# medvedevgroup/TwoPaCo

Hardware: AMD Instinct MI355X
Metric: kmers_hashed_per_sec (higher is better)
Workload: dtype u64

## Files before the change

twopaco_amd/csrc/tpc_capi.hip:

```cpp
#include "tpc_ctx.h"

namespace tpch {

int fail(tpc_ctx *c, int code, const char *fmt, ...)
{
    char buf[512];
    va_list ap;
    va_start(ap, fmt);
    vsnprintf(buf, sizeof buf, fmt, ap);
    va_end(ap);
    if (c) c->err = buf;
    return code;
}





TpcLaunch make_launch(const tpc_ctx *c)
{
    TpcLaunch a;
    a.P = c->P; a.tab = c->tab; a.bases = c->bases; a.nmask = c->nmask; a.n_text = c->n_text;
    a.n_tiles = c->n_tiles; a.filter = c->filter; a.stream = c->stream;
    a.stat_kernel = c->stat_kernel;
    return a;
}

TpcLaunch make_launch_periodic(const tpc_ctx *c)
{
    TpcLaunch a = make_launch(c);
    if (c->periodic && c->periodic_valid) {
        if (c->periodic_any_q) a.per_qs = c->periodic;
        if (c->periodic_any_i) a.per_i = c->periodic + (size_t)(1 + TPC_PER_PLANES) * c->n_words_alloc;
    }
    return a;
}

void ensure_periodic(tpc_ctx *c)
{
    if (c->periodic_valid || !c->opt_periodic || !c->bases || !c->have_params || c->n_words_alloc == 0) return;
    if ((c->sh_world > 1 || c->text_windowed) && !c->opt_shard_periodic && !replicated(c)) return;
    TpcLaunch a = make_launch(c);
    const uint64_t w0 = c->text_windowed ? c->text_w0 : 0, w1 = c->text_windowed ? std::min(c->text_w1, c->n_words) : c->n_words;
    const uint64_t pos_hi = c->text_windowed ? c->text_w1 << 5 : ~0ull;
    uint32_t any[2] = {0, 0};
    uint32_t *flags = reinterpret_cast<uint32_t *>(c->counters + 6);
    if (hipMemsetAsync(flags, 0, sizeof any, c->stream) != hipSuccess) return;
    tpc_launch_periodic_build(a, nullptr, nullptr, 0, nullptr, w0, w1, w0 << 5, pos_hi, flags);
    if (hipMemcpyAsync(any, flags, sizeof any, hipMemcpyDeviceToHost, c->stream) != hipSuccess || hipStreamSynchronize(c->stream) != hipSuccess) return;
    c->periodic_any_q = any[0] != 0; c->periodic_any_i = any[1] != 0;
    if (any[0] || any[1]) {
        const size_t words = (size_t)(2 + TPC_PER_PLANES) * c->n_words_alloc;
        if (!c->periodic && hipMalloc((void **)&c->periodic, words * sizeof(uint32_t)) != hipSuccess) { (void)hipGetLastError(); c->periodic = nullptr; return; }
        if (hipMemsetAsync(c->periodic, 0, words * sizeof(uint32_t), c->stream) != hipSuccess) return;
        tpc_launch_periodic_build(a, c->periodic, c->periodic + c->n_words_alloc, c->n_words_alloc, c->periodic + (size_t)(1 + TPC_PER_PLANES) * c->n_words_alloc, w0, w1, w0 << 5, pos_hi, flags);
        if (hipStreamSynchronize(c->stream) != hipSuccess) return;
    }
    c->periodic_valid = true;
}

uint64_t rotln_host(uint64_t x, int L, int r)
{
    if (r == 0) return x;
    const uint64_t maskn = (1ull << (L - r)) - 1ull;
    return ((x & maskn) << r) | (x >> (L - r));
}

std::atomic<int> tpc_test_fail_mallocs{0};
hipError_t dev_malloc(tpc_ctx *c, void **p, size_t bytes)
{
    hipError_t e = hipErrorOutOfMemory;
    if (tpc_test_fail_mallocs.load(std::memory_order_relaxed) > 0 && tpc_test_fail_mallocs.fetch_sub(1) > 0) *p = nullptr; else e = hipMalloc(p, bytes);
    if (e == hipSuccess) return e;
    (void)hipGetLastError();
    if (!release_partition_buffers(c)) return e;
    e = hipMalloc(p, bytes);
    if (e != hipSuccess) *p = nullptr;
    return e;
}


int read_counter(tpc_ctx *c, int i, uint64_t *out)
{
    unsigned long long v = 0;
    HIPCHK(c, hipMemcpyAsync(&v, c->counters + i, sizeof v, hipMemcpyDeviceToHost, c->stream));
    HIPCHK(c, hipStreamSynchronize(c->stream));
    *out = v;
    return 0;
}


int materialize_reset(tpc_ctx *c)
{
    { int rc0 = flush_pending_apply(c); if (rc0) return rc0; }
    if (!c->filter_zero_pending) return 0;
    Timed t(c, TPC_K_FILTER_RESET);
    HIPCHK(c, hipMemsetAsync(c->filter, 0, c->filter_words * sizeof(uint32_t), c->stream));
    c->filter_zero_pending = false;
    return 0;
}

int flush_pending_apply(tpc_ctx *c)
{
    if (!c->pending_apply) return 0;
    c->pending_apply = false;
    if (c->pending_lists) {
        c->pending_lists = false;
        Timed t(c, TPC_K_FUSED);
        const TpcPartPlan &g = c->pending_pl;
        if (tpc_launch_slice_combine(make_launch(c), g.slice_bits, g.b1, g.b2, g.perm_mult, g.perm_inv, nullptr, nullptr, nullptr, c->cmb_ls, true, c->pending_fresh, nullptr, 0, 1))
            return fail(c, -1, "apply launch failed");
        HIPCHK(c, hipGetLastError());
        return 0;
    }
    c->qb_valid = false;
    if (c->pending_shard) {
        c->pending_shard = false;
        Timed t(c, TPC_K_SHARD_APPLY);
        if (tpc_launch_insert_part_apply_only(make_launch(c), c->pending_pl, c->pending_fresh)) return fail(c, -1, "apply launch failed");
        HIPCHK(c, hipGetLastError());
        return 0;
    }
    Timed t(c, TPC_K_FUSED);
    const size_t ovf_need = std::max<size_t>((size_t)c->pending_novf * sizeof(uint64_t), sizeof(uint64_t));
    if (!ensure_pbuf(c, 4, ovf_need) || !ensure_pbuf(c, 5, 32 * sizeof(unsigned long long))) return fail(c, -10, "out of device memory for the deferred apply's overflow list");
    c->pending_pl.ovf = (uint64_t *)c->pbuf[4];
    c->pending_pl.ovf_cur = (unsigned long long *)c->pbuf[5];
    c->pending_pl.ovf_cap = std::min<uint64_t>(c->pending_pl.ovf_cap, c->pbytes[4] / sizeof(uint64_t));
    const unsigned long long cur[2] = {c->pending_novf, 0};
    if (c->pending_novf) HIPCHK(c, hipMemcpyAsync(c->pending_pl.ovf, c->ikeep_ovf, c->pending_novf * sizeof(uint64_t), hipMemcpyDeviceToDevice, c->stream));
    HIPCHK(c, hipMemcpyAsync(c->pending_pl.ovf_cur, cur, sizeof cur, hipMemcpyHostToDevice, c->stream));
    HIPCHK(c, hipStreamSynchronize(c->stream));
    if (tpc_launch_insert_part_apply_only(make_launch(c), c->pending_pl, c->pending_fresh)) return fail(c, -1, "apply launch failed");
    HIPCHK(c, hipGetLastError());
    return 0;
}

double range_mass(const tpc_ctx *c, uint64_t lo, uint64_t hi)
{
    const double size = (double)(c->P.lmask) + 1.0;
    auto below = [size](double x) { x = std::min(1.0, std::max(0.0, x / size)); return 1.0 - (1.0 - x) * (1.0 - x); };
    return std::min(1.0, std::max(0.0, below((double)hi + 1.0) - below((double)lo)));
}

bool ensure_pbuf(tpc_ctx *c, int i, size_t need)
{
    if (need <= c->pbytes[i]) return true;
    c->qb_valid = false;
    if (c->pbuf[i]) (void)hipFree(c->pbuf[i]);
    c->pbuf[i] = nullptr; c->pbytes[i] = 0;
    if (i == 8) c->off2_uploaded.clear();
    if (i == 11) c->off3_uploaded.clear();
    if (hipMalloc(&c->pbuf[i], need) != hipSuccess) { (void)hipGetLastError(); return false; }
    c->pbytes[i] = need;
    return true;
}

bool release_partition_buffers(tpc_ctx *c)
{
    if (c->pending_apply) return false;
    size_t held = 0;
    for (size_t b : c->pbytes) held += b;
    for (void *p : c->ikeep) if (p) held += 1;
    if (!held) return false;
    (void)hipStreamSynchronize(c->stream);
    c->qb_valid = false;
    for (int i = 0; i < tpc_ctx::NPBUF; i++) {
        if (c->pbuf[i]) (void)hipFree(c->pbuf[i]);
        c->pbuf[i] = nullptr; c->pbytes[i] = 0;
    }
    for (void *&p : c->ikeep) { if (p) (void)hipFree(p); p = nullptr; }
    for (size_t &b : c->ikeep_bytes) b = 0;
    c->off2_uploaded.clear();
    c->off3_uploaded.clear();
    c->sh_have[0] = c->sh_have[1] = false;
    c->stat_pbuf_releases++;
    return true;
}

uint64_t filter_words_for(int L, uint32_t world)
{
    return std::max<uint64_t>(1, ((1ull << L) >> 5) / world) + 1;
}

int64_t part_budget(const tpc_ctx *c)
{
    if (c->opt_part_budget > 0) return c->opt_part_budget;
    size_t free_b = 0, total_b = 0;
    if (hipMemGetInfo(&free_b, &total_b) != hipSuccess) { (void)hipGetLastError(); return (int64_t)40 << 30; }
    size_t held = 0;
    for (size_t b : c->pbytes) held += b;
    const double avail = std::max(0.0, (double)(free_b + held) - (double)(c->bases ? 0 : c->reserve_text_bytes));
    return std::max<int64_t>(std::min<int64_t>((int64_t)40 << 30, (int64_t)(avail * 0.90)), (int64_t)(avail * 0.60));
}

uint64_t next_batches(uint64_t b) { return b + std::max<uint64_t>(1, b / 8); }

uint64_t text_tiles512(const tpc_ctx *c) { return (c->n_text / TPC_RUN + 512) / 512; }

bool replicated(const tpc_ctx *c) { return c->opt_replicate && c->sh_world > 1; }
void pass_tiles(const tpc_ctx *c, uint64_t &t_begin, uint64_t &t_end)
{
    const uint64_t tiles = text_tiles512(c);
    t_begin = 0; t_end = tiles;
    if (replicated(c)) {
        const uint64_t chunk = (tiles + c->sh_world - 1) / c->sh_world;
        t_begin = std::min<uint64_t>(tiles, (uint64_t)c->sh_rank * chunk);
        t_end = std::min<uint64_t>(tiles, t_begin + chunk);
    }
}
uint64_t pass_tile_count(const tpc_ctx *c) { uint64_t a, b; pass_tiles(c, a, b); return std::max<uint64_t>(1, b - a); }

size_t qpart_need(const TpcQPlan &pl, int i)
{
    if (i == 0) return std::max(tpc_qpart_bytes(pl, 0), tpc_qpart_bytes(pl, 9));
    if (i == 9) return 0;
    return tpc_qpart_bytes(pl, i);
}

bool part_hash_supported(const tpc_ctx *c)
{
    if (c->P.q > TPC_KERNEL_MAXQ || tpc_test_force_anyq) return false;
    if (c->P.q > 8 && (c->P.L - c->opt_slice_bits > 24 || c->no_lean)) return false;
    return true;
}

bool plan_query(const tpc_ctx *c, uint64_t lo, uint64_t hi, bool gated, TpcQPlan &pl)
{
    const uint64_t tiles = pass_tile_count(c);
    if (c->P.q > TPC_KERNEL_MAXQ || tpc_test_force_anyq) return false;
    if (!replicated(c) && (c->opt_query_mode == 1 || (c->opt_query_mode == 0 && c->P.L < 28))) return false;
    const int64_t budget = part_budget(c);
    for (uint64_t batches = 1;; batches = next_batches(batches)) {
        const uint64_t per = (tiles + batches - 1) / batches;
        const bool ok = tpc_qpart_plan(c->P.L, c->opt_slice_bits, per, gated ? std::min(1.0, range_mass(c, lo, hi) * 1.15) : 1.0, pl, c->opt_part_levels);
        if (!ok && per * 512 * TPC_RUN <= (1ull << 30)) return false;
        if (ok && ((int64_t)(qpart_need(pl, 0) + tpc_qpart_bytes(pl, 2)) <= budget || (int64_t)per <= c->opt_part_min_tiles)) {
            const double per_slice = 6.0 * (gated ? range_mass(c, lo, hi) : 1.0) * (double)per * 512 * TPC_RUN / (double)(1ull << (c->P.L - pl.slice_bits));
            if (c->opt_query_mode == 0 && batches > 1 && per_slice < 2500.0 && !replicated(c)) return false;
            return true;
        }
        if (per <= 1) return false;
    }
}

int compact_mask(tpc_ctx *c, const uint32_t *m)
{
    Timed t(c, TPC_K_COMPACT);
    uint64_t n = 0;
    int rc = 0;
    if (m == c->rmask && c->rmask_sums_valid) {
        n = c->rmask_sums_n;
    } else {
        c->rmask_sums_valid = false;
        tpc_launch_mask_count(c->stream, m, c->n_words, c->block_sums, c->counters + 2);
        if ((rc = read_counter(c, 2, &n))) return rc;
    }
    rc = ensure(c, c->marks, c->marks_cap, n);
    if (rc) return rc;
    if (n) tpc_launch_mask_scatter(c->stream, m, c->n_words, c->block_sums, c->marks);
    c->n_marks = n;
    return 0;
}

}

extern "C" {

int tpc_ctx_create(int device, tpc_ctx **out)
{
    if (!out) return -1;
    *out = nullptr;
    int n = 0;
    if (hipGetDeviceCount(&n) != hipSuccess || n <= 0) return -2;
    if (device < 0 || device >= n) return -3;
    if (hipSetDevice(device) != hipSuccess) return -4;
    tpc_ctx *c = new tpc_ctx();
    c->device = device;
    c->dbg_ovf = getenv("TPC_DEBUG_OVF") != nullptr; c->dbg_phases = getenv("TPC_PROFILE_PHASES") != nullptr; c->dbg_timing = getenv("TWOPACO_TIMING") != nullptr; c->no_lean = TpcEnv::get().no_lean;
    if (const char *e = getenv("TPC_SHARD_TIGHT")) c->opt_shard_tight = atoi(e) ? 1 : 0;
    if (hipStreamCreate(&c->stream) != hipSuccess) { delete c; return -5; }
    for (int i = 0; i < TPC_K_COUNT; i++) {
        if (hipEventCreate(&c->ev0[i]) != hipSuccess || hipEventCreate(&c->ev1[i]) != hipSuccess) { delete c; return -5; }
    }
    if (hipMalloc((void **)&c->tab, TPC_TAB_WORDS * sizeof(uint64_t)) != hipSuccess ||
        hipMalloc((void **)&c->counters, 8 * sizeof(unsigned long long)) != hipSuccess ||
        hipMalloc((void **)&c->route_scratch, 128 * sizeof(unsigned long long)) != hipSuccess) { delete c; return -6; }
    *out = c;
    return 0;
}

void tpc_ctx_destroy(tpc_ctx *c)
{
    if (!c) return;
    (void)hipSetDevice(c->device);
    (void)hipStreamSynchronize(c->stream);
    void *ptrs[] = { c->tab, c->bases_alloc, c->nmask_alloc, c->filter, c->rmask, c->mask, c->marks, c->block_sums, c->table,
                     c->keys, c->idtab, c->emit_id, c->stream_buf, c->counters, c->route_scratch, c->sh_off, c->scan_blocks, c->sort_scratch, c->seg_name, c->seg_first, c->seg_ev[0], c->seg_ev[1], c->seg_ev[2] };
    for (void *p : ptrs) if (p) (void)hipFree(p);
    stream_part_release(c);
    for (void *p : c->pbuf) if (p) (void)hipFree(p);
    for (void *p : c->ikeep) if (p) (void)hipFree(p);
    if (c->periodic) (void)hipFree(c->periodic);
    if (c->cmb_base) (void)hipFree(c->cmb_base);
    if (c->cmb_cur) (void)hipFree(c->cmb_cur);
    if (c->ikeep_ovf) (void)hipFree(c->ikeep_ovf);
    if (c->iovf_cnt) (void)hipFree(c->iovf_cnt);
    if (c->iovf_off) (void)hipFree(c->iovf_off);
    for (int i = 0; i < TPC_K_COUNT; i++) { if (c->ev0[i]) (void)hipEventDestroy(c->ev0[i]); if (c->ev1[i]) (void)hipEventDestroy(c->ev1[i]); }
    if (c->stream2) (void)hipStreamDestroy(c->stream2);
    if (c->stream) (void)hipStreamDestroy(c->stream);
    delete c;
}

const char *tpc_last_error(const tpc_ctx *c) { return c ? c->err.c_str() : "null context"; }

int tpc_set_option(tpc_ctx *c, const char *name, int64_t value)
{
    if (!c || !name) return -1;
    if (!strcmp(name, "insert_test_first")) { c->opt_test_first = value != 0; return 0; }
    if (!strcmp(name, "insert_mode")) { c->opt_insert_mode = (int)value; return 0; }
    if (!strcmp(name, "slice_bits")) { c->opt_slice_bits = (int)value; return 0; }
    if (!strcmp(name, "query_mode")) { c->opt_query_mode = (int)value; return 0; }
    if (!strcmp(name, "part_budget_bytes")) { c->opt_part_budget = value; return 0; }
    if (!strcmp(name, "part_levels")) { c->opt_part_levels = (int)value; return 0; }
    if (!strcmp(name, "shard_tight_regions")) { c->opt_shard_tight = value ? 1 : 0; c->sh_have[0] = c->sh_have[1] = false; return 0; }
    if (!strcmp(name, "part_min_tiles")) { c->opt_part_min_tiles = value < 1 ? 1 : value; return 0; }
    if (!strcmp(name, "fuse_apply_lookup")) { c->opt_fuse = value != 0; return 0; }
    if (!strcmp(name, "test_q6_pb2")) { tpc_test_q6_pb2 = (int)value; return 0; }
    if (!strcmp(name, "insert_entry_fmt")) { tpc_test_insert_p3 = value == 3; return 0; }
    if (!strcmp(name, "shard_periodic_skip")) { c->opt_shard_periodic = value != 0; return 0; }
    if (!strcmp(name, "periodic_skip")) { c->opt_periodic = value != 0; if (!value) c->periodic_valid = false; return 0; }
    if (!strcmp(name, "test_tight_pinch")) { tpc_test_tight_pinch = (int)value; c->sh_have[0] = c->sh_have[1] = false; return 0; }
    if (!strcmp(name, "test_sched_cap")) { tpc_test_sched_cap = value > 0 ? (uint32_t)value : 0; return 0; }
    if (!strcmp(name, "text_window")) { c->opt_text_window = value != 0; return 0; }
    if (!strcmp(name, "replicate_filter")) { c->opt_replicate = value != 0; return 0; }
    if (!strcmp(name, "test_force_anyq")) { tpc_test_force_anyq = value != 0; return 0; }
    if (!strcmp(name, "test_fail_mallocs")) { tpc_test_fail_mallocs.store(value > 0 ? (int)value : 0); return 0; }
    return fail(c, -1, "unknown option %s", name);
}

int tpc_preload(int device)
{
    if (hipSetDevice(device) != hipSuccess) { (void)hipGetLastError(); return -10; }
    const bool timing = getenv("TWOPACO_TIMING") != nullptr;
    int (*const warm[4])() = { tpc_warm_partition, tpc_warm_qpartition, tpc_warm_pass2, tpc_warm_stream };
    const char *const name[4] = { "partition", "qpartition", "pass2", "stream" };
    for (int i = 0; i < 4; i++) {
        const auto t0 = std::chrono::steady_clock::now();
        if (warm[i]() != 0) return -10;
        if (timing) fprintf(stderr, "[timing]     code object %s: %.1f ms\n", name[i], std::chrono::duration<double, std::milli>(std::chrono::steady_clock::now() - t0).count());
    }
    return 0;
}

int tpc_warmup(tpc_ctx *c)
{
    if (!c) return -1;
    return tpc_preload(c->device);
}

int64_t tpc_get_stat(const tpc_ctx *c, const char *name)
{
    if (!c || !name) return -1;
    if (!strcmp(name, "insert_path")) return c->stat_path[0];
    if (!strcmp(name, "query_path")) return c->stat_path[1];
    if (!strcmp(name, "insert_entry_fmt")) return c->stat_fmt[0];
    if (!strcmp(name, "query_entry_fmt")) return c->stat_fmt[1];
    if (!strcmp(name, "insert_hash_kernel")) return c->stat_kernel[0];
    if (!strcmp(name, "query_hash_kernel")) return c->stat_kernel[1];
    if (!strcmp(name, "query_verify_kernel")) return c->stat_kernel[2];
    if (!strcmp(name, "insert_batches")) return c->stat_batches[0];
    if (!strcmp(name, "query_batches")) return c->stat_batches[1];
    if (!strcmp(name, "query_tiles_per_batch")) return c->stat_q_plan[0];
    if (!strcmp(name, "query_b1")) return c->stat_q_plan[1];
    if (!strcmp(name, "query_b2")) return c->stat_q_plan[2];
    if (!strcmp(name, "query_begun")) return c->stat_q_begun;
    if (!strcmp(name, "filter2_retries")) return c->stat_filter2_retries;
    if (!strcmp(name, "aggregate_retries")) return c->stat_aggregate_retries;
    if (!strcmp(name, "filter2_counted")) return c->stat_filter2_counted;
    if (!strcmp(name, "fused_lookups")) return c->stat_fused;
    if (!strcmp(name, "query_overflow_entries")) return c->stat_query_overflow;
    if (!strcmp(name, "insert_overflow_entries")) return c->stat_insert_overflow;
    if (!strcmp(name, "periodic_skip")) return c->periodic_valid ? 1 : 0;
    if (!strcmp(name, "pbuf_releases")) return c->stat_pbuf_releases;
    if (!strcmp(name, "text_words")) return (int64_t)(c->text_w1 - c->text_w0);
    if (!strcmp(name, "text_word_begin")) return (int64_t)c->text_w0;
    if (!strcmp(name, "text_word_end")) return (int64_t)c->text_w1;
    if (!strcmp(name, "periodic_any_query")) return c->periodic_valid && c->periodic_any_q ? 1 : 0;
    if (!strcmp(name, "periodic_any_insert")) return c->periodic_valid && c->periodic_any_i ? 1 : 0;
    if (!strcmp(name, "device_free_bytes") || !strcmp(name, "device_total_bytes")) {
        size_t free_b = 0, total_b = 0;
        if (hipSetDevice(c->device) != hipSuccess || hipMemGetInfo(&free_b, &total_b) != hipSuccess) { (void)hipGetLastError(); return -1; }
        return (int64_t)(name[7] == 'f' ? free_b : total_b);
    }
    if (!strcmp(name, "round_marks")) return c->marks_valid ? (int64_t)c->n_marks : -1;
    return -1;
}

int tpc_set_params(tpc_ctx *c, int k, int L, int q, const uint64_t *seed_table)
{
    if (!c || !seed_table) return -1;
    if (q < 1 || q > TPC_MAX_Q) return fail(c, -1, "q=%d unsupported (1..%d)", q, TPC_MAX_Q);
    if (L < 2 || L > 62) return fail(c, -1, "filter bits L=%d unsupported (2..62)", L);
    if (k < 1) return fail(c, -1, "k must be positive");
    const int C = (k + 4 + 31) / 32;
    if (C >= 20)
        return fail(c, -1, "The value of K is too big. Please refer to documentaion how to increase the max supported value of K.");
    HIPCHK(c, hipSetDevice(c->device));
    c->P.k = k; c->P.L = L; c->P.q = q; c->P.rk = k % L; c->P.lmask = (1ull << L) - 1ull;
    c->C = C;
    memset(c->tab_host, 0, sizeof c->tab_host);
    for (int i = 0; i < q; i++)
        for (int ch = 0; ch < 5; ch++) {
            const uint64_t h = seed_table[i * 5 + ch];
            if (h > c->P.lmask) return fail(c, -1, "seed table entry exceeds L bits");
            c->tab_host[i * 5 + ch] = h;
            c->tab_host[TPC_TAB_HK + i * 5 + ch] = rotln_host(h, L, c->P.rk);
        }
    HIPCHK(c, hipMemcpy(c->tab, c->tab_host, sizeof c->tab_host, hipMemcpyHostToDevice));
    const uint64_t fw = filter_words_for(L, c->opt_replicate ? 1 : c->sh_world);
    c->sh_have[0] = c->sh_have[1] = false;
    c->pending_lists = false; c->cmb_have_geo = false;
    if (fw != c->filter_words) {
        if (c->filter) (void)hipFree(c->filter);
        c->filter = nullptr;
        HIPCHK(c, hipMalloc((void **)&c->filter, fw * sizeof(uint32_t)));
        c->filter_words = fw;
    }
    c->have_params = true;
    c->periodic_valid = false;
    c->pending_apply = false;
    c->qb_valid = false;
    c->n_keys = 0; c->finalized = false; c->rounds_done = 0; c->mask_dirty = false; c->marks_valid = false; c->rmask_sums_valid = false;
    return 0;
}

int tpc_seq_upload(tpc_ctx *c, const uint64_t *bases, const uint32_t *nmask, uint64_t n_text)
{
    if (!c || !bases || !nmask || n_text < 2) return fail(c, -1, "bad text");
    HIPCHK(c, hipSetDevice(c->device));
    const auto t_begin = std::chrono::steady_clock::now();
    c->qb_valid = false;
    const uint64_t nw = (n_text + 31) / 32;
    if (!((nmask[0] & 1u) && ((nmask[(n_text - 1) >> 5] >> ((n_text - 1) & 31)) & 1u)))
        return fail(c, -1, "text must start and end with the N separator");
    const uint64_t tiles = (nw + TPC_TILE_THREADS - 1) / TPC_TILE_THREADS;
    const uint64_t alloc = ((n_text / TPC_RUN + 512) / 512) * 512 + TPC_XW_MAX + 2;
    uint64_t w0 = 0, w1 = alloc;
    const bool windowed = c->opt_text_window && c->sh_world > 1;
    if (windowed) {
        const uint64_t t512 = (n_text / TPC_RUN + 512) / 512, chunk = (t512 + c->sh_world - 1) / c->sh_world;
        const uint64_t ta = std::min<uint64_t>(t512, (uint64_t)c->sh_rank * chunk), tb = std::min<uint64_t>(t512, ta + chunk);
        w0 = ta * 512 > 0 ? ta * 512 - 1 : 0;
        w1 = std::min<uint64_t>(alloc, tb * 512 + TPC_XW_MAX + 2);
        if (w1 <= w0) w1 = w0 + 1;
    }
    for (void *p : { (void *)c->bases_alloc, (void *)c->nmask_alloc, (void *)c->rmask, (void *)c->mask, (void *)c->block_sums, (void *)c->periodic })
        if (p) (void)hipFree(p);
    c->periodic = nullptr; c->periodic_valid = false;
    c->bases = nullptr; c->nmask = nullptr; c->bases_alloc = nullptr; c->nmask_alloc = nullptr; c->rmask = nullptr; c->mask = nullptr; c->block_sums = nullptr;
    const uint64_t wn = w1 - w0;
    HIPCHK(c, dev_malloc(c, (void **)&c->bases_alloc, wn * sizeof(uint64_t)));
    HIPCHK(c, dev_malloc(c, (void **)&c->nmask_alloc, wn * sizeof(uint32_t)));
    HIPCHK(c, dev_malloc(c, (void **)&c->rmask, alloc * sizeof(uint32_t)));
    HIPCHK(c, dev_malloc(c, (void **)&c->mask, alloc * sizeof(uint32_t)));
    HIPCHK(c, dev_malloc(c, (void **)&c->block_sums, (alloc / 256 + 2 + 64) * sizeof(uint64_t)));
    HIPCHK(c, hipMemsetAsync(c->bases_alloc, 0, wn * sizeof(uint64_t), c->stream));
    HIPCHK(c, hipMemsetAsync(c->nmask_alloc, 0xFF, wn * sizeof(uint32_t), c->stream));
    HIPCHK(c, hipMemsetAsync(c->rmask, 0, alloc * sizeof(uint32_t), c->stream));
    HIPCHK(c, hipMemsetAsync(c->mask, 0, alloc * sizeof(uint32_t), c->stream));
    const uint64_t ce = std::min(nw, w1);
    uint32_t last_word = 0;
    if (ce > w0) {
        HIPCHK(c, hipMemcpyAsync(c->bases_alloc, bases + w0, (ce - w0) * sizeof(uint64_t), hipMemcpyHostToDevice, c->stream));
        HIPCHK(c, hipMemcpyAsync(c->nmask_alloc, nmask + w0, (ce - w0) * sizeof(uint32_t), hipMemcpyHostToDevice, c->stream));
        if ((n_text & 31) && ce == nw) {
            last_word = nmask[nw - 1] | (~0u << (n_text & 31));
            HIPCHK(c, hipMemcpyAsync(c->nmask_alloc + (nw - 1 - w0), &last_word, sizeof last_word, hipMemcpyHostToDevice, c->stream));
        }
    }
    HIPCHK(c, hipStreamSynchronize(c->stream));
    if (c->dbg_timing)
        fprintf(stderr, "[timing]   tpc_seq_upload (allocations, %.0f MB host to device): %.1f ms\n", (double)(ce > w0 ? (ce - w0) * 12 : 0) / 1e6,
                std::chrono::duration<double, std::milli>(std::chrono::steady_clock::now() - t_begin).count());
    c->bases = c->bases_alloc - w0;
    c->nmask = c->nmask_alloc - w0;
    c->text_windowed = windowed; c->text_w0 = w0; c->text_w1 = w1;
    c->pending_apply = false;
    c->n_text = n_text; c->n_words = (n_text >> 5) + 1; c->n_words_alloc = alloc; c->n_tiles = tiles;
    c->n_keys = 0; c->finalized = false; c->rounds_done = 0; c->mask_dirty = false; c->marks_valid = false; c->rmask_sums_valid = false;
    return 0;
}

int tpc_run_begin(tpc_ctx *c)
{
    if (!c) return -1;
    c->n_keys = 0; c->finalized = false; c->rounds_done = 0; c->mask_dirty = false; c->marks_valid = false; c->rmask_sums_valid = false;
    c->n_marks = 0; c->n_emit = 0; c->keys_host.clear();
    return 0;
}

int tpc_filter_reset(tpc_ctx *c)
{
    if (!c || !c->have_params) return fail(c, -1, "set_params first");
    c->filter_zero_pending = true;
    c->pending_apply = false;
    c->pending_shard = false;
    c->pending_lists = false;
    c->ev_used[TPC_K_FILTER_RESET] = false;
    return 0;
}

int tpc_pass1_insert(tpc_ctx *c, uint64_t lo, uint64_t hi, uint64_t *n_kmers)
{
    if (!c || !c->have_params || !c->bases) return fail(c, -1, "set_params and seq_upload first");
    if (c->sh_world > 1 && !c->opt_replicate) return fail(c, -1, "the filter is sharded: use tpc_shard_hash / tpc_shard_apply");
    HIPCHK(c, hipSetDevice(c->device));
    const bool gated = !(lo == 0 && hi >= c->P.lmask);
    { int rc0 = flush_pending_apply(c); if (rc0) return rc0; }
    c->qb_valid = false;
    ensure_periodic(c);
    if (n_kmers) HIPCHK(c, hipMemsetAsync(c->counters, 0, sizeof(unsigned long long), c->stream));
    uint64_t t_begin, t_end;
    pass_tiles(c, t_begin, t_end);
    TpcPartPlan pl;
    const double m_ins = gated ? range_mass(c, lo, hi) : 1.0;
    const double ins_frac = gated ? std::min(1.0, (1.0 - (1.0 - m_ins) * (1.0 - m_ins)) * 1.15) : 1.0;
    const uint64_t tiles = pass_tile_count(c);
    uint64_t batches = 1;
    bool defer = false;
    bool part = ((c->opt_insert_mode != 1 && !(c->opt_insert_mode == 0 && c->P.L < 28)) || replicated(c)) && part_hash_supported(c);
    if (replicated(c) && !part && c->P.q <= TPC_KERNEL_MAXQ)
        return fail(c, -1, "a replicated multi-GPU pass needs the partitioned hash kernels (q=%d, L=%d, slice_bits=%d are outside what they cover)", c->P.q, c->P.L, c->opt_slice_bits);
    if (part) {
        const int64_t budget = part_budget(c);
        for (;; batches = next_batches(batches)) {
            const uint64_t per = (tiles + batches - 1) / batches;
            if (!tpc_part_plan(c->P.L, c->P.q, c->opt_slice_bits, per, ins_frac, pl, c->opt_part_levels)) { part = false; break; }
            if ((int64_t)(std::max(tpc_part_buf1_bytes(pl), tpc_part_buf3_bytes(pl)) + tpc_part_buf2_bytes(pl)) <= budget || (int64_t)per <= c->opt_part_min_tiles) break;
        }
        if (part && c->opt_insert_mode == 0 && batches > 1 && !replicated(c)) {
            const double per_slice = (double)c->P.q * ins_frac * (double)pl.n_tiles * 512 * TPC_RUN / (double)(1ull << (c->P.L - pl.slice_bits));
            if (per_slice < (double)(1ull << pl.slice_bits) / 800.0) part = false;
        }
    }
    if (part) {
        size_t need[tpc_ctx::NPBUF] = { std::max(tpc_part_buf1_bytes(pl), tpc_part_buf3_bytes(pl)), tpc_part_cnt1_bytes(pl), tpc_part_buf2_bytes(pl), tpc_part_cnt2_bytes(pl),
                                        pl.ovf_cap * sizeof(uint64_t), 32 * sizeof(unsigned long long), 0, 0, 0, 0, tpc_part_cnt3_bytes(pl), 0 };
        TpcQPlan qpl;
        const bool qpart = plan_query(c, lo, hi, gated, qpl);
        for (int i = 0; i < tpc_ctx::NPBUF && qpart; i++) need[i] = std::max(need[i], qpart_need(qpl, i));
        for (int i = 0; i < tpc_ctx::NPBUF && part; i++) if (need[i]) part = ensure_pbuf(c, i, need[i]);
        defer = part && c->opt_fuse && batches == 1 && qpart && pl.b3 == 0 && qpl.b3 == 0 && qpl.slice_bits == pl.slice_bits &&
                qpl.b1 == pl.b1 && qpl.b2 == pl.b2 && (qpl.fmt == 6 || pl.fmt2 == 0);
        if (defer) {
            const size_t want[2] = { tpc_part_buf2_bytes(pl), tpc_part_cnt2_bytes(pl) };
            for (int i = 0; i < 2 && defer; i++) {
                if (want[i] <= c->ikeep_bytes[i]) continue;
                if (c->ikeep[i]) (void)hipFree(c->ikeep[i]);
                c->ikeep[i] = nullptr; c->ikeep_bytes[i] = 0;
                if (hipMalloc(&c->ikeep[i], want[i]) != hipSuccess) { (void)hipGetLastError(); defer = false; break; }
                c->ikeep_bytes[i] = want[i];
            }
        }
    }
    if (part) {
        pl.buf1 = (uint32_t *)c->pbuf[0]; pl.cnt1 = (uint32_t *)c->pbuf[1]; pl.buf2 = (uint32_t *)c->pbuf[2]; pl.cnt2 = (uint32_t *)c->pbuf[3];
        pl.ovf = (uint64_t *)c->pbuf[4]; pl.ovf_cur = (unsigned long long *)c->pbuf[5];
        pl.buf3 = (uint32_t *)c->pbuf[0]; pl.cnt3 = (uint32_t *)c->pbuf[10];
        if (defer) { pl.buf2 = (uint32_t *)c->ikeep[0]; pl.cnt2 = (uint32_t *)c->ikeep[1]; }
        bool fresh = c->filter_zero_pending;
        unsigned long long ov[2] = {0, 0};
        bool overflowed = false;
        uint64_t per_batch = 1;
        {
            Timed t(c, TPC_K_INSERT);
            if (fresh) HIPCHK(c, hipMemsetAsync(c->filter + (c->filter_words - 1), 0, sizeof(uint32_t), c->stream));
            const uint64_t per = pl.n_tiles;
            per_batch = per;
            for (uint64_t t0 = t_begin; t0 < t_end || t0 == t_begin; t0 += per) {
                pl.tile0 = t0;
                pl.n_tiles = t0 < t_end ? std::min<uint64_t>(per, t_end - t0) : 0;
                HIPCHK(c, hipMemsetAsync(pl.ovf_cur, 0, 2 * sizeof(unsigned long long), c->stream));
                if (defer) {
                    TpcPartPlan p1 = pl;
                    p1.rbuf1 = p1.buf1; p1.rcnt1 = p1.cnt1;
                    if (tpc_launch_insert_part_hash(make_launch_periodic(c), p1, lo, hi, gated, n_kmers ? c->counters : nullptr) ||
                        tpc_launch_insert_part_split(make_launch(c), p1)) return fail(c, -1, "partitioned insert launch failed");
                    HIPCHK(c, hipMemcpyAsync(ov, pl.ovf_cur, sizeof ov, hipMemcpyDeviceToHost, c->stream));
                    HIPCHK(c, hipStreamSynchronize(c->stream));
                    bool keep = ov[0] <= TPC_FUSE_MAX_OVF && ov[1] == 0;
                    const uint32_t n_slices = 1u << (p1.b1 + p1.b2);
                    if (keep && ov[0]) {
                        if (c->ikeep_ovf_cap < ov[0]) {
                            if (c->ikeep_ovf) (void)hipFree(c->ikeep_ovf);
                            c->ikeep_ovf = nullptr; c->ikeep_ovf_cap = 0;
                            const uint64_t cap = std::max<uint64_t>(4096, ov[0] + ov[0] / 4);
                            if (hipMalloc((void **)&c->ikeep_ovf, 2 * cap * sizeof(uint64_t)) == hipSuccess) c->ikeep_ovf_cap = cap; else { (void)hipGetLastError(); keep = false; }
                        }
                        if (keep && c->iovf_slices < n_slices) {
                            if (c->iovf_cnt) (void)hipFree(c->iovf_cnt);
                            if (c->iovf_off) (void)hipFree(c->iovf_off);
                            c->iovf_cnt = nullptr; c->iovf_off = nullptr; c->iovf_slices = 0;
                            if (hipMalloc((void **)&c->iovf_cnt, 2 * (size_t)n_slices * sizeof(uint32_t)) == hipSuccess &&
                                hipMalloc((void **)&c->iovf_off, ((size_t)n_slices + 1) * sizeof(uint64_t)) == hipSuccess) c->iovf_slices = n_slices;
                            else { (void)hipGetLastError(); keep = false; }
                        }
                        if (keep) {
                            HIPCHK(c, hipMemcpyAsync(c->ikeep_ovf, pl.ovf, ov[0] * sizeof(uint64_t), hipMemcpyDeviceToDevice, c->stream));
                            if (tpc_launch_ovf_by_slice(make_launch(c), c->ikeep_ovf, ov[0], p1.slice_bits, n_slices, c->iovf_cnt, c->iovf_cnt + n_slices, c->iovf_off,
                                                        c->ikeep_ovf + c->ikeep_ovf_cap)) return fail(c, -1, "overflow grouping launch failed");
                        }
                    }
                    if (keep) { c->pending_apply = true; c->pending_shard = false; c->pending_lists = false; c->pending_fresh = fresh; c->pending_pl = p1; c->pending_novf = ov[0]; }
                    else if (tpc_launch_insert_part_apply_only(make_launch(c), p1, fresh)) return fail(c, -1, "apply launch failed");
                    break;
                }
                if (tpc_launch_insert_partitioned(make_launch_periodic(c), pl, lo, hi, gated, fresh, n_kmers ? c->counters : nullptr))
                    return fail(c, -1, "partitioned insert launch failed");
                fresh = false;
                HIPCHK(c, hipMemcpyAsync(ov, pl.ovf_cur, sizeof ov, hipMemcpyDeviceToHost, c->stream));
                if (t0 + per < t_end) { HIPCHK(c, hipStreamSynchronize(c->stream)); overflowed = overflowed || ov[1] != 0; }
            }
        }
        c->filter_zero_pending = false;
        HIPCHK(c, hipGetLastError());
        HIPCHK(c, hipStreamSynchronize(c->stream));
        if (c->dbg_ovf)
            fprintf(stderr, "[ovf] insert: %llu overflow entries (cap %llu, flag %llu) b1=%d b2=%d ppr=%d cap1=%llu cap2=%llu nwg1=%u\n", ov[0], (unsigned long long)pl.ovf_cap, ov[1], pl.b1,
                    pl.b2, pl.pos_per_round, (unsigned long long)pl.cap1, (unsigned long long)pl.cap2, pl.nwg1);
        overflowed = overflowed || ov[1] != 0;
        c->stat_path[0] = (pl.b3 ? 3 : 2) + (overflowed ? 10 : 0);
        c->stat_fmt[0] = pl.fmt2;
        c->stat_insert_overflow = (int64_t)ov[0];
        c->stat_batches[0] = (int64_t)((tiles + per_batch - 1) / per_batch);
        if (!overflowed) {
            if (n_kmers) return read_counter(c, 0, n_kmers);
            return 0;
        }
        if (replicated(c)) return fail(c, -20, "overflow list overflowed (address skew beyond what the sharded path handles)");
        if (n_kmers) HIPCHK(c, hipMemsetAsync(c->counters, 0, sizeof(unsigned long long), c->stream));
    }
    int rc = materialize_reset(c);
    if (rc) return rc;
    if (!part) { c->stat_path[0] = 1; c->stat_batches[0] = 1; }
    {
        Timed t(c, TPC_K_INSERT);
        TpcLaunch ad = make_launch(c);
        if (replicated(c)) { ad.g_begin = t_begin * 512ull * TPC_RUN; ad.g_end = t_end * 512ull * TPC_RUN; }
        if (part) ad.stat_kernel = nullptr;
        if (tpc_launch_insert(ad, lo, hi, gated, c->opt_test_first != 0, n_kmers ? c->counters : nullptr))
            return fail(c, -1, "insert launch failed");
    }
    HIPCHK(c, hipGetLastError());
    if (n_kmers) return read_counter(c, 0, n_kmers);
    return 0;
}

int tpc_reserve(tpc_ctx *c, uint64_t n_text_max)
{
    if (!c || !c->have_params) return fail(c, -1, "set_params first");
    if (c->sh_world > 1 || n_text_max < 2) return 0;
    HIPCHK(c, hipSetDevice(c->device));
    const uint64_t keep = c->n_text;
    c->n_text = n_text_max;
    c->reserve_text_bytes = c->bases ? 0 : (n_text_max / 32 + 1024) * 20;
    const uint64_t tiles = text_tiles512(c);
    size_t need[tpc_ctx::NPBUF] = {};
    TpcPartPlan pl;
    bool part = c->opt_insert_mode != 1 && !(c->opt_insert_mode == 0 && c->P.L < 28) && part_hash_supported(c);
    if (part) {
        const int64_t budget = part_budget(c);
        for (uint64_t batches = 1;; batches = next_batches(batches)) {
            const uint64_t per = (tiles + batches - 1) / batches;
            if (!tpc_part_plan(c->P.L, c->P.q, c->opt_slice_bits, per, 1.0, pl, c->opt_part_levels)) { part = false; break; }
            if ((int64_t)(std::max(tpc_part_buf1_bytes(pl), tpc_part_buf3_bytes(pl)) + tpc_part_buf2_bytes(pl)) <= budget || (int64_t)per <= c->opt_part_min_tiles) break;
        }
    }
    if (part) {
        const size_t ins[tpc_ctx::NPBUF] = { std::max(tpc_part_buf1_bytes(pl), tpc_part_buf3_bytes(pl)), tpc_part_cnt1_bytes(pl), tpc_part_buf2_bytes(pl), tpc_part_cnt2_bytes(pl),
                                             pl.ovf_cap * sizeof(uint64_t), 32 * sizeof(unsigned long long), 0, 0, 0, 0, tpc_part_cnt3_bytes(pl), 0 };
        for (int i = 0; i < tpc_ctx::NPBUF; i++) need[i] = ins[i];
    }
    TpcQPlan qpl;
    const bool qpart = plan_query(c, 0, c->P.lmask + 1, false, qpl);
    for (int i = 0; i < tpc_ctx::NPBUF && qpart; i++) need[i] = std::max(need[i], qpart_need(qpl, i));
    c->n_text = keep;
    for (int i = 0; i < tpc_ctx::NPBUF; i++)
        if (need[i] && !ensure_pbuf(c, i, need[i])) {
            release_partition_buffers(c);
            return 0;
        }
    if (part && qpart && c->opt_fuse && pl.b3 == 0 && qpl.b3 == 0) {
        const size_t want[2] = { tpc_part_buf2_bytes(pl), tpc_part_cnt2_bytes(pl) };
        for (int i = 0; i < 2; i++) {
            if (want[i] <= c->ikeep_bytes[i]) continue;
            if (c->ikeep[i]) (void)hipFree(c->ikeep[i]);
            c->ikeep[i] = nullptr; c->ikeep_bytes[i] = 0;
            if (hipMalloc(&c->ikeep[i], want[i]) != hipSuccess) { (void)hipGetLastError(); break; }
            c->ikeep_bytes[i] = want[i];
        }
    }
    return 0;
}

int tpc_pass1_split_hist(tpc_ctx *c, const uint64_t *rec_start, const uint64_t *rec_len, uint32_t n_rec, uint32_t *bins_host)
{
    if (!c || !c->have_params || !c->bases || !bins_host) return fail(c, -1, "bad arguments");
    if (c->sh_world > 1) return fail(c, -1, "the split pass needs the whole filter as scratch: not available on a sharded context");
    HIPCHK(c, hipSetDevice(c->device));
    const uint64_t BINS = 1ull << 24;
    c->filter_zero_pending = false;
    c->pending_apply = false;
    const auto t_begin = std::chrono::steady_clock::now();
    std::vector<uint64_t> rs, rl;
    for (uint32_t r = 0; r < n_rec; r++) if (rec_len[r] >= (uint64_t)c->P.k) { rs.push_back(rec_start[r]); rl.push_back(rec_len[r]); }
    uint32_t *d_em = nullptr, *d_bins = nullptr;
    uint64_t *d_rec = nullptr;
    HIPCHK(c, hipMalloc((void **)&d_em, c->n_words_alloc * sizeof(uint32_t)));
    HIPCHK(c, hipMalloc((void **)&d_bins, BINS * sizeof(uint32_t)));
    HIPCHK(c, hipMalloc((void **)&d_rec, std::max<size_t>(1, 2 * rs.size()) * sizeof(uint64_t)));
    if (!rs.empty()) {
        HIPCHK(c, hipMemcpyAsync(d_rec, rs.data(), rs.size() * sizeof(uint64_t), hipMemcpyHostToDevice, c->stream));
        HIPCHK(c, hipMemcpyAsync(d_rec + rs.size(), rl.data(), rl.size() * sizeof(uint64_t), hipMemcpyHostToDevice, c->stream));
    }
    tpc_launch_split_emask(c->stream, d_rec, d_rec + rs.size(), (uint32_t)rs.size(), c->P.k, c->n_words_alloc, d_em);
    HIPCHK(c, hipMemsetAsync(d_bins, 0, BINS * sizeof(uint32_t), c->stream));
    HIPCHK(c, hipMemsetAsync(c->filter, 0, c->filter_words * sizeof(uint32_t), c->stream));
    const uint64_t real = 1ull << c->P.L;
    const uint64_t bin_size = std::max<uint64_t>(1, real / BINS);
    {
        Timed t(c, TPC_K_SPLIT);
        tpc_launch_split(make_launch(c), d_em, d_bins, bin_size);
    }
    HIPCHK(c, hipMemcpyAsync(bins_host, d_bins, BINS * sizeof(uint32_t), hipMemcpyDeviceToHost, c->stream));
    HIPCHK(c, hipStreamSynchronize(c->stream));
    (void)hipFree(d_em);
    (void)hipFree(d_bins);
    (void)hipFree(d_rec);
    if (c->dbg_timing)
        fprintf(stderr, "[timing]   tpc_pass1_split_hist: %.1f ms in all, the split kernel %.1f ms\n", std::chrono::duration<double, std::milli>(std::chrono::steady_clock::now() - t_begin).count(),
                tpc_kernel_ms(c, TPC_K_SPLIT));
    return 0;
}

namespace {
int pass1_query_impl(tpc_ctx *c, uint64_t lo, uint64_t hi, uint64_t *n_marks, bool begin_only);
}

int tpc_pass1_query(tpc_ctx *c, uint64_t lo, uint64_t hi, uint64_t *n_marks) { return pass1_query_impl(c, lo, hi, n_marks, false); }

int tpc_pass1_query_begin(tpc_ctx *c, uint64_t lo, uint64_t hi) { return pass1_query_impl(c, lo, hi, nullptr, true); }

namespace {

int pass1_query_impl(tpc_ctx *c, uint64_t lo, uint64_t hi, uint64_t *n_marks, bool begin_only)
{
    if (!c || !c->have_params || !c->bases) return fail(c, -1, "set_params and seq_upload first");
    if (c->sh_world > 1 && !c->opt_replicate) return fail(c, -1, "the filter is sharded: use tpc_shard_hash / tpc_shard_apply");
    HIPCHK(c, hipSetDevice(c->device));
    const bool gated = !(lo == 0 && hi >= c->P.lmask);
    bool begun = !begin_only && c->qb_valid && c->qb_lo == lo && c->qb_hi == hi;
    c->qb_valid = false;
    auto fuses = [c](const TpcQPlan &p) {
        return c->pending_apply && !c->pending_shard && p.b3 == 0 && p.slice_bits == c->pending_pl.slice_bits && p.b1 == c->pending_pl.b1 && p.b2 == c->pending_pl.b2 &&
               (p.fmt == 6 || c->pending_pl.fmt2 == 0);
    };
    if (begun && c->pending_apply && !fuses(c->qb_pl)) {
        int rc0 = materialize_reset(c);
        if (rc0) return rc0;
        begun = false;
    }
    c->stat_q_begun = begun ? 1 : 0;
    c->marks_valid = false; c->rmask_sums_valid = false;
    ensure_periodic(c);
    TpcQPlan pl;
    uint64_t t_begin, t_end;
    pass_tiles(c, t_begin, t_end);
    bool part = begun ? (pl = c->qb_pl, true) : plan_query(c, lo, hi, gated, pl);
    if (replicated(c)) {
        if (!part && c->P.q <= TPC_KERNEL_MAXQ) return fail(c, -1, "a replicated multi-GPU pass needs the partitioned query (q=%d, L=%d, slice_bits=%d)", c->P.q, c->P.L, c->opt_slice_bits);
        if (!begun) HIPCHK(c, hipMemsetAsync(c->rmask, 0, c->n_words_alloc * sizeof(uint32_t), c->stream));
    }
    if (begin_only && !part) return 0;
    if (part)
        for (int i = 0; i < tpc_ctx::NPBUF && part; i++) if (qpart_need(pl, i)) part = ensure_pbuf(c, i, qpart_need(pl, i));
    const bool fused = !begin_only && part && fuses(pl);
    if (!fused && !begin_only) { int rc0 = materialize_reset(c); if (rc0) return rc0; }
    if (part) {
        pl.buf1 = (uint64_t *)c->pbuf[0]; pl.cnt1 = (uint32_t *)c->pbuf[1]; pl.buf2 = (uint64_t *)c->pbuf[2]; pl.cnt2 = (uint32_t *)c->pbuf[3];
        pl.ovf = (uint64_t *)c->pbuf[4]; pl.ovf_cur = (unsigned long long *)c->pbuf[5];
        pl.surv = (uint64_t *)c->pbuf[6]; pl.surv_cur = (unsigned long long *)c->pbuf[7];
        pl.off2 = (const uint64_t *)c->pbuf[8];
        if (c->off2_uploaded != pl.off2_host) {
            HIPCHK(c, hipMemcpy(c->pbuf[8], pl.off2_host.data(), pl.off2_host.size() * 8, hipMemcpyHostToDevice));
            c->off2_uploaded = pl.off2_host;
        }
        pl.buf3 = (uint64_t *)c->pbuf[0]; pl.cnt3 = (uint32_t *)c->pbuf[10]; pl.off3 = (const uint64_t *)c->pbuf[11];
        pl.bnd = (uint32_t *)c->pbuf[18];
        if (pl.b3 && c->off3_uploaded != pl.off3_host) {
            HIPCHK(c, hipMemcpy(c->pbuf[11], pl.off3_host.data(), pl.off3_host.size() * 8, hipMemcpyHostToDevice));
            c->off3_uploaded = pl.off3_host;
        }
        unsigned long long f1[2] = {0, 0}, f2 = 0;
        bool overflowed = false;
        uint64_t per_batch = 1;
        {
            Timed t(c, TPC_K_QUERY);
            const uint64_t per = pl.n_tiles;
            per_batch = per;
            for (uint64_t t0 = t_begin; (t0 < t_end || t0 == t_begin) && !overflowed; t0 += per) {
                pl.tile0 = t0;
                pl.tile0_global = t0;
                pl.n_tiles = t0 < t_end ? std::min<uint64_t>(per, t_end - t0) : 0;
                const bool presplit = begun && t0 == t_begin;
                if (!presplit) {
                    HIPCHK(c, hipMemsetAsync(pl.ovf_cur, 0, 32 * sizeof(unsigned long long), c->stream));
                    HIPCHK(c, hipMemsetAsync(pl.surv_cur, 0, TPC_SURV_CUR_WORDS * sizeof(unsigned long long), c->stream));
                }
                if (begin_only) {
                    TpcQPlan p1 = pl;
                    p1.rbuf1 = p1.buf1; p1.rcnt1 = p1.cnt1;
                    if (tpc_launch_query_part_hash(make_launch_periodic(c), p1, c->rmask, lo, hi, gated) || tpc_launch_query_part_split(make_launch(c), p1))
                        return fail(c, -1, "partitioned query launch failed");
                    HIPCHK(c, hipGetLastError());
                    c->qb_valid = true; c->qb_lo = lo; c->qb_hi = hi;
                    c->qb_pl = pl; c->qb_pl.n_tiles = per;
                    return 0;
                }
                if (fused && t0 == t_begin) {
                    TpcQPlan p1 = pl;
                    p1.rbuf1 = p1.buf1; p1.rcnt1 = p1.cnt1;
                    p1.presplit = presplit;
                    c->pending_apply = false;
                    c->stat_fused++;
                    if (!presplit && tpc_launch_query_part_hash(make_launch_periodic(c), p1, c->rmask, lo, hi, gated)) return fail(c, -1, "partitioned query launch failed");
                    {
                        Timed tf(c, TPC_K_FUSED);
                        TpcLaunch af = make_launch(c);
                        af.ev_lookup0 = c->ev0[TPC_K_LOOKUP]; af.ev_lookup1 = c->ev1[TPC_K_LOOKUP]; c->ev_used[TPC_K_LOOKUP] = true;
                        const bool lists = c->pending_lists;
                        c->pending_lists = false;
                        if (tpc_launch_query_part_fused_lookup(af, p1, c->pending_pl, c->pending_fresh, c->pending_novf && !lists ? c->ikeep_ovf + c->ikeep_ovf_cap : nullptr,
                                                               c->pending_novf && !lists ? c->iovf_off : nullptr, lists ? &c->cmb_ls : nullptr)) return fail(c, -1, "fused lookup launch failed");
                    }
                    if (tpc_launch_query_verify(make_launch(c), p1, c->rmask)) return fail(c, -1, "verify launch failed");
                } else if (presplit) {
                    TpcQPlan p1 = pl;
                    p1.rbuf1 = p1.buf1; p1.rcnt1 = p1.cnt1;
                    p1.presplit = true;
                    if (tpc_launch_query_part_lookup(make_launch(c), p1) || tpc_launch_query_verify(make_launch(c), p1, c->rmask)) return fail(c, -1, "partitioned query launch failed");
                } else
                if (tpc_launch_query_partitioned(make_launch_periodic(c), pl, c->rmask, lo, hi, gated)) return fail(c, -1, "partitioned query launch failed");
                HIPCHK(c, hipMemcpyAsync(f1, pl.ovf_cur, sizeof f1, hipMemcpyDeviceToHost, c->stream));
                HIPCHK(c, hipMemcpyAsync(&f2, pl.surv_cur + 64, sizeof f2, hipMemcpyDeviceToHost, c->stream));
                if (t0 + per < t_end) {
                    unsigned long long sc[TPC_SURV_CUR_WORDS], batch_marks = 0;
                    const uint64_t w0 = t0 * 512, wn = std::min<uint64_t>(pl.n_tiles * 512, c->n_words > w0 ? c->n_words - w0 : 0);
                    if (wn) tpc_launch_mask_count(c->stream, c->rmask + w0, wn, c->block_sums, c->counters + 3);
                    HIPCHK(c, hipMemcpyAsync(sc, pl.surv_cur, sizeof sc, hipMemcpyDeviceToHost, c->stream));
                    if (wn) HIPCHK(c, hipMemcpyAsync(&batch_marks, c->counters + 3, sizeof batch_marks, hipMemcpyDeviceToHost, c->stream));
                    HIPCHK(c, hipStreamSynchronize(c->stream));
                    overflowed = f1[1] != 0 || f2 != 0;
                    unsigned long long surv = 0;
                    for (int i = 0; i < 64; i++) surv += std::min<unsigned long long>(sc[i], pl.surv_cap);
                    if (surv > 0) pl.group_survivors = batch_marks * 4 >= surv;
                }
            }
            if (c->periodic_valid && c->periodic_any_q && c->periodic) tpc_launch_periodic_copy(c->stream, c->rmask, c->periodic, c->periodic + c->n_words_alloc, c->n_words_alloc, c->n_words);
            tpc_launch_mask_count(c->stream, c->rmask, c->n_words, c->block_sums, c->counters + 1);
        }
        HIPCHK(c, hipGetLastError());
        uint64_t n = 0;
        int rc = read_counter(c, 1, &n);
        if (rc) return rc;
        overflowed = overflowed || f1[1] != 0 || f2 != 0;
        c->stat_query_overflow = (int64_t)f1[0];
        c->stat_path[1] = (pl.b3 ? 3 : 2) + (overflowed ? 10 : 0);
        c->stat_fmt[1] = pl.fmt;
        c->stat_batches[1] = (int64_t)((pass_tile_count(c) + per_batch - 1) / per_batch);
        c->stat_q_plan[0] = (int64_t)per_batch; c->stat_q_plan[1] = pl.b1; c->stat_q_plan[2] = pl.b2;
        if (c->dbg_ovf) {
            unsigned long long sc[65];
            (void)hipMemcpy(sc, pl.surv_cur, sizeof sc, hipMemcpyDeviceToHost);
            unsigned long long tot = 0, most = 0;
            for (int i = 0; i < 64; i++) { tot += sc[i]; most = std::max(most, sc[i]); }
            fprintf(stderr, "[ovf] query: %llu overflow entries (cap %llu, flag %llu), survivors %llu (fullest list %llu of %llu, flag %llu) b1=%d b2=%d ppr=%d loads=%d\n", f1[0],
                    (unsigned long long)pl.ovf_cap, f1[1], tot, most, (unsigned long long)pl.surv_cap, f2, pl.b1, pl.b2, pl.pos_per_round, pl.loads);
            static const char *const dump_path = getenv("TPC_DUMP_SURV");
            if (const char *path = dump_path) {
                if (FILE *fp = fopen(path, "w")) {
                    for (int i = 0; i < 64; i++) {
                        const size_t n = (size_t)std::min<unsigned long long>(sc[i], pl.surv_cap);
                        std::vector<uint64_t> ids(n);
                        if (n) (void)hipMemcpy(ids.data(), pl.surv + (size_t)i * pl.surv_cap, n * 8, hipMemcpyDeviceToHost);
                        for (uint64_t v : ids) fprintf(fp, "%llu\n", (unsigned long long)v);
                    }
                    fclose(fp);
                }
            }
            static const bool dbg_regions = getenv("TPC_DEBUG_OVF_REGIONS") != nullptr;
            if (dbg_regions && f1[0]) {
                const size_t n = (size_t)std::min<unsigned long long>(f1[0], 1u << 22);
                std::vector<uint64_t> ent(2 * n);
                (void)hipMemcpy(ent.data(), pl.ovf, 2 * n * 8, hipMemcpyDeviceToHost);
                std::map<uint32_t, uint32_t> h;
                std::map<uint64_t, uint32_t> ha;
                for (size_t i = 0; i < n; i++) { h[(uint32_t)(ent[2 * i] >> pl.slice_bits)]++; ha[ent[2 * i]]++; }
                std::vector<std::pair<uint32_t, uint32_t>> top;
                for (auto &kv : h) top.push_back({kv.second, kv.first});
                std::sort(top.rbegin(), top.rend());
                fprintf(stderr, "[ovf]   %zu entries in %zu permuted slices, %zu distinct addresses; top:", n, h.size(), ha.size());
                for (size_t i = 0; i < std::min<size_t>(top.size(), 10); i++) fprintf(stderr, " slice %u x %u;", top[i].second, top[i].first);
                std::vector<std::pair<uint32_t, uint64_t>> topa;
                for (auto &kv : ha) topa.push_back({kv.second, kv.first});
                std::sort(topa.rbegin(), topa.rend());
                for (size_t i = 0; i < std::min<size_t>(topa.size(), 6); i++) fprintf(stderr, " addr %llx x %u (edge %llu pos %llu);", (unsigned long long)topa[i].second, topa[i].first, 0ull, 0ull);
                fprintf(stderr, "\n");
            }
            if (dbg_regions && !pl.b3 && pl.fmt == 0) {
                const size_t nreg = pl.off2_host.size() - 1;
                std::vector<uint32_t> cnt(nreg);
                (void)hipMemcpy(cnt.data(), pl.cnt2, nreg * 4, hipMemcpyDeviceToHost);
                const uint32_t smask = (1u << (pl.b1 + pl.b2)) - 1u;
                size_t full = 0;
                std::vector<uint32_t> hist(64, 0);
                for (size_t r = 0; r < nreg; r++) {
                    const uint64_t cap = pl.off2_host[r + 1] - pl.off2_host[r];
                    const uint32_t s = (uint32_t)(((uint64_t)r * pl.perm_inv) & smask);
                    if (cnt[r] + 16 >= cap) { full++; hist[s >> (pl.b1 + pl.b2 - 6)]++; if (full <= 12) fprintf(stderr, "[ovf]   region %zu (slice %u of %zu): %u of %llu\n", r, s, nreg, cnt[r], (unsigned long long)cap); }
                }
                fprintf(stderr, "[ovf]   %zu full regions; by 64ths of the address space:", full);
                for (int i = 0; i < 64; i++) fprintf(stderr, " %u", hist[i]);
                fprintf(stderr, "\n");
            }
        }
        if (c->dbg_phases) {
            unsigned long long pr[32];
            (void)hipMemcpy(pr, pl.ovf_cur, sizeof pr, hipMemcpyDeviceToHost);
            fprintf(stderr, "[phases] ovf=%llu  split: push %llu book %llu copy %llu rounds %llu | hash: push %llu book %llu copy %llu rounds %llu (10 ns ticks summed over WGs) | lost at level 1: %llu, at level 2/3: %llu\n",
                    pr[0], pr[8], pr[9], pr[10], pr[12], pr[16], pr[17], pr[18], pr[20], pr[25], pr[27]);
        }
        if (!overflowed) {
            c->rmask_sums_valid = true;
            c->rmask_sums_n = n;
            if (n_marks) *n_marks = n;
            return 0;
        }
        if (replicated(c)) return fail(c, -20, "overflow or survivor list overflowed (address skew beyond what the sharded path handles)");
    }
    if (!part) { c->stat_path[1] = 1; c->stat_batches[1] = 1; }
    HIPCHK(c, hipMemsetAsync(c->counters + 1, 0, sizeof(unsigned long long), c->stream));
    {
        Timed t(c, TPC_K_QUERY);
        TpcLaunch ad = make_launch(c);
        if (replicated(c)) { ad.g_begin = t_begin * 512ull * TPC_RUN; ad.g_end = t_end * 512ull * TPC_RUN; }
        if (part) ad.stat_kernel = nullptr;
        if (tpc_launch_query(ad, c->rmask, lo, hi, gated, c->counters + 1)) return fail(c, -1, "query launch failed");
    }
    HIPCHK(c, hipGetLastError());
    uint64_t n = 0;
    int rc = read_counter(c, 1, &n);
    if (rc) return rc;
    if (n_marks) *n_marks = n;
    return 0;
}

}

uint64_t tpc_filter_words(const tpc_ctx *c) { return c ? c->filter_words : 0; }

int tpc_filter_download(tpc_ctx *c, uint32_t *words_host)
{
    if (!c || !c->filter) return -1;
    HIPCHK(c, hipSetDevice(c->device));
    { int rc0 = materialize_reset(c); if (rc0) return rc0; }
    HIPCHK(c, hipStreamSynchronize(c->stream));
    HIPCHK(c, hipMemcpy(words_host, c->filter, c->filter_words * sizeof(uint32_t), hipMemcpyDeviceToHost));
    return 0;
}

int tpc_filter_upload(tpc_ctx *c, const uint32_t *words_host)
{
    if (!c || !c->filter || !words_host) return -1;
    HIPCHK(c, hipSetDevice(c->device));
    HIPCHK(c, hipStreamSynchronize(c->stream));
    HIPCHK(c, hipMemcpy(c->filter, words_host, c->filter_words * sizeof(uint32_t), hipMemcpyHostToDevice));
    c->filter_zero_pending = false;
    c->pending_apply = false;
    return 0;
}

uint64_t tpc_mask_words(const tpc_ctx *c) { return c ? c->n_words : 0; }

int tpc_mask_download(tpc_ctx *c, int run_wide, uint32_t *words_host)
{
    if (!c || !c->rmask) return -1;
    HIPCHK(c, hipSetDevice(c->device));
    HIPCHK(c, hipStreamSynchronize(c->stream));
    HIPCHK(c, hipMemcpy(words_host, run_wide ? c->mask : c->rmask, c->n_words * sizeof(uint32_t), hipMemcpyDeviceToHost));
    return 0;
}

int tpc_periodic_download(tpc_ctx *c, uint32_t *qs_host, uint32_t *planes_host, uint32_t *ins_host)
{
    if (!c || !c->have_params || !c->bases || !qs_host || !planes_host || !ins_host) return fail(c, -1, "set_params and seq_upload first");
    HIPCHK(c, hipSetDevice(c->device));
    ensure_periodic(c);
    const size_t nw = c->n_words, stride = c->n_words_alloc;
    memset(qs_host, 0, nw * sizeof(uint32_t));
    memset(planes_host, 0, nw * TPC_PER_PLANES * sizeof(uint32_t));
    memset(ins_host, 0, nw * sizeof(uint32_t));
    if (!(c->periodic_valid && c->periodic && (c->periodic_any_q || c->periodic_any_i))) return 0;
    HIPCHK(c, hipStreamSynchronize(c->stream));
    HIPCHK(c, hipMemcpy(qs_host, c->periodic, nw * sizeof(uint32_t), hipMemcpyDeviceToHost));
    for (int b = 0; b < TPC_PER_PLANES; b++)
        HIPCHK(c, hipMemcpy(planes_host + (size_t)b * nw, c->periodic + (size_t)(1 + b) * stride, nw * sizeof(uint32_t), hipMemcpyDeviceToHost));
    HIPCHK(c, hipMemcpy(ins_host, c->periodic + (size_t)(1 + TPC_PER_PLANES) * stride, nw * sizeof(uint32_t), hipMemcpyDeviceToHost));
    return 0;
}

int tpc_hash_dump(tpc_ctx *c, uint64_t g0, uint64_t n, uint64_t *out_host)
{
    if (!c || !c->have_params || !c->bases) return -1;
    if (g0 + n + c->P.k > c->n_text) return fail(c, -1, "range past the text");
    if (c->text_windowed) return fail(c, -1, "this context holds only its window of the text");
    HIPCHK(c, hipSetDevice(c->device));
    uint64_t *d = nullptr;
    const size_t bytes = n * 2 * c->P.q * sizeof(uint64_t);
    HIPCHK(c, hipMalloc((void **)&d, bytes));
    tpc_launch_hash_dump(make_launch(c), g0, n, d);
    HIPCHK(c, hipMemcpy(out_host, d, bytes, hipMemcpyDeviceToHost));
    (void)hipFree(d);
    return 0;
}

double tpc_kernel_ms(const tpc_ctx *c, int which)
{
    if (!c || which < 0 || which >= TPC_K_COUNT || !c->ev_used[which]) return -1.0;
    if (hipEventSynchronize(c->ev1[which]) != hipSuccess) return -1.0;
    float ms = 0;
    if (hipEventElapsedTime(&ms, c->ev0[which], c->ev1[which]) != hipSuccess) return -1.0;
    return ms;
}

}
```

twopaco_amd/csrc/tpc_capi_pass2.hip:

```cpp
#include "tpc_ctx.h"

namespace {
int pass2_filter_impl(tpc_ctx *c, const uint64_t *fmarks, uint64_t n_fmarks, bool external, uint64_t abundance, uint64_t *n_true, uint64_t *n_false, uint64_t *table_size,
                      bool records = false, bool aggregated = false);
inline bool aggregated_counted(uint64_t abundance) { return abundance < (1ull << 40); }
}

int tpc_pass2_filter(tpc_ctx *c, uint64_t abundance, uint64_t *n_true, uint64_t *n_false, uint64_t *table_size)
{
    return pass2_filter_impl(c, nullptr, 0, false, abundance, n_true, n_false, table_size);
}

int tpc_pass2_marks(tpc_ctx *c, uint64_t *n_marks)
{
    if (!c || !c->have_params || !c->bases || !n_marks) return fail(c, -1, "set_params and seq_upload first");
    HIPCHK(c, hipSetDevice(c->device));
    int rc = compact_mask(c, c->rmask);
    if (rc) return rc;
    c->marks_valid = true;
    *n_marks = c->n_marks;
    return 0;
}

int tpc_pass2_mark_owners(tpc_ctx *c, uint32_t world, uint64_t *pos_dev, int32_t *owner_dev)
{
    if (!c || !c->marks_valid || world == 0 || (c->n_marks && (!pos_dev || !owner_dev))) return fail(c, -1, "tpc_pass2_marks first");
    if (c->text_windowed) return fail(c, -1, "this context holds only its window of the text (option text_window)");
    HIPCHK(c, hipSetDevice(c->device));
    if (c->n_marks) {
        HIPCHK(c, hipMemcpyAsync(pos_dev, c->marks, c->n_marks * sizeof(uint64_t), hipMemcpyDeviceToDevice, c->stream));
        if (tpc_launch_mark_owner(make_launch(c), c->C, c->marks, c->n_marks, world, owner_dev)) return fail(c, -1, "owner launch failed");
    }
    HIPCHK(c, hipGetLastError());
    HIPCHK(c, hipStreamSynchronize(c->stream));
    return 0;
}

int tpc_pass2_filter_positions(tpc_ctx *c, const uint64_t *pos_dev, uint64_t n, uint64_t abundance, uint64_t *n_true, uint64_t *n_false, uint64_t *table_size)
{
    if (n && !pos_dev) return fail(c, -1, "bad arguments");
    return pass2_filter_impl(c, pos_dev, n, true, abundance, n_true, n_false, table_size);
}

int tpc_pass2_mark_records(tpc_ctx *c, uint32_t world, uint64_t *records_dev, int32_t *owner_dev)
{
    if (!c || !c->marks_valid || world == 0 || (c->n_marks && (!records_dev || !owner_dev))) return fail(c, -1, "tpc_pass2_marks first");
    HIPCHK(c, hipSetDevice(c->device));
    if (c->n_marks && tpc_launch_mark_records(make_launch(c), c->C, c->marks, c->n_marks, world, records_dev, owner_dev)) return fail(c, -1, "record launch failed");
    HIPCHK(c, hipGetLastError());
    HIPCHK(c, hipStreamSynchronize(c->stream));
    return 0;
}

int tpc_pass2_filter_records(tpc_ctx *c, const uint64_t *records_dev, uint64_t n, uint64_t abundance, uint64_t *n_true, uint64_t *n_false, uint64_t *table_size)
{
    if (n && !records_dev) return fail(c, -1, "bad arguments");
    return pass2_filter_impl(c, records_dev, n, true, abundance, n_true, n_false, table_size, true);
}

int tpc_pass2_aggregate_records(tpc_ctx *c, uint32_t world, uint64_t abundance, uint64_t *records_dev, int32_t *owner_dev, uint64_t *n_records)
{
    if (!c || !c->marks_valid || world == 0 || !n_records || (c->n_marks && (!records_dev || !owner_dev))) return fail(c, -1, "tpc_pass2_marks first");
    HIPCHK(c, hipSetDevice(c->device));
    *n_records = 0;
    if (c->n_marks == 0) return 0;
    const size_t sb = tpc_table_slot_bytes(c->C);
    TpcLaunch a = make_launch(c);
    const bool counted = aggregated_counted(abundance);
    if (!c->scan_blocks) HIPCHK(c, hipMalloc((void **)&c->scan_blocks, 2 * TPC_SCAN2_BLOCKS * sizeof(uint64_t)));
    uint64_t full = 1024;
    while (full < 2 * c->n_marks + 2) full <<= 1;
    uint64_t cap = 1024;
    while (cap < c->n_marks / 4 + 2) cap <<= 1;
    c->stat_filter2_counted = counted ? 1 : 0;
    c->stat_aggregate_retries = 0;
    for (;;) {
        if (cap > c->table_alloc) {
            if (c->table) (void)hipFree(c->table);
            c->table = nullptr;
            c->table_alloc = 0;
            HIPCHK(c, dev_malloc(c, &c->table, cap * sb));
            c->table_alloc = cap;
        }
        HIPCHK(c, hipMemsetAsync(c->counters + 6, 0, sizeof(unsigned long long), c->stream));
        Timed t(c, TPC_K_FILTER2);
        tpc_launch_table_init(c->stream, c->table, cap);
        if (tpc_launch_filter2(a, c->C, c->marks, c->n_marks, c->table, cap, counted, c->counters + 6)) return fail(c, -1, "filter2 launch failed");
        if (tpc_launch_scan2_count(a, c->table, cap, abundance, counted, c->scan_blocks, c->scan_blocks + TPC_SCAN2_BLOCKS, c->counters + 4))
            return fail(c, -1, "scan2 launch failed");
        unsigned long long three[3] = {0, 0, 0};
        HIPCHK(c, hipMemcpyAsync(three, c->counters + 4, sizeof three, hipMemcpyDeviceToHost, c->stream));
        HIPCHK(c, hipStreamSynchronize(c->stream));
        if (!three[2]) {
            *n_records = three[1];
            if (tpc_launch_table_records(a, c->C, c->marks, c->table, cap, c->scan_blocks + TPC_SCAN2_BLOCKS, world, records_dev, owner_dev))
                return fail(c, -1, "record launch failed");
            break;
        }
        if (cap >= full) return fail(c, -1, "exact-filter table overflow at full size");
        cap = full;
        c->stat_aggregate_retries++;
    }
    HIPCHK(c, hipGetLastError());
    HIPCHK(c, hipStreamSynchronize(c->stream));
    return 0;
}

int tpc_pass2_filter_aggregated(tpc_ctx *c, const uint64_t *records_dev, uint64_t n, uint64_t abundance, uint64_t *n_true, uint64_t *n_false, uint64_t *table_size)
{
    if (n && !records_dev) return fail(c, -1, "bad arguments");
    return pass2_filter_impl(c, records_dev, n, true, abundance, n_true, n_false, table_size, true, true);
}

int tpc_shard_permute_rows(tpc_ctx *c, const uint64_t *src_dev, const uint32_t *perm_dev, uint64_t n, int row_words, uint64_t *dst_dev)
{
    if (!c || row_words < 1 || (n && (!src_dev || !perm_dev || !dst_dev))) return fail(c, -1, "bad arguments");
    HIPCHK(c, hipSetDevice(c->device));
    tpc_launch_permute_rows(c->stream, src_dev, perm_dev, n, row_words, dst_dev);
    HIPCHK(c, hipGetLastError());
    HIPCHK(c, hipStreamSynchronize(c->stream));
    return 0;
}

namespace {

int pass2_filter_impl(tpc_ctx *c, const uint64_t *fmarks, uint64_t n_fmarks, bool external, uint64_t abundance, uint64_t *n_true, uint64_t *n_false, uint64_t *table_size,
                      bool records, bool aggregated)
{
    if (!c || !c->have_params || !c->bases) return fail(c, -1, "set_params and seq_upload first");
    if (c->text_windowed && !records) return fail(c, -1, "this context holds only its window of the text (option text_window): the second pass needs all of it");
    HIPCHK(c, hipSetDevice(c->device));
    if (!external) {
        int rc = compact_mask(c, c->rmask);
        if (rc) return rc;
        c->marks_valid = true;
    } else if (!c->marks_valid) return fail(c, -1, "tpc_pass2_marks first");
    const uint64_t *marks = external ? fmarks : c->marks;
    const uint64_t n_marks = external ? n_fmarks : c->n_marks;
    const size_t sb = tpc_table_slot_bytes(c->C);
    TpcLaunch a = make_launch(c);
    const bool counted = (records && aggregated_counted(abundance)) || (!aggregated && abundance < n_marks);
    if (!c->scan_blocks) HIPCHK(c, hipMalloc((void **)&c->scan_blocks, 2 * TPC_SCAN2_BLOCKS * sizeof(uint64_t)));
    uint64_t full = 1024;
    while (full < 2 * n_marks + 2) full <<= 1;
    uint64_t cap = 1024;
    while (cap < n_marks / 4 + 2) cap <<= 1;
    if (aggregated) cap = full;
    uint64_t tp = 0, used = 0;
    c->stat_filter2_retries = 0;
    c->stat_filter2_counted = counted ? 1 : 0;
    for (;;) {
        if (cap > c->table_alloc) {
            if (c->table) (void)hipFree(c->table);
            c->table = nullptr;
            c->table_alloc = 0;
            HIPCHK(c, dev_malloc(c, &c->table, cap * sb));
            c->table_alloc = cap;
        }
        c->table_cap = cap;
        HIPCHK(c, hipMemsetAsync(c->counters + 6, 0, sizeof(unsigned long long), c->stream));
        {
            Timed t(c, TPC_K_FILTER2);
            tpc_launch_table_init(c->stream, c->table, cap);
            if (records ? tpc_launch_filter2_rec(a, c->C, marks, n_marks, c->table, cap, counted, c->counters + 6)
                        : tpc_launch_filter2(a, c->C, marks, n_marks, c->table, cap, counted, c->counters + 6)) return fail(c, -1, "filter2 launch failed");
        }
        uint64_t too_full = 0;
        {
            Timed t(c, TPC_K_SCAN2);
            if (tpc_launch_scan2_count(a, c->table, cap, abundance, counted, c->scan_blocks, c->scan_blocks + TPC_SCAN2_BLOCKS, c->counters + 4))
                return fail(c, -1, "scan2 launch failed");
            unsigned long long three[3] = {0, 0, 0};
            HIPCHK(c, hipMemcpyAsync(three, c->counters + 4, sizeof three, hipMemcpyDeviceToHost, c->stream));
            HIPCHK(c, hipStreamSynchronize(c->stream));
            tp = three[0]; used = three[1]; too_full = three[2];
            if (!too_full && tp) {
                const uint64_t need = c->n_keys + tp;
                if (need > c->keys_cap) {
                    uint64_t *nk = nullptr;
                    const uint64_t ncap = need + need / 4 + 1024;
                    HIPCHK(c, dev_malloc(c, (void **)&nk, ncap * c->C * sizeof(uint64_t)));
                    if (c->n_keys) HIPCHK(c, hipMemcpyAsync(nk, c->keys, c->n_keys * c->C * sizeof(uint64_t), hipMemcpyDeviceToDevice, c->stream));
                    HIPCHK(c, hipStreamSynchronize(c->stream));
                    if (c->keys) (void)hipFree(c->keys);
                    c->keys = nk;
                    c->keys_cap = ncap;
                }
                if (records ? tpc_launch_scan2_write_rec(a, c->C, marks, c->table, cap, abundance, counted, c->scan_blocks, c->keys + c->n_keys * c->C)
                            : tpc_launch_scan2_write(a, c->C, marks, c->table, cap, abundance, counted, c->scan_blocks, c->keys + c->n_keys * c->C))
                    return fail(c, -1, "scan2 launch failed");
                c->n_keys += tp;
            }
        }
        if (!too_full) break;
        if (cap >= full) return fail(c, -1, "exact-filter table overflow at full size");
        cap = full;
        c->stat_filter2_retries++;
    }
    if (c->rounds_done == 0) {
        HIPCHK(c, hipMemcpyAsync(c->mask, c->rmask, c->n_words_alloc * sizeof(uint32_t), hipMemcpyDeviceToDevice, c->stream));
    } else {
        tpc_launch_mask_or(c->stream, c->mask, c->rmask, c->n_words_alloc);
        c->mask_dirty = true;
    }
    c->rounds_done++;
    c->finalized = false;
    HIPCHK(c, hipGetLastError());
    HIPCHK(c, hipStreamSynchronize(c->stream));
    if (n_true) *n_true = tp;
    if (n_false) *n_false = used - tp;
    if (table_size) *table_size = used;
    return 0;
}

}

int tpc_junctions_finalize(tpc_ctx *c, uint64_t *n_junctions)
{
    if (!c || !c->have_params) return fail(c, -1, "set_params first");
    HIPCHK(c, hipSetDevice(c->device));
    {
        Timed t(c, TPC_K_SORT);
        int rc = tpc_launch_sort_keys(c->stream, c->C, c->P.k, c->keys, c->n_keys, &c->sort_scratch, &c->sort_scratch_bytes);
        if (rc) return fail(c, rc, "key sort failed (%d)", rc);
        uint64_t cap = 1024;
        while (cap < 2 * c->n_keys + 2) cap <<= 1;
        const size_t slot_bytes = c->C == 1 ? 16 : 4;
        if (cap * slot_bytes > c->idtab_bytes) {
            if (c->idtab) (void)hipFree(c->idtab);
            c->idtab = nullptr;
            c->idtab_bytes = 0;
            HIPCHK(c, dev_malloc(c, (void **)&c->idtab, cap * slot_bytes));
            c->idtab_bytes = cap * slot_bytes;
        }
        c->idtab_cap = cap;
        HIPCHK(c, hipMemsetAsync(c->idtab, 0, cap * slot_bytes, c->stream));
        if (c->n_keys >= 0xFFFFFFFFull) return fail(c, -1, "too many junctions for the 32-bit id index");
        tpc_launch_idtab_build(c->stream, c->C, c->keys, c->n_keys, c->idtab, cap);
    }
    HIPCHK(c, hipGetLastError());
    HIPCHK(c, hipStreamSynchronize(c->stream));
    c->finalized = true;
    c->keys_host.clear();
    if (n_junctions) *n_junctions = c->n_keys;
    return 0;
}

int tpc_key_words(const tpc_ctx *c) { return c ? c->C : 0; }

int tpc_junction_keys(tpc_ctx *c, uint64_t *keys_host)
{
    if (!c || !c->finalized) return fail(c, -1, "junctions_finalize first");
    HIPCHK(c, hipSetDevice(c->device));
    if (c->n_keys) HIPCHK(c, hipMemcpy(keys_host, c->keys, c->n_keys * c->C * sizeof(uint64_t), hipMemcpyDeviceToHost));
    return 0;
}

int tpc_junction_keys_raw(tpc_ctx *c, uint64_t *keys_host, uint64_t *n)
{
    if (!c || !n) return -1;
    HIPCHK(c, hipSetDevice(c->device));
    *n = c->n_keys;
    if (keys_host && c->n_keys) {
        HIPCHK(c, hipStreamSynchronize(c->stream));
        HIPCHK(c, hipMemcpy(keys_host, c->keys, c->n_keys * c->C * sizeof(uint64_t), hipMemcpyDeviceToHost));
    }
    return 0;
}

int tpc_junction_keys_set(tpc_ctx *c, const uint64_t *keys_host, uint64_t n)
{
    if (!c || (!keys_host && n)) return -1;
    HIPCHK(c, hipSetDevice(c->device));
    if (n > c->keys_cap) {
        if (c->keys) (void)hipFree(c->keys);
        c->keys = nullptr; c->keys_cap = 0;
        HIPCHK(c, dev_malloc(c, (void **)&c->keys, (n + 1024) * c->C * sizeof(uint64_t)));
        c->keys_cap = n + 1024;
    }
    if (n) HIPCHK(c, hipMemcpy(c->keys, keys_host, n * c->C * sizeof(uint64_t), hipMemcpyHostToDevice));
    c->n_keys = n;
    c->finalized = false;
    c->keys_host.clear();
    return 0;
}

int tpc_junction_keys_export(tpc_ctx *c, uint64_t *dst_dev, uint64_t cap_keys, uint64_t *n)
{
    if (!c || !n || (!dst_dev && cap_keys)) return -1;
    HIPCHK(c, hipSetDevice(c->device));
    *n = c->n_keys;
    const uint64_t m = std::min(c->n_keys, cap_keys);
    if (m) HIPCHK(c, hipMemcpyAsync(dst_dev, c->keys, m * c->C * sizeof(uint64_t), hipMemcpyDeviceToDevice, c->stream));
    HIPCHK(c, hipStreamSynchronize(c->stream));
    return 0;
}

int tpc_junction_keys_import(tpc_ctx *c, const uint64_t *src_dev, uint64_t n, int append)
{
    if (!c || (!src_dev && n)) return -1;
    HIPCHK(c, hipSetDevice(c->device));
    const uint64_t base = append ? c->n_keys : 0;
    const uint64_t need = base + n;
    if (need > c->keys_cap) {
        uint64_t *nk = nullptr;
        const uint64_t ncap = need + need / 2 + 1024;
        HIPCHK(c, dev_malloc(c, (void **)&nk, ncap * c->C * sizeof(uint64_t)));
        if (base) HIPCHK(c, hipMemcpy(nk, c->keys, base * c->C * sizeof(uint64_t), hipMemcpyDeviceToDevice));
        if (c->keys) (void)hipFree(c->keys);
        c->keys = nk;
        c->keys_cap = ncap;
    }
    if (n) HIPCHK(c, hipMemcpyAsync(c->keys + base * c->C, src_dev, n * c->C * sizeof(uint64_t), hipMemcpyDeviceToDevice, c->stream));
    HIPCHK(c, hipStreamSynchronize(c->stream));
    c->n_keys = need;
    c->finalized = false;
    c->keys_host.clear();
    return 0;
}

int64_t tpc_get_id(tpc_ctx *c, const char *kmer)
{
    if (!c || !c->finalized || !kmer) return TPC_INVALID_VERTEX;
    const int k = c->P.k, C = c->C;
    if (c->keys_host.size() != c->n_keys * C) {
        c->keys_host.resize(c->n_keys * C);
        if (tpc_junction_keys(c, c->keys_host.data())) return TPC_INVALID_VERTEX;
    }
    std::vector<uint64_t> fw(C, 0), rc(C, 0);
    for (int i = 0; i < k; i++) {
        int code;
        switch (kmer[i]) { case 'A': code = 0; break; case 'C': code = 1; break; case 'G': code = 2; break; case 'T': code = 3; break; default: return TPC_INVALID_VERTEX; }
        fw[i >> 5] |= (uint64_t)code << (2 * (i & 31));
        const int j = k - 1 - i;
        rc[j >> 5] |= (uint64_t)(3 - code) << (2 * (j & 31));
    }
    auto find = [&](const std::vector<uint64_t> &key) -> int64_t {
        uint64_t lo = 0, hi = c->n_keys;
        auto less = [&](const uint64_t *a, const uint64_t *b) {
            for (int w = 0; w < C; w++) if (a[w] != b[w]) return a[w] < b[w];
            return false;
        };
        while (lo < hi) {
            const uint64_t mid = (lo + hi) / 2;
            if (less(&c->keys_host[mid * C], key.data())) lo = mid + 1; else hi = mid;
        }
        if (lo < c->n_keys && !less(key.data(), &c->keys_host[lo * C]) && !less(&c->keys_host[lo * C], key.data())) return (int64_t)lo;
        return -1;
    };
    int64_t r = find(fw);
    if (r >= 0) return r + 1;
    r = find(rc);
    if (r >= 0) return -(r + 1);
    return TPC_INVALID_VERTEX;
}

int tpc_emit(tpc_ctx *c, uint64_t *n_marked, uint64_t *n_valid)
{
    if (!c || !c->finalized) return fail(c, -1, "junctions_finalize first");
    HIPCHK(c, hipSetDevice(c->device));
    int rc;
    if (c->mask_dirty || !c->marks_valid) {
        if ((rc = compact_mask(c, c->mask))) return rc;
        c->marks_valid = false; c->rmask_sums_valid = false;
    }
    if (c->n_marks > c->emit_cap || !c->emit_id) {
        if (c->emit_id) (void)hipFree(c->emit_id);
        c->emit_id = nullptr;
        const uint64_t cap = c->n_marks + c->n_marks / 8 + 16;
        HIPCHK(c, dev_malloc(c, (void **)&c->emit_id, cap * sizeof(int64_t)));
        c->emit_cap = cap;
    }
    HIPCHK(c, hipMemsetAsync(c->counters + 3, 0, sizeof(unsigned long long), c->stream));
    {
        Timed t(c, TPC_K_EMIT);
        if (tpc_launch_emit(make_launch(c), c->C, c->marks, c->n_marks, c->keys, c->n_keys, c->idtab, c->idtab_cap, c->emit_id, c->counters + 3))
            return fail(c, -1, "emit launch failed");
    }
    HIPCHK(c, hipGetLastError());
    uint64_t nv = 0;
    if ((rc = read_counter(c, 3, &nv))) return rc;
    c->n_emit = c->n_marks;
    if (n_marked) *n_marked = c->n_marks;
    if (n_valid) *n_valid = nv;
    return 0;
}

int tpc_emit_stream(tpc_ctx *c, const uint64_t *rec_start, const uint64_t *rec_len, uint32_t n_rec, uint64_t *n_bytes, uint64_t *n_records)
{
    if (!c || !c->finalized || !rec_start || !rec_len || !n_rec) return fail(c, -1, "tpc_emit first; records required");
    if (c->n_emit != c->n_marks || (c->n_marks && !c->emit_id)) return fail(c, -1, "tpc_emit first");
    HIPCHK(c, hipSetDevice(c->device));
    uint32_t r_last = 0;
    for (uint32_t r = 0; r < n_rec; r++) if (rec_len[r] >= (uint64_t)c->P.k) r_last = r;
    uint64_t *d_rec = nullptr, *vscan = nullptr;
    void *plan = nullptr;
    int rc = 0;
    uint64_t totals[2] = {0, 0};
    if (hipMalloc((void **)&d_rec, 2 * (size_t)n_rec * sizeof(uint64_t)) != hipSuccess || dev_malloc(c, (void **)&vscan, (c->n_marks + 1) * sizeof(uint64_t)) != hipSuccess ||
        hipMalloc(&plan, tpc_stream_plan_bytes(n_rec)) != hipSuccess) rc = -10;
    if (rc == 0 && (hipMemcpyAsync(d_rec, rec_start, (size_t)n_rec * 8, hipMemcpyHostToDevice, c->stream) != hipSuccess ||
                    hipMemcpyAsync(d_rec + n_rec, rec_len, (size_t)n_rec * 8, hipMemcpyHostToDevice, c->stream) != hipSuccess)) rc = -10;
    if (rc == 0) {
        Timed t(c, TPC_K_STREAM);
        rc = tpc_launch_stream_plan(c->stream, d_rec, d_rec + n_rec, n_rec, c->P.k, c->marks, c->emit_id, c->n_marks, vscan, plan, r_last, totals);
        if (rc == 0) {
            const uint64_t bytes = totals[1] * 12;
            if (bytes > c->stream_cap) {
                if (c->stream_buf) (void)hipFree(c->stream_buf);
                c->stream_buf = nullptr; c->stream_cap = 0;
                if (dev_malloc(c, (void **)&c->stream_buf, bytes + 64) != hipSuccess) rc = -10; else c->stream_cap = bytes;
            }
            if (rc == 0 && bytes)
                rc = tpc_launch_stream_write(c->stream, d_rec, d_rec + n_rec, n_rec, c->P.k, c->marks, c->emit_id, c->n_marks, vscan, plan, r_last,
                                             c->n_keys + 42, c->stream_buf);
            c->stream_bytes = bytes;
        }
    }
    const hipError_t e = hipStreamSynchronize(c->stream);
    for (void *p : { (void *)d_rec, (void *)vscan, plan }) if (p) (void)hipFree(p);
    if (rc) return fail(c, rc, "junction stream failed (%d)", rc);
    HIPCHK(c, e);
    HIPCHK(c, hipGetLastError());
    if (n_bytes) *n_bytes = c->stream_bytes;
    if (n_records) *n_records = totals[0];
    return 0;
}

namespace tpch {
void stream_part_release(tpc_ctx *c)
{
    for (void *p : { (void *)c->sp_rec, (void *)c->sp_vscan, (void *)c->sp_cnt, (void *)c->sp_lo, (void *)c->sp_flags }) if (p) (void)hipFree(p);
    c->sp_rec = c->sp_vscan = c->sp_cnt = c->sp_lo = nullptr;
    c->sp_flags = nullptr;
    c->sp_n_rec = 0;
}
}

int tpc_shard_chunk(const tpc_ctx *c, uint64_t *chunk_lo, uint64_t *chunk_hi)
{
    if (!c || !chunk_lo || !chunk_hi || !c->n_text) return -1;
    const uint64_t W = c->sh_world, tiles = text_tiles512(c), chunk = (tiles + W - 1) / W;
    const uint64_t t0 = std::min<uint64_t>(tiles, (uint64_t)c->sh_rank * chunk), t1 = std::min<uint64_t>(tiles, t0 + chunk);
    *chunk_lo = t0 * 512 * TPC_RUN;
    *chunk_hi = c->sh_rank + 1 == W ? ~0ull : t1 * 512 * TPC_RUN;
    return 0;
}

int tpc_emit_stream_partial(tpc_ctx *c, const uint64_t *rec_start, const uint64_t *rec_len, uint32_t n_rec, uint64_t *cnt_host, uint32_t *flags_host)
{
    if (!c || !c->finalized || !rec_start || !rec_len || !n_rec || !cnt_host || !flags_host) return fail(c, -1, "tpc_emit first; records required");
    if (c->n_emit != c->n_marks || (c->n_marks && !c->emit_id)) return fail(c, -1, "tpc_emit first");
    HIPCHK(c, hipSetDevice(c->device));
    stream_part_release(c);
    if (hipMalloc((void **)&c->sp_rec, 2 * (size_t)n_rec * sizeof(uint64_t)) != hipSuccess || dev_malloc(c, (void **)&c->sp_vscan, (c->n_marks + 1) * sizeof(uint64_t)) != hipSuccess ||
        hipMalloc((void **)&c->sp_cnt, (size_t)n_rec * sizeof(uint64_t)) != hipSuccess || hipMalloc((void **)&c->sp_lo, (size_t)n_rec * sizeof(uint64_t)) != hipSuccess ||
        hipMalloc((void **)&c->sp_flags, (size_t)n_rec * sizeof(uint32_t)) != hipSuccess) { stream_part_release(c); return fail(c, -10, "out of device memory for the junction stream"); }
    c->sp_n_rec = n_rec;
    HIPCHK(c, hipMemcpyAsync(c->sp_rec, rec_start, (size_t)n_rec * 8, hipMemcpyHostToDevice, c->stream));
    HIPCHK(c, hipMemcpyAsync(c->sp_rec + n_rec, rec_len, (size_t)n_rec * 8, hipMemcpyHostToDevice, c->stream));
    int rc;
    {
        Timed t(c, TPC_K_STREAM);
        rc = tpc_launch_stream_partial(c->stream, c->sp_rec, c->sp_rec + n_rec, n_rec, c->P.k, c->marks, c->emit_id, c->n_marks, c->sp_vscan, c->sp_cnt, c->sp_flags, c->sp_lo);
    }
    if (rc) return fail(c, rc, "junction stream failed (%d)", rc);
    HIPCHK(c, hipMemcpy(cnt_host, c->sp_cnt, (size_t)n_rec * sizeof(uint64_t), hipMemcpyDeviceToHost));
    HIPCHK(c, hipMemcpy(flags_host, c->sp_flags, (size_t)n_rec * sizeof(uint32_t), hipMemcpyDeviceToHost));
    HIPCHK(c, hipGetLastError());
    return 0;
}

int tpc_emit_stream_part(tpc_ctx *c, const uint64_t *rec_start, const uint64_t *rec_len, uint32_t n_rec, const uint32_t *gflags_host,
                         const uint64_t *e_scan_host, const uint64_t *s_scan_host, const uint64_t *before_host, uint32_t r_last,
                         uint64_t chunk_lo, uint64_t chunk_hi, uint64_t slot0, uint64_t n_slots, uint64_t *n_bytes)
{
    (void)rec_start; (void)rec_len;
    if (!c || !c->sp_rec || c->sp_n_rec != n_rec || !gflags_host || !e_scan_host || !s_scan_host || !before_host) return fail(c, -1, "tpc_emit_stream_partial first");
    HIPCHK(c, hipSetDevice(c->device));
    uint64_t *d_e = nullptr, *d_s = nullptr, *d_b = nullptr;
    uint32_t *d_f = nullptr;
    int rc = 0;
    if (hipMalloc((void **)&d_e, ((size_t)n_rec + 1) * 8) != hipSuccess || hipMalloc((void **)&d_s, ((size_t)n_rec + 1) * 8) != hipSuccess ||
        hipMalloc((void **)&d_b, (size_t)n_rec * 8) != hipSuccess || hipMalloc((void **)&d_f, (size_t)n_rec * 4) != hipSuccess) rc = -10;
    const uint64_t bytes = n_slots * 12;
    if (rc == 0 && bytes > c->stream_cap) {
        if (c->stream_buf) (void)hipFree(c->stream_buf);
        c->stream_buf = nullptr; c->stream_cap = 0;
        if (dev_malloc(c, (void **)&c->stream_buf, bytes + 64) != hipSuccess) rc = -10; else c->stream_cap = bytes;
    }
    if (rc == 0 && (hipMemcpyAsync(d_e, e_scan_host, ((size_t)n_rec + 1) * 8, hipMemcpyHostToDevice, c->stream) != hipSuccess ||
                    hipMemcpyAsync(d_s, s_scan_host, ((size_t)n_rec + 1) * 8, hipMemcpyHostToDevice, c->stream) != hipSuccess ||
                    hipMemcpyAsync(d_b, before_host, (size_t)n_rec * 8, hipMemcpyHostToDevice, c->stream) != hipSuccess ||
                    hipMemcpyAsync(d_f, gflags_host, (size_t)n_rec * 4, hipMemcpyHostToDevice, c->stream) != hipSuccess)) rc = -10;
    if (rc == 0 && bytes) {
        Timed t(c, TPC_K_STREAM);
        rc = tpc_launch_stream_write_part(c->stream, c->sp_rec, c->sp_rec + n_rec, n_rec, c->P.k, c->marks, c->emit_id, c->n_marks, c->sp_vscan, c->sp_lo, d_f, d_e, d_s, d_b,
                                          r_last, c->n_keys + 42, chunk_lo, chunk_hi, slot0, c->stream_buf);
    }
    const hipError_t e = hipStreamSynchronize(c->stream);
    for (void *p : { (void *)d_e, (void *)d_s, (void *)d_b, (void *)d_f }) if (p) (void)hipFree(p);
    stream_part_release(c);
    if (rc) return fail(c, rc, "junction stream failed (%d)", rc);
    HIPCHK(c, e);
    HIPCHK(c, hipGetLastError());
    c->stream_bytes = bytes;
    if (n_bytes) *n_bytes = bytes;
    return 0;
}

int tpc_emit_stream_fetch(tpc_ctx *c, uint64_t offset, uint64_t nbytes, void *dst_host)
{
    if (!c || (nbytes && !dst_host) || offset + nbytes > c->stream_bytes) return -1;
    if (hipSetDevice(c->device) != hipSuccess) return -10;
    if (nbytes && hipMemcpy(dst_host, (const char *)c->stream_buf + offset, nbytes, hipMemcpyDeviceToHost) != hipSuccess) return -10;
    return 0;
}

int tpc_host_alloc(void **ptr, uint64_t bytes)
{
    if (!ptr) return -1;
    return hipHostMalloc(ptr, bytes, hipHostMallocDefault) == hipSuccess ? 0 : -10;
}

void tpc_host_free(void *ptr)
{
    if (ptr) (void)hipHostFree(ptr);
}

int tpc_emit_fetch(tpc_ctx *c, uint64_t *g_host, int64_t *id_host)
{
    if (!c) return -1;
    HIPCHK(c, hipSetDevice(c->device));
    if (c->n_emit) {
        HIPCHK(c, hipMemcpy(g_host, c->marks, c->n_emit * sizeof(uint64_t), hipMemcpyDeviceToHost));
        HIPCHK(c, hipMemcpy(id_host, c->emit_id, c->n_emit * sizeof(int64_t), hipMemcpyDeviceToHost));
    }
    return 0;
}

int tpc_emit_export(tpc_ctx *c, uint64_t *g_dev, int64_t *id_dev)
{
    if (!c || (c->n_emit && (!g_dev || !id_dev))) return fail(c, -1, "bad arguments");
    HIPCHK(c, hipSetDevice(c->device));
    if (c->n_emit) {
        HIPCHK(c, hipMemcpyAsync(g_dev, c->marks, c->n_emit * sizeof(uint64_t), hipMemcpyDeviceToDevice, c->stream));
        HIPCHK(c, hipMemcpyAsync(id_dev, c->emit_id, c->n_emit * sizeof(int64_t), hipMemcpyDeviceToDevice, c->stream));
    }
    HIPCHK(c, hipStreamSynchronize(c->stream));
    return 0;
}

int tpc_emit_import(tpc_ctx *c, const uint64_t *g_dev, const int64_t *id_dev, uint64_t n)
{
    if (!c || !c->finalized || (n && (!g_dev || !id_dev))) return fail(c, -1, "junctions_finalize first");
    HIPCHK(c, hipSetDevice(c->device));
    int rc = ensure(c, c->marks, c->marks_cap, n);
    if (rc) return rc;
    if (n > c->emit_cap || !c->emit_id) {
        if (c->emit_id) (void)hipFree(c->emit_id);
        c->emit_id = nullptr; c->emit_cap = 0;
        const uint64_t cap = n + n / 8 + 16;
        HIPCHK(c, dev_malloc(c, (void **)&c->emit_id, cap * sizeof(int64_t)));
        c->emit_cap = cap;
    }
    if (n) {
        HIPCHK(c, hipMemcpyAsync(c->marks, g_dev, n * sizeof(uint64_t), hipMemcpyDeviceToDevice, c->stream));
        HIPCHK(c, hipMemcpyAsync(c->emit_id, id_dev, n * sizeof(int64_t), hipMemcpyDeviceToDevice, c->stream));
    }
    HIPCHK(c, hipStreamSynchronize(c->stream));
    c->n_marks = n; c->n_emit = n;
    c->marks_valid = false; c->rmask_sums_valid = false;
    return 0;
}
```

twopaco_amd/csrc/tpc_ctx.h:

```cpp
#pragma once
#include "../../include/twopaco_hip.h"
#include "tpc_internal.h"

#include <algorithm>
#include <atomic>
#include <cmath>
#include <chrono>
#include <cstdarg>
#include <cstdio>
#include <cstdlib>
#include <cstring>
#include <string>
#include <vector>
#include <map>

struct tpc_ctx {
    int device = 0;
    hipStream_t stream = nullptr;
    std::string err;
    bool have_params = false;
    TpcHashParams P{};
    uint64_t tab_host[TPC_TAB_WORDS]{};
    uint64_t *tab = nullptr;
    int C = 1;
    uint64_t *bases = nullptr;
    uint32_t *nmask = nullptr;
    uint64_t n_text = 0, n_words = 0, n_words_alloc = 0, n_tiles = 0;
    uint32_t *periodic = nullptr;
    bool periodic_valid = false;
    bool periodic_any_q = false, periodic_any_i = false;
    int opt_periodic = 1;
    bool opt_shard_periodic = false;
    uint64_t *bases_alloc = nullptr;
    uint32_t *nmask_alloc = nullptr;
    int opt_text_window = 0;
    bool text_windowed = false;
    uint64_t text_w0 = 0, text_w1 = 0;
    uint32_t *filter = nullptr;
    uint64_t filter_words = 0;
    uint32_t *rmask = nullptr, *mask = nullptr;
    bool mask_dirty = false;
    int rounds_done = 0;
    uint64_t *marks = nullptr;
    uint64_t marks_cap = 0, n_marks = 0;
    bool marks_valid = false;
    bool rmask_sums_valid = false;
    uint64_t rmask_sums_n = 0;
    uint64_t *block_sums = nullptr;
    uint64_t *scan_blocks = nullptr;
    void *table = nullptr;
    uint64_t table_cap = 0, table_alloc = 0;
    uint64_t *keys = nullptr;
    uint64_t n_keys = 0, keys_cap = 0;
    bool finalized = false;
    std::vector<uint64_t> keys_host;
    uint32_t *idtab = nullptr;
    uint64_t idtab_cap = 0;
    size_t idtab_bytes = 0;
    void *sort_scratch = nullptr;
    size_t sort_scratch_bytes = 0;
    int64_t *emit_id = nullptr;
    uint64_t emit_cap = 0, n_emit = 0;
    uint32_t *stream_buf = nullptr;
    uint64_t stream_cap = 0, stream_bytes = 0;
    uint64_t *sp_rec = nullptr, *sp_vscan = nullptr, *sp_cnt = nullptr, *sp_lo = nullptr;
    uint32_t *sp_flags = nullptr;
    uint32_t sp_n_rec = 0;
    int64_t *seg_name = nullptr;
    uint32_t *seg_first = nullptr;
    uint32_t *seg_ev[3] = {nullptr, nullptr, nullptr};
    uint32_t seg_n_rec = 0;
    uint64_t seg_events = 0, seg_segments = 0, seg_named = 0, seg_table_bytes = 0, seg_slots = 0, seg_peak_bytes = 0;
    uint64_t seg_err_slot = 0;
    int seg_err_kind = 0;
    bool seg_valid = false;
    unsigned long long *counters = nullptr;
    unsigned long long *route_scratch = nullptr;
    uint64_t *sh_off = nullptr;
    size_t sh_off_bytes = 0;
    int opt_test_first = 0;
    int opt_insert_mode = 0;
    int opt_slice_bits = 20;
    bool filter_zero_pending = false;
    static constexpr int NPBUF = 19;
    void *pbuf[NPBUF] = {};
    size_t pbytes[NPBUF] = {};
    std::vector<uint64_t> off2_uploaded, off3_uploaded;
    int opt_part_levels = 0;
    int opt_shard_tight = 1;
    int stat_path[2] = {0, 0};
    int64_t stat_batches[2] = {0, 0};
    mutable int stat_kernel[3] = {0, 0, 0};
    int stat_fmt[2] = {0, 0};
    int64_t stat_filter2_retries = 0;
    int64_t stat_aggregate_retries = 0;
    int stat_filter2_counted = 0;
    int64_t opt_part_min_tiles = 256;
    int64_t opt_part_budget = 0;
    int opt_query_mode = 0;
    int opt_fuse = 1;
    bool pending_apply = false;
    bool pending_fresh = false;
    bool pending_shard = false;
    TpcPartPlan pending_pl;
    void *ikeep[2] = {nullptr, nullptr};
    size_t ikeep_bytes[2] = {0, 0};
    uint64_t *ikeep_ovf = nullptr;
    uint64_t ikeep_ovf_cap = 0;
    uint64_t pending_novf = 0;
    uint32_t *iovf_cnt = nullptr;
    uint64_t *iovf_off = nullptr;
    uint32_t iovf_slices = 0;
    int64_t stat_fused = 0;
    int64_t stat_query_overflow = 0;
    int64_t stat_insert_overflow = 0;
    int64_t stat_pbuf_releases = 0;
    uint32_t sh_rank = 0, sh_world = 1;
    TpcPartPlan sh_ipl;
    TpcQPlan sh_qpl;
    bool sh_have[2] = {false, false};
    uint64_t sh_per[2] = {0, 0}, sh_batches[2] = {0, 0};
    uint64_t sh_nsurv = 0;
    bool sh_defer = false;
    bool sh_ovf_set[2] = {false, false};
    hipStream_t stream2 = nullptr;
    bool sh_async[2] = {false, false};
    unsigned long long sh_ov_host[2][2] = {{0, 0}, {0, 0}};
    int opt_replicate = 0;
    bool qb_valid = false;
    uint64_t qb_lo = 0, qb_hi = 0;
    TpcQPlan qb_pl;
    int64_t stat_q_plan[3] = {0, 0, 0};
    int stat_q_begun = 0;
    bool pending_lists = false;
    TpcListSrc cmb_ls;
    TpcPartPlan cmb_geo;
    bool cmb_have_geo = false;
    uint64_t *cmb_base = nullptr;
    unsigned long long *cmb_cur = nullptr;
    hipEvent_t ev0[TPC_K_COUNT]{}, ev1[TPC_K_COUNT]{};
    bool ev_used[TPC_K_COUNT]{};
    bool dbg_ovf = false, dbg_phases = false, dbg_timing = false, no_lean = false;
    uint64_t reserve_text_bytes = 0;
};

namespace tpch {

int fail(tpc_ctx *c, int code, const char *fmt, ...);
TpcLaunch make_launch(const tpc_ctx *c);
TpcLaunch make_launch_periodic(const tpc_ctx *c);
void ensure_periodic(tpc_ctx *c);
uint64_t rotln_host(uint64_t x, int L, int r);
hipError_t dev_malloc(tpc_ctx *c, void **p, size_t bytes);
int read_counter(tpc_ctx *c, int i, uint64_t *out);
int materialize_reset(tpc_ctx *c);
int flush_pending_apply(tpc_ctx *c);
double range_mass(const tpc_ctx *c, uint64_t lo, uint64_t hi);
bool ensure_pbuf(tpc_ctx *c, int i, size_t need);
bool release_partition_buffers(tpc_ctx *c);
uint64_t filter_words_for(int L, uint32_t world);
int64_t part_budget(const tpc_ctx *c);
uint64_t next_batches(uint64_t b);
uint64_t text_tiles512(const tpc_ctx *c);
bool replicated(const tpc_ctx *c);
void pass_tiles(const tpc_ctx *c, uint64_t &t_begin, uint64_t &t_end);
uint64_t pass_tile_count(const tpc_ctx *c);
size_t qpart_need(const TpcQPlan &pl, int i);
bool part_hash_supported(const tpc_ctx *c);
bool plan_query(const tpc_ctx *c, uint64_t lo, uint64_t hi, bool gated, TpcQPlan &pl);
int compact_mask(tpc_ctx *c, const uint32_t *m);
void stream_part_release(tpc_ctx *c);

#define HIPCHK(c, expr)                                                                         \
    do {                                                                                        \
        hipError_t e_ = (expr);                                                                 \
        if (e_ != hipSuccess) return tpch::fail(c, -10, "%s failed: %s", #expr, hipGetErrorString(e_)); \
    } while (0)

struct Timed {
    tpc_ctx *c;
    int which;
    Timed(tpc_ctx *c_, int w) : c(c_), which(w) { (void)hipEventRecord(c->ev0[w], c->stream); }
    ~Timed() { (void)hipEventRecord(c->ev1[which], c->stream); c->ev_used[which] = true; }
};

template <typename T>
int ensure(tpc_ctx *c, T *&p, uint64_t &cap, uint64_t need)
{
    if (need <= cap && p) return 0;
    if (p) (void)hipFree(p);
    p = nullptr;
    cap = 0;
    uint64_t n = need + need / 8 + 16;
    HIPCHK(c, dev_malloc(c, (void **)&p, n * sizeof(T)));
    cap = n;
    return 0;
}

}

using namespace tpch;
```

twopaco_amd/csrc/tpc_internal.h:

```cpp
#pragma once
#include "tpc_device.h"
#include <algorithm>
#include <cstdlib>
#include <vector>

struct TpcEnv {
    bool no_lean, rb_hash, verify_eager, gated_full;
    int ppr_insert, gated_loads, split_loads9;
    int slice_grid;
    static const TpcEnv &get()
    {
        static const TpcEnv e = [] {
            TpcEnv v;
            v.no_lean = getenv("TPC_NO_LEAN") != nullptr;
            v.rb_hash = getenv("TPC_RB_HASH") != nullptr;
            const char *lz = getenv("TPC_VERIFY_LAZY");
            v.verify_eager = lz && lz[0] == '0';
            v.gated_full = getenv("TPC_GATED_FULL_REGIONS") != nullptr;
            const char *p = getenv("TPC_PPR_INSERT"), *g = getenv("TPC_GATED_LOADS");
            v.ppr_insert = p ? atoi(p) : 0;
            v.gated_loads = g ? atoi(g) : 0;
            const char *s9 = getenv("TPC_SPLIT_LOADS9");
            v.split_loads9 = s9 ? atoi(s9) : 0;
            const char *lg = getenv("TPC_LOOKUP_GRID");
            int n_cu = 0, dev = 0;
            if (hipGetDevice(&dev) != hipSuccess || hipDeviceGetAttribute(&n_cu, hipDeviceAttributeMultiprocessorCount, dev) != hipSuccess || n_cu <= 0) { (void)hipGetLastError(); n_cu = 256; }
            v.slice_grid = lg ? atoi(lg) : 2 * n_cu;
            return v;
        }();
        return e;
    }
};

inline uint32_t tpc_slice_grid(uint32_t n_slices)
{
    const int g = TpcEnv::get().slice_grid;
    return g > 0 ? std::min<uint32_t>(n_slices, (uint32_t)g) : n_slices;
}

#define TPC_TAB_MAXQ 64
#define TPC_KERNEL_MAXQ 16
#define TPC_TAB_HK (TPC_TAB_MAXQ * 5)
#define TPC_TAB_WORDS (2 * TPC_TAB_MAXQ * 5)

struct TpcLaunch {
    TpcHashParams P;
    const uint64_t *tab;
    const uint64_t *bases;
    const uint32_t *nmask;
    uint64_t n_text;
    uint64_t n_tiles;
    uint32_t *filter;
    hipStream_t stream;
    const uint32_t *per_i = nullptr, *per_qs = nullptr;
    uint64_t g_begin = 0, g_end = ~0ull;
    hipEvent_t ev_lookup0 = nullptr, ev_lookup1 = nullptr;
    int *stat_kernel = nullptr;
};
constexpr int TPC_PER_MAXP = 63;
constexpr int TPC_PER_PLANES = 6;
int tpc_launch_periodic_build(const TpcLaunch &a, uint32_t *qs, uint32_t *qd, uint64_t stride, uint32_t *ins, uint64_t w_begin, uint64_t w_end, uint64_t pos_lo, uint64_t pos_hi,
                              uint32_t *any);
int tpc_launch_periodic_copy(hipStream_t stream, uint32_t *rmask, const uint32_t *qs, const uint32_t *qd, uint64_t stride, uint64_t n_words);

int tpc_launch_insert(const TpcLaunch &a, uint64_t lo, uint64_t hi, bool gated, bool test, unsigned long long *n_kmers);
int tpc_launch_query(const TpcLaunch &a, uint32_t *rmask, uint64_t lo, uint64_t hi, bool gated, unsigned long long *n_marks);
int tpc_launch_split(const TpcLaunch &a, uint32_t *emask, uint32_t *bins, uint64_t bin_size);
int tpc_launch_split_emask(hipStream_t s, const uint64_t *d_rec_start, const uint64_t *d_rec_len, uint32_t n_rec, int k, uint64_t n_words, uint32_t *emask);
int tpc_launch_hash_dump(const TpcLaunch &a, uint64_t g0, uint64_t n, uint64_t *out);
int tpc_launch_insert_anyq(const TpcLaunch &a, uint64_t lo, uint64_t hi, bool gated, bool test, unsigned long long *n_kmers);
int tpc_launch_query_anyq(const TpcLaunch &a, uint32_t *rmask, uint64_t lo, uint64_t hi, bool gated, unsigned long long *n_marks);
int tpc_launch_split_anyq(const TpcLaunch &a, uint32_t *emask, uint32_t *bins, uint64_t bin_size);
extern int tpc_test_force_anyq;

struct TpcPartPlan {
    int slice_bits, b1, b2, pos_per_round;
    int b3 = 0;
    uint32_t perm_mult, perm_inv;
    uint64_t tile0, n_tiles;
    uint32_t nwg1, wpb;
    uint32_t wpb3 = 1;
    uint64_t cap1, cap2;
    uint64_t cap3 = 0;
    int fmt2 = 0;
    uint64_t ovf_cap;
    uint32_t *buf1, *cnt1, *buf2, *cnt2;
    uint32_t *buf3 = nullptr, *cnt3 = nullptr;
    uint64_t *ovf;
    unsigned long long *ovf_cur;
    uint32_t rank = 0, world = 1;
    const uint32_t *rbuf1 = nullptr, *rcnt1 = nullptr;
    const uint64_t *roff1 = nullptr;
    const uint32_t *rown1 = nullptr, *rowncnt1 = nullptr;
};
bool tpc_part_plan(int L, int q, int slice_bits, uint64_t n_tiles, double frac, TpcPartPlan &pl, int levels = 0);
size_t tpc_part_buf1_bytes(const TpcPartPlan &pl);
size_t tpc_part_cnt1_bytes(const TpcPartPlan &pl);
size_t tpc_part_buf2_bytes(const TpcPartPlan &pl);
size_t tpc_part_cnt2_bytes(const TpcPartPlan &pl);
size_t tpc_part_buf3_bytes(const TpcPartPlan &pl);
size_t tpc_part_cnt3_bytes(const TpcPartPlan &pl);
bool tpc_part_plan_sharded(int L, int q, int slice_bits, uint64_t n_tiles, double frac, uint32_t rank, uint32_t world, TpcPartPlan &pl, int levels = 0, bool tight = false,
                           bool packed = false);
int tpc_launch_insert_partitioned(const TpcLaunch &a, const TpcPartPlan &pl, uint64_t lo, uint64_t hi, bool gated, bool fresh,
                                  unsigned long long *n_kmers);
int tpc_launch_insert_part_hash(const TpcLaunch &a, const TpcPartPlan &pl, uint64_t lo, uint64_t hi, bool gated, unsigned long long *n_kmers);
int tpc_launch_insert_part_apply(const TpcLaunch &a, const TpcPartPlan &pl, bool fresh);

struct TpcQPlan {
    int slice_bits, b1, b2, pos_per_round, sub_rounds, loads;
    int b3 = 0, loads3 = 1;
    uint32_t wpb3 = 1;
    uint64_t cap2 = 0;
    std::vector<uint64_t> off3_host;
    uint64_t buf3_entries = 0;
    uint64_t *buf3 = nullptr;
    uint32_t *cnt3 = nullptr;
    const uint64_t *off3 = nullptr;
    uint32_t perm_mult, perm_inv;
    uint64_t tile0, n_tiles;
    uint64_t tile0_global = 0;
    uint32_t nwg1, wpb;
    uint64_t cap1;
    std::vector<uint64_t> off2_host;
    uint64_t buf2_entries;
    const uint64_t *off2;
    uint64_t ovf_cap;
    uint64_t surv_cap;
    uint64_t *buf1, *buf2;
    uint32_t *cnt1, *cnt2;
    uint64_t *ovf;
    unsigned long long *ovf_cur;
    uint64_t *surv;
    unsigned long long *surv_cur;
    uint32_t rank = 0, world = 1;
    const uint64_t *rbuf1 = nullptr;
    const uint32_t *rcnt1 = nullptr;
    const uint64_t *roff1 = nullptr;
    const uint64_t *rown1 = nullptr;
    const uint32_t *rowncnt1 = nullptr;
    bool group_survivors = true;
    int fmt = 0;
    bool presplit = false;
    uint32_t tiles_per_wg = 0, n_groups = 0, pb2 = 0;
    uint32_t *bnd = nullptr;
};
#define TPC_SURV_CUR_WORDS 72
bool tpc_qpart_plan(int L, int slice_bits, uint64_t n_tiles, double frac, TpcQPlan &pl, int levels = 0);
size_t tpc_qpart_bytes(const TpcQPlan &pl, int which);
bool tpc_qpart_plan_sharded(int L, int slice_bits, uint64_t n_tiles, double frac, uint32_t rank, uint32_t world, TpcQPlan &pl, int levels = 0, bool tight = false,
                            bool packed = false);
int tpc_launch_query_partitioned(const TpcLaunch &a, const TpcQPlan &pl, uint32_t *rmask, uint64_t lo, uint64_t hi, bool gated);
int tpc_launch_insert_part_split(const TpcLaunch &a, const TpcPartPlan &pl);
int tpc_launch_insert_part_apply_only(const TpcLaunch &a, const TpcPartPlan &pl, bool fresh);
struct TpcListSrc;
int tpc_launch_query_part_fused_lookup(const TpcLaunch &a, const TpcQPlan &pl, const TpcPartPlan &ipl, bool fresh, const uint64_t *iovf_sorted, const uint64_t *iovf_off,
                                       const TpcListSrc *lists = nullptr);
int tpc_launch_ovf_by_slice(const TpcLaunch &a, const uint64_t *list, uint64_t n, int slice_bits, uint32_t n_slices, uint32_t *cnt, uint32_t *cursor,
                            uint64_t *off, uint64_t *sorted, uint32_t rank = 0, uint32_t world = 1, int log_nb2 = 0);
#define TPC_FUSE_MAX_OVF (16ull << 20)
int tpc_launch_query_verify(const TpcLaunch &a, const TpcQPlan &pl, uint32_t *rmask);
extern int tpc_test_tight_pinch;
extern int tpc_test_q6_pb2;
extern int tpc_test_insert_p3;
extern uint32_t tpc_test_sched_cap;
int tpc_launch_region_offsets(const TpcLaunch &a, const uint32_t *cnt, uint32_t n_regions, uint64_t *off);
int tpc_launch_region_pack(const TpcLaunch &a, const void *regions, uint64_t cap_entries, uint32_t entry_bytes, const uint32_t *cnt, const uint64_t *off,
                           uint32_t n_regions, void *packed);
int tpc_launch_query_part_hash(const TpcLaunch &a, const TpcQPlan &pl, uint32_t *rmask, uint64_t lo, uint64_t hi, bool gated);
int tpc_launch_query_part_lookup(const TpcLaunch &a, const TpcQPlan &pl);
int tpc_launch_query_part_split(const TpcLaunch &a, const TpcQPlan &pl);
int tpc_launch_surv_gather(const TpcLaunch &a, const TpcQPlan &pl, uint64_t *out);
int tpc_launch_verify_addrs(const TpcLaunch &a, const TpcQPlan &pl, int fn, int fn_count, const uint64_t *sid, uint64_t n, uint64_t *addr_out, int32_t *owner_out,
                            unsigned long long *owner_counts = nullptr);
#define TPC_V_OWNER_SHIFT 56
int tpc_launch_finish(hipStream_t s, const TpcQPlan &pl, const uint64_t *sid, uint64_t n, int fn_count, const uint8_t *hit, const uint32_t *perm, uint32_t *rmask,
                      unsigned long long *n_marked);
int tpc_launch_route64(hipStream_t s, const uint64_t *v, uint64_t n, int shift, uint32_t omask, uint64_t keep, unsigned long long *counts, unsigned long long *cursor,
                       uint32_t *perm, uint64_t *dst, int phase);
int tpc_launch_shard_probe(const TpcLaunch &a, const uint64_t *addr, uint64_t n, uint8_t *hit);
int tpc_launch_shard_mark(const TpcLaunch &a, const TpcQPlan &pl, const uint64_t *sid, uint64_t n, uint32_t *rmask);

int tpc_launch_survivor_sources(hipStream_t s, const uint64_t *sid, uint64_t n, uint32_t world, int32_t *src);
int tpc_launch_route(hipStream_t s, const int32_t *owner, uint64_t n, unsigned long long *counts, unsigned long long *cursor, uint32_t *perm, int phase);
int tpc_launch_permute64(hipStream_t s, const uint64_t *src, const uint32_t *perm, uint64_t n, uint64_t *dst);
int tpc_launch_select(hipStream_t s, const uint64_t *sid, uint64_t n, int fn_count, const uint8_t *hit, const uint32_t *perm, uint64_t *out, unsigned long long *n_out);

constexpr int TPC_LIST_WINDOW_BITS = 16;
constexpr int TPC_LIST_WINDOW_WORDS = 1 << (TPC_LIST_WINDOW_BITS - 5);

struct TpcListSrc {
    const uint16_t *payload = nullptr;
    const uint64_t *base = nullptr;
    const uint64_t *dir = nullptr;
    uint64_t dir_stride = 0;
    uint32_t n_src = 0;
    uint32_t n_owner = 0;
};

__host__ __device__ __forceinline__ uint32_t tpc_list_windows(int slice_bits) { return slice_bits > TPC_LIST_WINDOW_BITS ? 1u << (slice_bits - TPC_LIST_WINDOW_BITS) : 1u; }

struct TpcCombineOut { uint16_t *payload; uint64_t cap; unsigned long long *cur; uint64_t *dir; uint32_t n_dest; };
constexpr uint32_t TPC_COMBINE_PERSIST_SLICES = 16384, TPC_COMBINE_CHUNK = 512, TPC_COMBINE_MAX_WG = 1024;
int tpc_launch_slice_combine(const TpcLaunch &a, int slice_bits, int b1, int b2, uint32_t perm_mult, uint32_t perm_inv, const TpcPartPlan *ipl, const uint64_t *iovf,
                             const uint64_t *iovf_off, const TpcListSrc &ls, bool dense, bool fresh, const TpcCombineOut *out, uint32_t rank, uint32_t world);

int tpc_launch_mask_count(hipStream_t s, const uint32_t *mask, uint64_t n_words, uint64_t *block_sums, unsigned long long *n_out);
int tpc_launch_mask_scatter(hipStream_t s, const uint32_t *mask, uint64_t n_words, const uint64_t *block_sums, uint64_t *list);
int tpc_launch_mask_or(hipStream_t s, uint32_t *dst, const uint32_t *src, uint64_t n_words);

size_t tpc_table_slot_bytes(int C);
int tpc_launch_table_init(hipStream_t s, void *table, uint64_t cap);
#define TPC_FILTER2_PROBE_LIMIT 512u
int tpc_launch_mark_owner(const TpcLaunch &a, int C, const uint64_t *marks, uint64_t n_marks, uint32_t world, int32_t *owner);
int tpc_launch_mark_records(const TpcLaunch &a, int C, const uint64_t *marks, uint64_t n_marks, uint32_t world, uint64_t *records, int32_t *owner);
int tpc_launch_table_records(const TpcLaunch &a, int C, const uint64_t *marks, const void *table, uint64_t cap, const uint64_t *block_off, uint32_t world,
                             uint64_t *records, int32_t *owner);
int tpc_launch_filter2_rec(const TpcLaunch &a, int C, const uint64_t *records, uint64_t n, void *table, uint64_t cap, bool counted, unsigned long long *overflow);
int tpc_launch_scan2_write_rec(const TpcLaunch &a, int C, const uint64_t *records, const void *table, uint64_t cap, uint64_t abundance, bool counted,
                               const uint64_t *block_off, uint64_t *keys_out);
int tpc_launch_permute_rows(hipStream_t s, const uint64_t *src, const uint32_t *perm, uint64_t n, int row_words, uint64_t *dst);
int tpc_launch_filter2(const TpcLaunch &a, int C, const uint64_t *marks, uint64_t n_marks, void *table, uint64_t cap, bool counted,
                       unsigned long long *overflow);
#define TPC_SCAN2_BLOCKS 4096
int tpc_launch_scan2_count(const TpcLaunch &a, const void *table, uint64_t cap, uint64_t abundance, bool counted, uint64_t *block_tp,
                           uint64_t *block_used, unsigned long long *totals);
int tpc_launch_scan2_write(const TpcLaunch &a, int C, const uint64_t *marks, const void *table, uint64_t cap, uint64_t abundance, bool counted,
                           const uint64_t *block_off, uint64_t *keys_out);

int tpc_launch_sort_keys(hipStream_t s, int C, int k, uint64_t *keys, uint64_t J, void **scratch, size_t *scratch_bytes);

int tpc_launch_idtab_build(hipStream_t s, int C, const uint64_t *keys, uint64_t J, uint32_t *idtab, uint64_t cap);
int tpc_launch_emit(const TpcLaunch &a, int C, const uint64_t *marks, uint64_t n_marks, const uint64_t *keys, uint64_t J,
                    const uint32_t *idtab, uint64_t cap, int64_t *ids, unsigned long long *n_valid);

size_t tpc_stream_plan_bytes(uint32_t n_rec);
int tpc_launch_stream_plan(hipStream_t s, const uint64_t *d_rec_start, const uint64_t *d_rec_len, uint32_t n_rec, int k, const uint64_t *marks,
                           const int64_t *ids, uint64_t n_marks, uint64_t *vscan, void *rec, uint32_t r_last, uint64_t *totals_host);
int tpc_launch_stream_write(hipStream_t s, const uint64_t *d_rec_start, const uint64_t *d_rec_len, uint32_t n_rec, int k, const uint64_t *marks,
                            const int64_t *ids, uint64_t n_marks, const uint64_t *vscan, const void *rec, uint32_t r_last, uint64_t first_stub, uint32_t *out);

int tpc_launch_stream_partial(hipStream_t s, const uint64_t *d_rec_start, const uint64_t *d_rec_len, uint32_t n_rec, int k, const uint64_t *marks,
                              const int64_t *ids, uint64_t n_marks, uint64_t *vscan, uint64_t *cnt, uint32_t *flags, uint64_t *mark_lo);
int tpc_launch_stream_write_part(hipStream_t s, const uint64_t *d_rec_start, const uint64_t *d_rec_len, uint32_t n_rec, int k, const uint64_t *marks,
                                 const int64_t *ids, uint64_t n_marks, const uint64_t *vscan, const uint64_t *mark_lo, const uint32_t *gflags,
                                 const uint64_t *e_scan, const uint64_t *s_scan, const uint64_t *before, uint32_t r_last, uint64_t first_stub,
                                 uint64_t chunk_lo, uint64_t chunk_hi, uint64_t slot0, uint32_t *out);

int tpc_warm_pass1();
int tpc_warm_partition();
int tpc_warm_qpartition();
int tpc_warm_pass2();
int tpc_warm_stream();
#define TPC_SEG_ERR_TEXT 256
struct TpcSegResult { uint64_t events, segments, named, table_bytes, peak_bytes, err_slot; int err_kind; };
int tpc_launch_segments(hipStream_t s, const uint32_t *slots, uint64_t n_slots, int k, const uint64_t *bases, const uint32_t *nmask,
                        const uint64_t *d_rec_start, const uint64_t *d_rec_len, uint32_t n_rec, const uint64_t *d_amb, uint64_t n_amb,
                        int64_t **name_out, uint32_t **first_out, uint32_t **ev_out , TpcSegResult *res, char *err);
```

twopaco_amd/csrc/tpc_pass2.hip:

```cpp
#include "tpc_device.h"
#include "tpc_internal.h"
#include <rocprim/rocprim.hpp>
#include <algorithm>

#ifndef TPC_PASS2_PART
#define TPC_PASS2_PART 0
#endif
#if TPC_PASS2_PART == 0
#define TPC_PASS2_FN(name) name
#else
#define TPC_PASS2_FN(name) name##_long
#endif

namespace {

constexpr uint64_t EMPTY = ~0ull;
constexpr int META_NEXT_SHIFT = 5;
constexpr int META_COUNT_SHIFT = 16;
constexpr uint64_t META_MULTI = 1ull << 10;

struct Slot { uint64_t key; uint64_t meta; };

__device__ __forceinline__ uint32_t wave_incl_scan(uint32_t v)
{
    const int lane = threadIdx.x & 63;
    for (int off = 1; off < 64; off <<= 1) {
        const uint32_t t = __shfl_up(v, off, 64);
        if (lane >= off) v += t;
    }
    return v;
}

__device__ __forceinline__ uint32_t block_excl_scan256(uint32_t v, uint32_t *s_w, uint32_t &total)
{
    const int lane = threadIdx.x & 63, wv = threadIdx.x >> 6;
    const uint32_t inc = wave_incl_scan(v);
    if (lane == 63) s_w[wv] = inc;
    __syncthreads();
    uint32_t base = 0;
    for (int i = 0; i < wv; i++) base += s_w[i];
    total = s_w[0] + s_w[1] + s_w[2] + s_w[3];
    __syncthreads();
    return base + inc - v;
}

__device__ __forceinline__ void wave_add64(unsigned long long *dst, unsigned v)
{
    for (int off = 32; off > 0; off >>= 1) v += __shfl_down(v, off, 64);
    if ((threadIdx.x & 63) == 0 && v) atomicAdd(dst, (unsigned long long)v);
}

__device__ __forceinline__ void block_add64(unsigned long long *dst, unsigned v, uint32_t *s_w)
{
    for (int off = 32; off > 0; off >>= 1) v += __shfl_down(v, off, 64);
    if ((threadIdx.x & 63) == 0) s_w[threadIdx.x >> 6] = v;
    __syncthreads();
    if (threadIdx.x == 0) {
        const unsigned t = s_w[0] + s_w[1] + s_w[2] + s_w[3];
        if (t) atomicAdd(dst, (unsigned long long)t);
    }
    __syncthreads();
}

__global__ void __launch_bounds__(256) k_mask_count(const uint32_t *__restrict__ mask, uint64_t n_words, uint64_t *block_sums)
{
    __shared__ uint32_t s_w[4];
    const uint64_t w = (uint64_t)blockIdx.x * 256 + threadIdx.x;
    const uint32_t c = w < n_words ? __popc(mask[w]) : 0;
    uint32_t total;
    block_excl_scan256(c, s_w, total);
    if (threadIdx.x == 0) block_sums[blockIdx.x] = total;
}

__global__ void __launch_bounds__(256) k_scan_sums(uint64_t *block_sums, uint64_t n, unsigned long long *n_out)
{
    __shared__ unsigned long long s_w[4];
    constexpr int PER = 16;
    const int lane = threadIdx.x & 63, wv = threadIdx.x >> 6;
    unsigned long long carry = 0;
    for (uint64_t base = 0; base < n; base += 256 * PER) {
        const uint64_t i0 = base + (uint64_t)threadIdx.x * PER;
        unsigned long long v[PER], sum = 0;
#pragma unroll
        for (int j = 0; j < PER; j++) { v[j] = i0 + j < n ? block_sums[i0 + j] : 0; sum += v[j]; }
        unsigned long long inc = sum;
        for (int off = 1; off < 64; off <<= 1) {
            const unsigned long long t = __shfl_up(inc, off, 64);
            if (lane >= off) inc += t;
        }
        if (lane == 63) s_w[wv] = inc;
        __syncthreads();
        unsigned long long run = carry + inc - sum;
        for (int i = 0; i < wv; i++) run += s_w[i];
        carry += s_w[0] + s_w[1] + s_w[2] + s_w[3];
        __syncthreads();
#pragma unroll
        for (int j = 0; j < PER; j++) { if (i0 + j < n) block_sums[i0 + j] = run; run += v[j]; }
    }
    if (threadIdx.x == 0) *n_out = carry;
}

__global__ void __launch_bounds__(256) k_mask_scatter(const uint32_t *__restrict__ mask, uint64_t n_words,
                                                      const uint64_t *__restrict__ block_sums, uint64_t *__restrict__ list)
{
    __shared__ uint32_t s_w[4];
    __shared__ uint16_t s_loc[256 * 32];
    const uint64_t w = (uint64_t)blockIdx.x * 256 + threadIdx.x;
    uint32_t m = w < n_words ? mask[w] : 0;
    uint32_t total;
    uint32_t o = block_excl_scan256(__popc(m), s_w, total);
    while (m) {
        const int b = __ffs(m) - 1;
        s_loc[o++] = (uint16_t)(threadIdx.x * 32u + (uint32_t)b);
        m &= m - 1;
    }
    __syncthreads();
    const uint64_t base = block_sums[blockIdx.x], pos0 = (uint64_t)blockIdx.x * (256u * 32u);
    for (uint32_t i = threadIdx.x; i < total; i += 256) list[base + i] = pos0 + s_loc[i];
}

__global__ void k_mask_or(uint32_t *__restrict__ dst, const uint32_t *__restrict__ src, uint64_t n_words)
{
    const uint64_t stride = (uint64_t)gridDim.x * blockDim.x;
    for (uint64_t i = (uint64_t)blockIdx.x * blockDim.x + threadIdx.x; i < n_words; i += stride) dst[i] |= src[i];
}

template <int C>
__device__ __forceinline__ void load_kmer(const uint64_t *__restrict__ bases, uint64_t g, int k, uint64_t (&fw)[C])
{
#pragma unroll
    for (int w = 0; w < C; w++) {
        const int rem = k - 32 * w;
        uint64_t x = rem > 0 ? tpc_text_word(bases, g + 32 * w) : 0ull;
        if (rem > 0 && rem < 32) x &= (1ull << (2 * rem)) - 1ull;
        fw[w] = x;
    }
}

template <int C>
__device__ __forceinline__ void revcomp_kmer(const uint64_t (&fw)[C], int k, uint64_t (&rc)[C])
{
    uint64_t R[C + 2];
#pragma unroll
    for (int w = 0; w < C; w++) R[w] = tpc_revcomp_word(fw[C - 1 - w]);
    R[C] = 0; R[C + 1] = 0;
    const int s = 64 * C - 2 * k;
    const int ws = s >> 6, bs = s & 63;
#pragma unroll
    for (int w = 0; w < C; w++) {
        const uint64_t lo = ws ? R[w + 1] : R[w];
        const uint64_t hi = ws ? R[w + 2] : R[w + 1];
        rc[w] = bs ? ((lo >> bs) | (hi << (64 - bs))) : lo;
    }
}

template <int C>
__device__ __forceinline__ uint64_t fold_h0(const uint64_t (&x)[C], int k, const uint64_t *s_h0, int L, uint64_t lmask)
{
    uint64_t h = 0;
#pragma unroll
    for (int w = 0; w < C; w++) {
        int n = k - 32 * w;
        n = n > 32 ? 32 : n;
        uint64_t y = x[w];
        for (int t = 0; t < n; t++) { h = tpc_rotl1(h, L, lmask) ^ s_h0[y & 3]; y >>= 2; }
    }
    return h;
}

template <int C>
__device__ __forceinline__ bool keys_equal(const uint64_t (&a)[C], const uint64_t (&b)[C])
{
    bool eq = true;
#pragma unroll
    for (int w = 0; w < C; w++) eq = eq && a[w] == b[w];
    return eq;
}

constexpr int CANON_TAB = 32 * 4;
__device__ __forceinline__ uint64_t canon_rotl(uint64_t x, int r, int L, uint64_t lmask) { return r ? ((x << r) & lmask) | (x >> (L - r)) : x; }
__device__ __forceinline__ void canon_tab_build(uint4 *s_ct, const uint64_t *s_h0, int k, int L, uint64_t lmask)
{
    for (int i = threadIdx.x; i < 4 * (k < 32 ? k : 32); i += blockDim.x) {
        const int t = i >> 2, c = i & 3;
        const uint64_t a = canon_rotl(s_h0[c], (k - 1 - t) % L, L, lmask), b = canon_rotl(s_h0[3 - c], t % L, L, lmask);
        s_ct[i] = make_uint4((uint32_t)a, (uint32_t)(a >> 32), (uint32_t)b, (uint32_t)(b >> 32));
    }
}

template <int C>
__device__ __forceinline__ bool forward_is_canonical(const uint64_t (&fw)[C], const uint64_t (&rc)[C], int k,
                                                     const uint64_t *s_h0, int L, uint64_t lmask, const uint4 *s_ct)
{
    uint64_t hp, hn;
    if constexpr (C == 1) {
        uint32_t pl = 0, ph = 0, nl = 0, nh = 0;
        uint64_t y = fw[0];
        for (int t = 0; t < k; t++) {
            const uint4 e = s_ct[4 * t + (int)(y & 3)];
            pl ^= e.x; ph ^= e.y; nl ^= e.z; nh ^= e.w;
            y >>= 2;
        }
        hp = (uint64_t)pl | ((uint64_t)ph << 32);
        hn = (uint64_t)nl | ((uint64_t)nh << 32);
    } else {
        hp = fold_h0<C>(fw, k, s_h0, L, lmask);
        hn = fold_h0<C>(rc, k, s_h0, L, lmask);
    }
    if (hp != hn) return hp < hn;
#pragma unroll
    for (int w = 0; w < C; w++) {
        const uint64_t d = fw[w] ^ rc[w];
        if (d) {
            const int grp = (__ffsll((unsigned long long)d) - 1) >> 1;
            return ((fw[w] >> (2 * grp)) & 3) < ((rc[w] >> (2 * grp)) & 3);
        }
    }
    return false;
}

template <int C>
__device__ __forceinline__ uint64_t key_hash(const uint64_t (&key)[C])
{
    uint64_t h = 0;
#pragma unroll
    for (int w = 0; w < C; w++) h = tpc_mix64(h ^ key[w]);
    return h;
}

__global__ void k_table_init(Slot *table, uint64_t cap)
{
    const uint64_t stride = (uint64_t)gridDim.x * blockDim.x;
    for (uint64_t i = (uint64_t)blockIdx.x * blockDim.x + threadIdx.x; i < cap; i += stride) { table[i].key = EMPTY; table[i].meta = 0; }
}

template <int C, bool COUNTED>
__global__ void __launch_bounds__(256)
k_filter2(TpcHashParams P, const uint64_t *__restrict__ tab, const uint64_t *__restrict__ bases,
          const uint32_t *__restrict__ nmask, const uint64_t *__restrict__ marks, uint64_t n_marks, Slot *table, uint64_t cap,
          unsigned long long *overflow)
{
    __shared__ uint64_t s_h0[4];
    __shared__ uint4 s_ct[C == 1 ? CANON_TAB : 1];
    if (threadIdx.x < 4) s_h0[threadIdx.x] = tab[threadIdx.x];
    __syncthreads();
    if (C == 1) { canon_tab_build(s_ct, s_h0, P.k, P.L, P.lmask); __syncthreads(); }
    const uint64_t idx = (uint64_t)blockIdx.x * blockDim.x + threadIdx.x;
    if (idx >= n_marks) return;
    const uint64_t g = marks[idx];
    uint64_t fw[C], rc[C];
    load_kmer<C>(bases, g, P.k, fw);
    revcomp_kmer<C>(fw, P.k, rc);
    const bool fwd = forward_is_canonical<C>(fw, rc, P.k, s_h0, P.L, P.lmask, s_ct);
    int prev = tpc_text_char(bases, nmask, g - 1);
    int next = tpc_text_char(bases, nmask, g + P.k);
    if (!fwd) {
        const int t = prev;
        prev = tpc_rc(next);
        next = tpc_rc(t);
    }
    uint64_t ck[C];
#pragma unroll
    for (int w = 0; w < C; w++) ck[w] = fwd ? fw[w] : rc[w];
    const uint64_t mask = cap - 1;
    uint64_t slot = key_hash<C>(ck) & mask;
    bool claimed = false;
    uint64_t seen_meta = 0;
    for (uint32_t probes = 0;; probes++) {
        if (probes >= TPC_FILTER2_PROBE_LIMIT) { *overflow = 1ull; return; }
        const uint4 raw = *reinterpret_cast<const uint4 *>(&table[slot]);
        uint64_t cur = (uint64_t)raw.x | ((uint64_t)raw.y << 32);
        seen_meta = (uint64_t)raw.z | ((uint64_t)raw.w << 32);
        if (cur == EMPTY) {
            cur = atomicCAS((unsigned long long *)&table[slot].key, (unsigned long long)EMPTY, (unsigned long long)(C == 1 ? ck[0] : idx));
            seen_meta = 0;
            if (cur == EMPTY) { claimed = true; break; }
        }
        if (C == 1) {
            if (cur == ck[0]) break;
        } else {
            uint64_t ofw[C], orc[C];
            load_kmer<C>(bases, marks[cur], P.k, ofw);
            if (keys_equal<C>(ofw, ck)) break;
            revcomp_kmer<C>(ofw, P.k, orc);
            if (keys_equal<C>(orc, ck)) break;
        }
        slot = (slot + 1) & mask;
    }
    unsigned long long *meta = (unsigned long long *)&table[slot].meta;
    uint64_t want = (1ull << prev) | (1ull << (META_NEXT_SHIFT + next));
    if (!COUNTED && !claimed) want |= META_MULTI;
    if ((seen_meta & want) != want) atomicOr(meta, (unsigned long long)want);
    if (COUNTED) atomicAdd(meta, 1ull << META_COUNT_SHIFT);
}

template <int C>
__global__ void __launch_bounds__(256)
k_mark_owner(TpcHashParams P, const uint64_t *__restrict__ tab, const uint64_t *__restrict__ bases, const uint64_t *__restrict__ marks,
             uint64_t n_marks, uint32_t world, int32_t *__restrict__ owner)
{
    __shared__ uint64_t s_h0[4];
    __shared__ uint4 s_ct[C == 1 ? CANON_TAB : 1];
    if (threadIdx.x < 4) s_h0[threadIdx.x] = tab[threadIdx.x];
    __syncthreads();
    if (C == 1) { canon_tab_build(s_ct, s_h0, P.k, P.L, P.lmask); __syncthreads(); }
    const uint64_t idx = (uint64_t)blockIdx.x * blockDim.x + threadIdx.x;
    if (idx >= n_marks) return;
    uint64_t fw[C], rc[C];
    load_kmer<C>(bases, marks[idx], P.k, fw);
    revcomp_kmer<C>(fw, P.k, rc);
    const bool fwd = forward_is_canonical<C>(fw, rc, P.k, s_h0, P.L, P.lmask, s_ct);
    uint64_t ck[C];
#pragma unroll
    for (int w = 0; w < C; w++) ck[w] = fwd ? fw[w] : rc[w];
    owner[idx] = (int32_t)((key_hash<C>(ck) >> 40) % world);
}

template <int C>
__global__ void __launch_bounds__(256)
k_mark_records(TpcHashParams P, const uint64_t *__restrict__ tab, const uint64_t *__restrict__ bases, const uint32_t *__restrict__ nmask,
               const uint64_t *__restrict__ marks, uint64_t n_marks, uint32_t world, uint64_t *__restrict__ records, int32_t *__restrict__ owner)
{
    __shared__ uint64_t s_h0[4];
    __shared__ uint4 s_ct[C == 1 ? CANON_TAB : 1];
    if (threadIdx.x < 4) s_h0[threadIdx.x] = tab[threadIdx.x];
    __syncthreads();
    if (C == 1) { canon_tab_build(s_ct, s_h0, P.k, P.L, P.lmask); __syncthreads(); }
    const uint64_t idx = (uint64_t)blockIdx.x * blockDim.x + threadIdx.x;
    if (idx >= n_marks) return;
    const uint64_t g = marks[idx];
    uint64_t fw[C], rc[C];
    load_kmer<C>(bases, g, P.k, fw);
    revcomp_kmer<C>(fw, P.k, rc);
    const bool fwd = forward_is_canonical<C>(fw, rc, P.k, s_h0, P.L, P.lmask, s_ct);
    int prev = tpc_text_char(bases, nmask, g - 1);
    int next = tpc_text_char(bases, nmask, g + P.k);
    if (!fwd) {
        const int t = prev;
        prev = tpc_rc(next);
        next = tpc_rc(t);
    }
    uint64_t ck[C];
#pragma unroll
    for (int w = 0; w < C; w++) { ck[w] = fwd ? fw[w] : rc[w]; records[idx * (C + 1) + w] = ck[w]; }
    records[idx * (C + 1) + C] = (uint64_t)prev | ((uint64_t)next << 3);
    owner[idx] = (int32_t)((key_hash<C>(ck) >> 40) % world);
}

template <int C, bool COUNTED>
__global__ void __launch_bounds__(256)
k_filter2_rec(const uint64_t *__restrict__ records, uint64_t n, Slot *table, uint64_t cap, unsigned long long *overflow)
{
    const uint64_t idx = (uint64_t)blockIdx.x * blockDim.x + threadIdx.x;
    if (idx >= n) return;
    uint64_t ck[C];
#pragma unroll
    for (int w = 0; w < C; w++) ck[w] = records[idx * (C + 1) + w];
    const uint64_t pn = records[idx * (C + 1) + C];
    const bool agg = (pn >> 63) != 0;
    const int prev = (int)(pn & 7), next = (int)((pn >> 3) & 7);
    const uint64_t mask = cap - 1;
    uint64_t slot = key_hash<C>(ck) & mask;
    bool claimed = false;
    uint64_t seen_meta = 0;
    for (uint32_t probes = 0;; probes++) {
        if (probes >= TPC_FILTER2_PROBE_LIMIT) { *overflow = 1ull; return; }
        const uint4 raw = *reinterpret_cast<const uint4 *>(&table[slot]);
        uint64_t cur = (uint64_t)raw.x | ((uint64_t)raw.y << 32);
        seen_meta = (uint64_t)raw.z | ((uint64_t)raw.w << 32);
        if (cur == EMPTY) {
            cur = atomicCAS((unsigned long long *)&table[slot].key, (unsigned long long)EMPTY, (unsigned long long)(C == 1 ? ck[0] : idx));
            seen_meta = 0;
            if (cur == EMPTY) { claimed = true; break; }
        }
        if (C == 1) {
            if (cur == ck[0]) break;
        } else {
            uint64_t ok[C];
#pragma unroll
            for (int w = 0; w < C; w++) ok[w] = records[cur * (C + 1) + w];
            if (keys_equal<C>(ok, ck)) break;
        }
        slot = (slot + 1) & mask;
    }
    unsigned long long *meta = (unsigned long long *)&table[slot].meta;
    uint64_t want = agg ? (pn & ((1ull << (2 * META_NEXT_SHIFT)) - 1)) : (1ull << prev) | (1ull << (META_NEXT_SHIFT + next));
    if (!COUNTED && (!claimed || (agg && (pn & META_MULTI)))) want |= META_MULTI;
    if ((seen_meta & want) != want) atomicOr(meta, (unsigned long long)want);
    if (COUNTED) atomicAdd(meta, agg ? (pn & ~(1ull << 63)) >> META_COUNT_SHIFT << META_COUNT_SHIFT : 1ull << META_COUNT_SHIFT);
}

__device__ __forceinline__ bool slot_is_junction(const Slot &sl, uint64_t abundance, bool counted);

template <int C>
__global__ void __launch_bounds__(256)
k_scan2_write_rec(const uint64_t *__restrict__ records, const Slot *__restrict__ table, uint64_t cap, uint64_t chunk, uint64_t abundance, int counted,
                  const uint64_t *__restrict__ block_off, uint64_t *keys_out)
{
    __shared__ uint32_t s_w[4];
    const uint64_t lo = (uint64_t)blockIdx.x * chunk, hi = min(cap, lo + chunk);
    uint64_t base = block_off[blockIdx.x];
    for (uint64_t s0 = lo; s0 < hi; s0 += 256) {
        const uint64_t s = s0 + threadIdx.x;
        Slot sl;
        sl.key = EMPTY; sl.meta = 0;
        if (s < hi) {
            const uint4 raw = *reinterpret_cast<const uint4 *>(&table[s]);
            sl.key = (uint64_t)raw.x | ((uint64_t)raw.y << 32);
            sl.meta = (uint64_t)raw.z | ((uint64_t)raw.w << 32);
        }
        const bool tp = sl.key != EMPTY && slot_is_junction(sl, abundance, counted != 0);
        uint32_t total;
        const uint32_t ex = block_excl_scan256(tp ? 1u : 0u, s_w, total);
        if (tp) {
            const uint64_t o = base + ex;
            if (C == 1) keys_out[o] = sl.key;
            else {
#pragma unroll
                for (int w = 0; w < C; w++) keys_out[o * C + w] = records[sl.key * (C + 1) + w];
            }
        }
        base += total;
    }
}

__device__ __forceinline__ bool slot_is_junction(const Slot &sl, uint64_t abundance, bool counted)
{
    const uint64_t cnt = sl.meta >> META_COUNT_SHIFT;
    const unsigned pm = (unsigned)sl.meta & 31u, nm = (unsigned)(sl.meta >> META_NEXT_SHIFT) & 31u;
    const bool twice = counted ? cnt >= 2 : (sl.meta & META_MULTI) != 0;
    const bool bif = twice && (__popc(pm) > 1 || __popc(nm) > 1 || (pm & 16u) || (nm & 16u));
    return bif && (!counted || cnt <= abundance);
}

__global__ void __launch_bounds__(256)
k_scan2_count(const Slot *__restrict__ table, uint64_t cap, uint64_t chunk, uint64_t abundance, int counted,
              uint64_t *block_tp, uint64_t *block_used)
{
    __shared__ uint32_t s_w[4];
    const uint64_t lo = (uint64_t)blockIdx.x * chunk, hi = min(cap, lo + chunk);
    unsigned used = 0, tp = 0;
    for (uint64_t s = lo + threadIdx.x; s < hi; s += 256) {
        const uint4 raw = *reinterpret_cast<const uint4 *>(&table[s]);
        Slot sl;
        sl.key = (uint64_t)raw.x | ((uint64_t)raw.y << 32);
        sl.meta = (uint64_t)raw.z | ((uint64_t)raw.w << 32);
        if (sl.key == EMPTY) continue;
        used++;
        tp += slot_is_junction(sl, abundance, counted != 0);
    }
    uint32_t total;
    block_excl_scan256(tp, s_w, total);
    if (threadIdx.x == 0) block_tp[blockIdx.x] = total;
    block_excl_scan256(used, s_w, total);
    if (threadIdx.x == 0) block_used[blockIdx.x] = total;
}

template <int C>
__global__ void __launch_bounds__(256)
k_scan2_write(TpcHashParams P, const uint64_t *__restrict__ tab, const uint64_t *__restrict__ bases,
              const uint64_t *__restrict__ marks, const Slot *__restrict__ table, uint64_t cap, uint64_t chunk, uint64_t abundance,
              int counted, const uint64_t *__restrict__ block_off, uint64_t *keys_out)
{
    __shared__ uint64_t s_h0[4];
    __shared__ uint32_t s_w[4];
    __shared__ uint4 s_ct[C == 1 ? CANON_TAB : 1];
    if (threadIdx.x < 4) s_h0[threadIdx.x] = tab[threadIdx.x];
    __syncthreads();
    if (C == 1) { canon_tab_build(s_ct, s_h0, P.k, P.L, P.lmask); __syncthreads(); }
    const uint64_t lo = (uint64_t)blockIdx.x * chunk, hi = min(cap, lo + chunk);
    uint64_t base = block_off[blockIdx.x];
    for (uint64_t s0 = lo; s0 < hi; s0 += 256) {
        const uint64_t s = s0 + threadIdx.x;
        Slot sl;
        sl.key = EMPTY; sl.meta = 0;
        if (s < hi) {
            const uint4 raw = *reinterpret_cast<const uint4 *>(&table[s]);
            sl.key = (uint64_t)raw.x | ((uint64_t)raw.y << 32);
            sl.meta = (uint64_t)raw.z | ((uint64_t)raw.w << 32);
        }
        const bool tp = sl.key != EMPTY && slot_is_junction(sl, abundance, counted != 0);
        uint32_t total;
        const uint32_t ex = block_excl_scan256(tp ? 1u : 0u, s_w, total);
        if (tp) {
            const uint64_t o = base + ex;
            if (C == 1) {
                keys_out[o] = sl.key;
            } else {
                uint64_t fw[C], rc[C];
                load_kmer<C>(bases, marks[sl.key], P.k, fw);
                revcomp_kmer<C>(fw, P.k, rc);
                const bool fwd = forward_is_canonical<C>(fw, rc, P.k, s_h0, P.L, P.lmask, s_ct);
#pragma unroll
                for (int w = 0; w < C; w++) keys_out[o * C + w] = fwd ? fw[w] : rc[w];
            }
        }
        base += total;
    }
}

template <int C>
__global__ void __launch_bounds__(256)
k_table_records(TpcHashParams P, const uint64_t *__restrict__ tab, const uint64_t *__restrict__ bases, const uint64_t *__restrict__ marks,
                const Slot *__restrict__ table, uint64_t cap, uint64_t chunk, const uint64_t *__restrict__ block_off, uint32_t world,
                uint64_t *__restrict__ records, int32_t *__restrict__ owner)
{
    __shared__ uint64_t s_h0[4];
    __shared__ uint32_t s_w[4];
    __shared__ uint4 s_ct[C == 1 ? CANON_TAB : 1];
    if (threadIdx.x < 4) s_h0[threadIdx.x] = tab[threadIdx.x];
    __syncthreads();
    if (C == 1) { canon_tab_build(s_ct, s_h0, P.k, P.L, P.lmask); __syncthreads(); }
    const uint64_t lo = (uint64_t)blockIdx.x * chunk, hi = min(cap, lo + chunk);
    uint64_t base = block_off[blockIdx.x];
    for (uint64_t s0 = lo; s0 < hi; s0 += 256) {
        const uint64_t s = s0 + threadIdx.x;
        Slot sl;
        sl.key = EMPTY; sl.meta = 0;
        if (s < hi) {
            const uint4 raw = *reinterpret_cast<const uint4 *>(&table[s]);
            sl.key = (uint64_t)raw.x | ((uint64_t)raw.y << 32);
            sl.meta = (uint64_t)raw.z | ((uint64_t)raw.w << 32);
        }
        const bool used = sl.key != EMPTY;
        uint32_t total;
        const uint32_t ex = block_excl_scan256(used ? 1u : 0u, s_w, total);
        if (used) {
            const uint64_t o = base + ex;
            uint64_t ck[C];
            if (C == 1) ck[0] = sl.key;
            else {
                uint64_t fw[C], rc[C];
                load_kmer<C>(bases, marks[sl.key], P.k, fw);
                revcomp_kmer<C>(fw, P.k, rc);
                const bool fwd = forward_is_canonical<C>(fw, rc, P.k, s_h0, P.L, P.lmask, s_ct);
#pragma unroll
                for (int w = 0; w < C; w++) ck[w] = fwd ? fw[w] : rc[w];
            }
#pragma unroll
            for (int w = 0; w < C; w++) records[o * (C + 1) + w] = ck[w];
            records[o * (C + 1) + C] = sl.meta | ((sl.meta >> META_COUNT_SHIFT) >= 2 ? META_MULTI : 0ull) | (1ull << 63);
            owner[o] = (int32_t)((key_hash<C>(ck) >> 40) % world);
        }
        base += total;
    }
}

template <int C>
__global__ void __launch_bounds__(256) k_idtab_build(const uint64_t *__restrict__ keys, uint64_t J, uint32_t *idtab, uint64_t cap)
{
    const uint64_t i = (uint64_t)blockIdx.x * blockDim.x + threadIdx.x;
    if (i >= J) return;
    uint64_t key[C];
#pragma unroll
    for (int w = 0; w < C; w++) key[w] = keys[i * C + w];
    const uint64_t mask = cap - 1;
    uint64_t slot = key_hash<C>(key) & mask;
    if (C == 1) {
        while (atomicCAS(&idtab[slot * 4 + 2], 0u, (uint32_t)(i + 1)) != 0u) slot = (slot + 1) & mask;
        idtab[slot * 4 + 0] = (uint32_t)key[0];
        idtab[slot * 4 + 1] = (uint32_t)(key[0] >> 32);
        return;
    }
    while (atomicCAS(&idtab[slot], 0u, (uint32_t)(i + 1)) != 0u) slot = (slot + 1) & mask;
}

template <int C>
__global__ void __launch_bounds__(256)
k_emit(TpcHashParams P, const uint64_t *__restrict__ tab, const uint64_t *__restrict__ bases,
       const uint64_t *__restrict__ marks, uint64_t n_marks, const uint64_t *__restrict__ keys, uint64_t J,
       const uint32_t *__restrict__ idtab, uint64_t cap, int64_t *__restrict__ ids, unsigned long long *n_valid)
{
    __shared__ uint64_t s_h0[4];
    __shared__ uint4 s_ct[C == 1 ? CANON_TAB : 1];
    if (threadIdx.x < 4) s_h0[threadIdx.x] = tab[threadIdx.x];
    __syncthreads();
    if (C == 1) { canon_tab_build(s_ct, s_h0, P.k, P.L, P.lmask); __syncthreads(); }
    __shared__ uint32_t s_w[4];
    unsigned valid = 0;
    const uint64_t stride = (uint64_t)gridDim.x * blockDim.x;
    for (uint64_t idx = (uint64_t)blockIdx.x * blockDim.x + threadIdx.x; idx < n_marks; idx += stride) {
        int64_t id = INT64_MAX;
        if (J > 0) {
            const uint64_t g = marks[idx];
            uint64_t fw[C], rc[C], ck[C];
            load_kmer<C>(bases, g, P.k, fw);
            revcomp_kmer<C>(fw, P.k, rc);
            const bool fwd = forward_is_canonical<C>(fw, rc, P.k, s_h0, P.L, P.lmask, s_ct);
#pragma unroll
            for (int w = 0; w < C; w++) ck[w] = fwd ? fw[w] : rc[w];
            const uint64_t mask = cap - 1;
            uint64_t slot = key_hash<C>(ck) & mask;
            for (;;) {
                uint32_t r;
                uint64_t sk[C];
                if (C == 1) {
                    const uint4 sl = reinterpret_cast<const uint4 *>(idtab)[slot];
                    r = sl.z;
                    if (r == 0) break;
                    sk[0] = (uint64_t)sl.x | ((uint64_t)sl.y << 32);
                } else {
                    r = idtab[slot];
                    if (r == 0) break;
#pragma unroll
                    for (int w = 0; w < C; w++) sk[w] = keys[(uint64_t)(r - 1) * C + w];
                }
                if (keys_equal<C>(sk, ck)) {
                    id = keys_equal<C>(ck, fw) ? (int64_t)r : -(int64_t)r;
                    valid++;
                    break;
                }
                slot = (slot + 1) & mask;
            }
        }
        ids[idx] = id;
    }
    block_add64(n_valid, valid, s_w);
}

__global__ void k_iota(uint32_t *p, uint64_t n)
{
    const uint64_t i = (uint64_t)blockIdx.x * blockDim.x + threadIdx.x;
    if (i < n) p[i] = (uint32_t)i;
}
__global__ void k_gather_word(const uint64_t *__restrict__ keys, const uint32_t *__restrict__ perm, uint64_t n, int C, int w, uint64_t *out)
{
    const uint64_t i = (uint64_t)blockIdx.x * blockDim.x + threadIdx.x;
    if (i < n) out[i] = keys[(uint64_t)perm[i] * C + w];
}
__global__ void k_gather_keys(const uint64_t *__restrict__ keys, const uint32_t *__restrict__ perm, uint64_t n, int C, uint64_t *out)
{
    const uint64_t i = (uint64_t)blockIdx.x * blockDim.x + threadIdx.x;
    if (i < n)
        for (int w = 0; w < C; w++) out[i * C + w] = keys[(uint64_t)perm[i] * C + w];
}

inline unsigned nblk(uint64_t n, unsigned b) { return (unsigned)((n + b - 1) / b); }

}

#if TPC_PASS2_PART == 0
#define TPC_DISPATCH_C(C_, CALL)                                                                  \
    switch (C_) {                                                                                 \
    case 1: CALL(1); break; case 2: CALL(2); break;                                               \
    default: return -1;                                                                           \
    }
#else
#define TPC_DISPATCH_C(C_, CALL)                                                                  \
    switch (C_) {                                                                                 \
    case 3: CALL(3); break; case 4: CALL(4); break;                                               \
    case 5: CALL(5); break; case 6: CALL(6); break; case 7: CALL(7); break; case 8: CALL(8); break;       \
    case 9: CALL(9); break; case 10: CALL(10); break; case 11: CALL(11); break; case 12: CALL(12); break; \
    case 13: CALL(13); break; case 14: CALL(14); break; case 15: CALL(15); break; case 16: CALL(16); break; \
    case 17: CALL(17); break; case 18: CALL(18); break; case 19: CALL(19); break;                 \
    default: return -1;                                                                           \
    }
#endif
int tpc_launch_filter2_long(const TpcLaunch &a, int C, const uint64_t *marks, uint64_t n_marks, void *table, uint64_t cap, bool counted,
                            unsigned long long *overflow);
int tpc_launch_scan2_write_long(const TpcLaunch &a, int C, const uint64_t *marks, const void *table, uint64_t cap, uint64_t abundance, bool counted,
                                const uint64_t *block_off, uint64_t *keys_out);
int tpc_launch_idtab_build_long(hipStream_t s, int C, const uint64_t *keys, uint64_t J, uint32_t *idtab, uint64_t cap);
int tpc_launch_sort_keys_long(hipStream_t s, int C, uint64_t *keys, uint64_t J);
int tpc_launch_emit_long(const TpcLaunch &a, int C, const uint64_t *marks, uint64_t n_marks, const uint64_t *keys, uint64_t J,
                         const uint32_t *idtab, uint64_t cap, int64_t *ids, unsigned long long *n_valid);

#if TPC_PASS2_PART == 0
constexpr uint32_t SCAN_SEG = 4096;
__global__ void __launch_bounds__(256) k_scan_sums_seg(const uint64_t *__restrict__ block_sums, uint64_t n, unsigned long long *__restrict__ seg_tot)
{
    __shared__ unsigned long long s64[4];
    const uint64_t i0 = (uint64_t)blockIdx.x * SCAN_SEG, i1 = min(n, i0 + SCAN_SEG);
    unsigned long long sum = 0;
    for (uint64_t i = i0 + threadIdx.x; i < i1; i += 256) sum += block_sums[i];
    for (int o = 32; o > 0; o >>= 1) sum += __shfl_xor(sum, o, 64);
    if ((threadIdx.x & 63) == 0) s64[threadIdx.x >> 6] = sum;
    __syncthreads();
    if (threadIdx.x == 0) seg_tot[blockIdx.x] = s64[0] + s64[1] + s64[2] + s64[3];
}
__global__ void __launch_bounds__(256) k_scan_sums_wide(uint64_t *block_sums, uint64_t n, const unsigned long long *__restrict__ seg_tot, unsigned long long *n_out)
{
    __shared__ unsigned long long s_w[4];
    constexpr int PER = SCAN_SEG / 256;
    const int lane = threadIdx.x & 63, wv = threadIdx.x >> 6;
    unsigned long long base = 0, all = 0;
    for (uint32_t g = 0; g < gridDim.x; g++) { const unsigned long long t = seg_tot[g]; if (g < blockIdx.x) base += t; all += t; }
    const uint64_t i0 = (uint64_t)blockIdx.x * SCAN_SEG + (uint64_t)threadIdx.x * PER;
    unsigned long long v[PER], sum = 0;
#pragma unroll
    for (int j = 0; j < PER; j++) { v[j] = i0 + j < n ? block_sums[i0 + j] : 0; sum += v[j]; }
    unsigned long long inc = sum;
    for (int off = 1; off < 64; off <<= 1) {
        const unsigned long long t = __shfl_up(inc, off, 64);
        if (lane >= off) inc += t;
    }
    if (lane == 63) s_w[wv] = inc;
    __syncthreads();
    unsigned long long run = base + inc - sum;
    for (int i = 0; i < wv; i++) run += s_w[i];
#pragma unroll
    for (int j = 0; j < PER; j++) { if (i0 + j < n) block_sums[i0 + j] = run; run += v[j]; }
    if (blockIdx.x == 0 && threadIdx.x == 0) *n_out = all;
}

int tpc_launch_mask_count(hipStream_t s, const uint32_t *mask, uint64_t n_words, uint64_t *block_sums, unsigned long long *n_out)
{
    const unsigned nb = nblk(n_words, 256);
    hipLaunchKernelGGL(k_mask_count, dim3(nb), dim3(256), 0, s, mask, n_words, block_sums);
    const unsigned segs = (nb + SCAN_SEG - 1) / SCAN_SEG;
    if (segs < 2 || segs > 64) { hipLaunchKernelGGL(k_scan_sums, dim3(1), dim3(256), 0, s, block_sums, (uint64_t)nb, n_out); return 0; }
    unsigned long long *seg_tot = reinterpret_cast<unsigned long long *>(block_sums + nb);
    hipLaunchKernelGGL(k_scan_sums_seg, dim3(segs), dim3(256), 0, s, block_sums, (uint64_t)nb, seg_tot);
    hipLaunchKernelGGL(k_scan_sums_wide, dim3(segs), dim3(256), 0, s, block_sums, (uint64_t)nb, seg_tot, n_out);
    return 0;
}

int tpc_launch_mask_scatter(hipStream_t s, const uint32_t *mask, uint64_t n_words, const uint64_t *block_sums, uint64_t *list)
{
    hipLaunchKernelGGL(k_mask_scatter, dim3(nblk(n_words, 256)), dim3(256), 0, s, mask, n_words, block_sums, list);
    return 0;
}

int tpc_launch_mask_or(hipStream_t s, uint32_t *dst, const uint32_t *src, uint64_t n_words)
{
    hipLaunchKernelGGL(k_mask_or, dim3(2048), dim3(256), 0, s, dst, src, n_words);
    return 0;
}

size_t tpc_table_slot_bytes(int) { return sizeof(Slot); }

int tpc_launch_table_init(hipStream_t s, void *table, uint64_t cap)
{
    hipLaunchKernelGGL(k_table_init, dim3(2048), dim3(256), 0, s, (Slot *)table, cap);
    return 0;
}

#endif

int TPC_PASS2_FN(tpc_launch_filter2)(const TpcLaunch &a, int C, const uint64_t *marks, uint64_t n_marks, void *table, uint64_t cap, bool counted,
                       unsigned long long *overflow)
{
    if (n_marks == 0) return 0;
#if TPC_PASS2_PART == 0
    if (C > 2) return tpc_launch_filter2_long(a, C, marks, n_marks, table, cap, counted, overflow);
#endif
#define CALL(C_)                                                                                                                         \
    if (counted) hipLaunchKernelGGL((k_filter2<C_, true>), dim3(nblk(n_marks, 256)), dim3(256), 0, a.stream, a.P, a.tab, a.bases, a.nmask, \
                                    marks, n_marks, (Slot *)table, cap, overflow);                                                       \
    else hipLaunchKernelGGL((k_filter2<C_, false>), dim3(nblk(n_marks, 256)), dim3(256), 0, a.stream, a.P, a.tab, a.bases, a.nmask, marks, \
                            n_marks, (Slot *)table, cap, overflow)
    TPC_DISPATCH_C(C, CALL)
#undef CALL
    return 0;
}

int tpc_launch_mark_owner_long(const TpcLaunch &a, int C, const uint64_t *marks, uint64_t n_marks, uint32_t world, int32_t *owner);
int TPC_PASS2_FN(tpc_launch_mark_owner)(const TpcLaunch &a, int C, const uint64_t *marks, uint64_t n_marks, uint32_t world, int32_t *owner)
{
    if (n_marks == 0) return 0;
#if TPC_PASS2_PART == 0
    if (C > 2) return tpc_launch_mark_owner_long(a, C, marks, n_marks, world, owner);
#endif
#define CALL(C_) hipLaunchKernelGGL((k_mark_owner<C_>), dim3(nblk(n_marks, 256)), dim3(256), 0, a.stream, a.P, a.tab, a.bases, marks, n_marks, world, owner)
    TPC_DISPATCH_C(C, CALL)
#undef CALL
    return 0;
}

int tpc_launch_mark_records_long(const TpcLaunch &a, int C, const uint64_t *marks, uint64_t n_marks, uint32_t world, uint64_t *records, int32_t *owner);
int TPC_PASS2_FN(tpc_launch_mark_records)(const TpcLaunch &a, int C, const uint64_t *marks, uint64_t n_marks, uint32_t world, uint64_t *records, int32_t *owner)
{
    if (n_marks == 0) return 0;
#if TPC_PASS2_PART == 0
    if (C > 2) return tpc_launch_mark_records_long(a, C, marks, n_marks, world, records, owner);
#endif
#define CALL(C_) hipLaunchKernelGGL((k_mark_records<C_>), dim3(nblk(n_marks, 256)), dim3(256), 0, a.stream, a.P, a.tab, a.bases, a.nmask, marks, n_marks, world, records, owner)
    TPC_DISPATCH_C(C, CALL)
#undef CALL
    return 0;
}

int tpc_launch_table_records_long(const TpcLaunch &a, int C, const uint64_t *marks, const void *table, uint64_t cap, const uint64_t *block_off, uint32_t world,
                                  uint64_t *records, int32_t *owner);
uint64_t TPC_PASS2_FN(tpc_scan2_chunk)(uint64_t cap);
int TPC_PASS2_FN(tpc_launch_table_records)(const TpcLaunch &a, int C, const uint64_t *marks, const void *table, uint64_t cap, const uint64_t *block_off, uint32_t world,
                                           uint64_t *records, int32_t *owner)
{
#if TPC_PASS2_PART == 0
    if (C > 2) return tpc_launch_table_records_long(a, C, marks, table, cap, block_off, world, records, owner);
#endif
    const uint64_t chunk = TPC_PASS2_FN(tpc_scan2_chunk)(cap);
#define CALL(C_) hipLaunchKernelGGL((k_table_records<C_>), dim3(TPC_SCAN2_BLOCKS), dim3(256), 0, a.stream, a.P, a.tab, a.bases, marks, (const Slot *)table, cap, chunk, block_off, world, records, owner)
    TPC_DISPATCH_C(C, CALL)
#undef CALL
    return 0;
}

int tpc_launch_filter2_rec_long(const TpcLaunch &a, int C, const uint64_t *records, uint64_t n, void *table, uint64_t cap, bool counted, unsigned long long *overflow);
int TPC_PASS2_FN(tpc_launch_filter2_rec)(const TpcLaunch &a, int C, const uint64_t *records, uint64_t n, void *table, uint64_t cap, bool counted,
                                         unsigned long long *overflow)
{
    if (n == 0) return 0;
#if TPC_PASS2_PART == 0
    if (C > 2) return tpc_launch_filter2_rec_long(a, C, records, n, table, cap, counted, overflow);
#endif
#define CALL(C_)                                                                                                                                  \
    if (counted) hipLaunchKernelGGL((k_filter2_rec<C_, true>), dim3(nblk(n, 256)), dim3(256), 0, a.stream, records, n, (Slot *)table, cap, overflow); \
    else hipLaunchKernelGGL((k_filter2_rec<C_, false>), dim3(nblk(n, 256)), dim3(256), 0, a.stream, records, n, (Slot *)table, cap, overflow)
    TPC_DISPATCH_C(C, CALL)
#undef CALL
    return 0;
}

uint64_t TPC_PASS2_FN(tpc_scan2_chunk)(uint64_t cap);
int tpc_launch_scan2_write_rec_long(const TpcLaunch &a, int C, const uint64_t *records, const void *table, uint64_t cap, uint64_t abundance, bool counted,
                                    const uint64_t *block_off, uint64_t *keys_out);
int TPC_PASS2_FN(tpc_launch_scan2_write_rec)(const TpcLaunch &a, int C, const uint64_t *records, const void *table, uint64_t cap, uint64_t abundance, bool counted,
                                             const uint64_t *block_off, uint64_t *keys_out)
{
#if TPC_PASS2_PART == 0
    if (C > 2) return tpc_launch_scan2_write_rec_long(a, C, records, table, cap, abundance, counted, block_off, keys_out);
#endif
    const uint64_t chunk = TPC_PASS2_FN(tpc_scan2_chunk)(cap);
#define CALL(C_) hipLaunchKernelGGL((k_scan2_write_rec<C_>), dim3(TPC_SCAN2_BLOCKS), dim3(256), 0, a.stream, records, (const Slot *)table, cap, chunk, abundance, counted ? 1 : 0, block_off, keys_out)
    TPC_DISPATCH_C(C, CALL)
#undef CALL
    return 0;
}

uint64_t TPC_PASS2_FN(tpc_scan2_chunk)(uint64_t cap) { return ((cap + TPC_SCAN2_BLOCKS - 1) / TPC_SCAN2_BLOCKS + 255) / 256 * 256; }

#if TPC_PASS2_PART == 0
int tpc_launch_scan2_count(const TpcLaunch &a, const void *table, uint64_t cap, uint64_t abundance, bool counted, uint64_t *block_tp,
                           uint64_t *block_used, unsigned long long *totals)
{
    const uint64_t chunk = tpc_scan2_chunk(cap);
    hipLaunchKernelGGL(k_scan2_count, dim3(TPC_SCAN2_BLOCKS), dim3(256), 0, a.stream, (const Slot *)table, cap, chunk, abundance, counted ? 1 : 0,
                       block_tp, block_used);
    hipLaunchKernelGGL(k_scan_sums, dim3(1), dim3(256), 0, a.stream, block_tp, (uint64_t)TPC_SCAN2_BLOCKS, totals);
    hipLaunchKernelGGL(k_scan_sums, dim3(1), dim3(256), 0, a.stream, block_used, (uint64_t)TPC_SCAN2_BLOCKS, totals + 1);
    return 0;
}

#endif

int TPC_PASS2_FN(tpc_launch_scan2_write)(const TpcLaunch &a, int C, const uint64_t *marks, const void *table, uint64_t cap, uint64_t abundance, bool counted,
                           const uint64_t *block_off, uint64_t *keys_out)
{
#if TPC_PASS2_PART == 0
    if (C > 2) return tpc_launch_scan2_write_long(a, C, marks, table, cap, abundance, counted, block_off, keys_out);
#endif
    const uint64_t chunk = TPC_PASS2_FN(tpc_scan2_chunk)(cap);
#define CALL(C_) hipLaunchKernelGGL((k_scan2_write<C_>), dim3(TPC_SCAN2_BLOCKS), dim3(256), 0, a.stream, a.P, a.tab, a.bases, marks, (const Slot *)table, cap, chunk, abundance, counted ? 1 : 0, block_off, keys_out)
    TPC_DISPATCH_C(C, CALL)
#undef CALL
    return 0;
}

#if TPC_PASS2_PART == 0
int tpc_launch_sort_keys(hipStream_t s, int C, int k, uint64_t *keys, uint64_t J, void **scratch, size_t *scratch_bytes)
{
    if (J < 2) return 0;
    hipError_t e;
    if (C == 1) {
        size_t tmp_bytes = 0;
        int end_bit = 2 * k;
        if (end_bit > 64) end_bit = 64;
        uint64_t *out = nullptr;
        if ((e = rocprim::radix_sort_keys(nullptr, tmp_bytes, keys, out, J, 0, end_bit, s)) != hipSuccess) return -2;
        const size_t out_bytes = (J * sizeof(uint64_t) + 255) & ~(size_t)255;
        const size_t need = out_bytes + (tmp_bytes ? tmp_bytes : 8);
        if (need > *scratch_bytes) {
            if (*scratch) (void)hipFree(*scratch);
            *scratch = nullptr; *scratch_bytes = 0;
            if (hipMalloc(scratch, need + need / 4) != hipSuccess) return -3;
            *scratch_bytes = need + need / 4;
        }
        out = (uint64_t *)*scratch;
        void *tmp = (char *)*scratch + out_bytes;
        e = rocprim::radix_sort_keys(tmp, tmp_bytes, keys, out, J, 0, end_bit, s);
        if (e == hipSuccess) e = hipMemcpyAsync(keys, out, J * sizeof(uint64_t), hipMemcpyDeviceToDevice, s);
        return e == hipSuccess ? 0 : -2;
    }
    return tpc_launch_sort_keys_long(s, C, keys, J);
}
#endif

#if TPC_PASS2_PART == 1
int tpc_launch_sort_keys_long(hipStream_t s, int C, uint64_t *keys, uint64_t J)
{
    uint64_t *kw = nullptr, *kw2 = nullptr, *out = nullptr;
    uint32_t *perm = nullptr, *perm2 = nullptr;
    void *tmp = nullptr;
    size_t tmp_bytes = 0;
    int rc = 0;
    if (rocprim::radix_sort_pairs(nullptr, tmp_bytes, kw, kw2, perm, perm2, J, 0, 64, s) != hipSuccess) return -2;
    if (hipMalloc(&kw, J * 8) != hipSuccess || hipMalloc(&kw2, J * 8) != hipSuccess || hipMalloc(&out, J * C * 8) != hipSuccess ||
        hipMalloc(&perm, J * 4) != hipSuccess || hipMalloc(&perm2, J * 4) != hipSuccess || hipMalloc(&tmp, tmp_bytes ? tmp_bytes : 8) != hipSuccess) {
        rc = -3;
    } else {
        hipLaunchKernelGGL(k_iota, dim3(nblk(J, 256)), dim3(256), 0, s, perm, J);
        for (int w = C - 1; w >= 0 && rc == 0; w--) {
            hipLaunchKernelGGL(k_gather_word, dim3(nblk(J, 256)), dim3(256), 0, s, keys, perm, J, C, w, kw);
            if (rocprim::radix_sort_pairs(tmp, tmp_bytes, kw, kw2, perm, perm2, J, 0, 64, s) != hipSuccess) rc = -2;
            uint32_t *t = perm; perm = perm2; perm2 = t;
        }
        if (rc == 0) {
            hipLaunchKernelGGL(k_gather_keys, dim3(nblk(J, 256)), dim3(256), 0, s, keys, perm, J, C, out);
            if (hipMemcpyAsync(keys, out, J * C * 8, hipMemcpyDeviceToDevice, s) != hipSuccess) rc = -2;
        }
        (void)hipStreamSynchronize(s);
    }
    (void)hipFree(kw); (void)hipFree(kw2); (void)hipFree(out); (void)hipFree(perm); (void)hipFree(perm2); (void)hipFree(tmp);
    return rc;
}
#endif

int TPC_PASS2_FN(tpc_launch_idtab_build)(hipStream_t s, int C, const uint64_t *keys, uint64_t J, uint32_t *idtab, uint64_t cap)
{
    if (J == 0) return 0;
#if TPC_PASS2_PART == 0
    if (C > 2) return tpc_launch_idtab_build_long(s, C, keys, J, idtab, cap);
#endif
#define CALL(C_) hipLaunchKernelGGL((k_idtab_build<C_>), dim3(nblk(J, 256)), dim3(256), 0, s, keys, J, idtab, cap)
    TPC_DISPATCH_C(C, CALL)
#undef CALL
    return 0;
}

int TPC_PASS2_FN(tpc_launch_emit)(const TpcLaunch &a, int C, const uint64_t *marks, uint64_t n_marks, const uint64_t *keys, uint64_t J,
                    const uint32_t *idtab, uint64_t cap, int64_t *ids, unsigned long long *n_valid)
{
    if (n_marks == 0) return 0;
#if TPC_PASS2_PART == 0
    if (C > 2) return tpc_launch_emit_long(a, C, marks, n_marks, keys, J, idtab, cap, ids, n_valid);
#endif
#define CALL(C_) hipLaunchKernelGGL((k_emit<C_>), dim3(std::min<unsigned>(nblk(n_marks, 256), 16384u)), dim3(256), 0, a.stream, a.P, a.tab, a.bases, marks, n_marks, keys, J, idtab, cap, ids, n_valid)
    TPC_DISPATCH_C(C, CALL)
#undef CALL
    return 0;
}

#if TPC_PASS2_PART == 0
__global__ void k_warm_pass2() {}
int tpc_warm_pass2() { hipFuncAttributes a; return hipFuncGetAttributes(&a, reinterpret_cast<const void *>(k_warm_pass2)) == hipSuccess ? 0 : -1; }
#endif
```

Baseline: 12.38 billion.

## Emit junction ids via filter2 slot indices instead of rehashing marks

During filter2, each mark records the hash-table slot it landed in plus a strand bit. scan2_write records the slot of each junction key, and the key sort now carries those slots as values. Emit then builds a slot-to-rank table and maps every mark to its id through two small array lookups, which avoids recomputing k-mers and probing the id hash table. Building the id table is skipped when this path is used. The change adds per-mark and per-key slot arrays, a sort that now carries values, and a validity flag that many entry points must clear. The filter2 table-size divisor becomes an option.

```diff
diff --git a/twopaco_amd/csrc/tpc_capi.hip b/twopaco_amd/csrc/tpc_capi.hip
--- a/twopaco_amd/csrc/tpc_capi.hip
+++ b/twopaco_amd/csrc/tpc_capi.hip
@@ -256,6 +256,7 @@
         tpc_launch_mask_count(c->stream, m, c->n_words, c->block_sums, c->counters + 2);
         if ((rc = read_counter(c, 2, &n))) return rc;
     }
+    c->ms_valid = false;
     rc = ensure(c, c->marks, c->marks_cap, n);
     if (rc) return rc;
     if (n) tpc_launch_mask_scatter(c->stream, m, c->n_words, c->block_sums, c->marks);
@@ -296,7 +297,7 @@
     (void)hipSetDevice(c->device);
     (void)hipStreamSynchronize(c->stream);
     void *ptrs[] = { c->tab, c->bases_alloc, c->nmask_alloc, c->filter, c->rmask, c->mask, c->marks, c->block_sums, c->table,
-                     c->keys, c->idtab, c->emit_id, c->stream_buf, c->counters, c->route_scratch, c->sh_off, c->scan_blocks, c->sort_scratch, c->seg_name, c->seg_first, c->seg_ev[0], c->seg_ev[1], c->seg_ev[2] };
+                     c->keys, c->idtab, c->markslot, c->key_slot, c->slotrank, c->emit_id, c->stream_buf, c->counters, c->route_scratch, c->sh_off, c->scan_blocks, c->sort_scratch, c->seg_name, c->seg_first, c->seg_ev[0], c->seg_ev[1], c->seg_ev[2] };
     for (void *p : ptrs) if (p) (void)hipFree(p);
     stream_part_release(c);
     for (void *p : c->pbuf) if (p) (void)hipFree(p);
@@ -333,6 +334,8 @@
     if (!strcmp(name, "periodic_skip")) { c->opt_periodic = value != 0; if (!value) c->periodic_valid = false; return 0; }
     if (!strcmp(name, "test_tight_pinch")) { tpc_test_tight_pinch = (int)value; c->sh_have[0] = c->sh_have[1] = false; return 0; }
     if (!strcmp(name, "test_sched_cap")) { tpc_test_sched_cap = value > 0 ? (uint32_t)value : 0; return 0; }
+    if (!strcmp(name, "emit_by_slot")) { c->opt_emit_by_slot = value != 0; return 0; }
+    if (!strcmp(name, "filter2_table_div")) { c->opt_filter2_div = value < 1 ? 1 : value; return 0; }
     if (!strcmp(name, "text_window")) { c->opt_text_window = value != 0; return 0; }
     if (!strcmp(name, "replicate_filter")) { c->opt_replicate = value != 0; return 0; }
     if (!strcmp(name, "test_force_anyq")) { tpc_test_force_anyq = value != 0; return 0; }
@@ -379,6 +382,12 @@
     if (!strcmp(name, "filter2_retries")) return c->stat_filter2_retries;
     if (!strcmp(name, "aggregate_retries")) return c->stat_aggregate_retries;
     if (!strcmp(name, "filter2_counted")) return c->stat_filter2_counted;
+    if (!strcmp(name, "emit_by_slot")) return c->stat_emit_by_slot;
+    if (!strcmp(name, "filter2_table_slots")) return (int64_t)c->table_cap;
+    if (!strcmp(name, "pass2_bytes")) {
+        return (int64_t)(c->marks_cap * 8 + c->emit_cap * 8 + c->table_alloc * tpc_table_slot_bytes(c->C) + c->keys_cap * c->C * 8 + c->idtab_bytes + c->markslot_cap * 4 +
+                         c->key_slot_cap * 4 + c->slotrank_cap * 4 + c->sort_scratch_bytes + c->stream_cap);
+    }
     if (!strcmp(name, "fused_lookups")) return c->stat_fused;
     if (!strcmp(name, "query_overflow_entries")) return c->stat_query_overflow;
     if (!strcmp(name, "insert_overflow_entries")) return c->stat_insert_overflow;
diff --git a/twopaco_amd/csrc/tpc_capi_pass2.hip b/twopaco_amd/csrc/tpc_capi_pass2.hip
--- a/twopaco_amd/csrc/tpc_capi_pass2.hip
+++ b/twopaco_amd/csrc/tpc_capi_pass2.hip
@@ -63,6 +63,7 @@
     if (!c || !c->marks_valid || world == 0 || !n_records || (c->n_marks && (!records_dev || !owner_dev))) return fail(c, -1, "tpc_pass2_marks first");
     HIPCHK(c, hipSetDevice(c->device));
     *n_records = 0;
+    c->ms_valid = false;
     if (c->n_marks == 0) return 0;
     const size_t sb = tpc_table_slot_bytes(c->C);
     TpcLaunch a = make_launch(c);
@@ -85,7 +86,7 @@
         HIPCHK(c, hipMemsetAsync(c->counters + 6, 0, sizeof(unsigned long long), c->stream));
         Timed t(c, TPC_K_FILTER2);
         tpc_launch_table_init(c->stream, c->table, cap);
-        if (tpc_launch_filter2(a, c->C, c->marks, c->n_marks, c->table, cap, counted, c->counters + 6)) return fail(c, -1, "filter2 launch failed");
+        if (tpc_launch_filter2(a, c->C, c->marks, c->n_marks, c->table, cap, counted, c->counters + 6, nullptr)) return fail(c, -1, "filter2 launch failed");
         if (tpc_launch_scan2_count(a, c->table, cap, abundance, counted, c->scan_blocks, c->scan_blocks + TPC_SCAN2_BLOCKS, c->counters + 4))
             return fail(c, -1, "scan2 launch failed");
         unsigned long long three[3] = {0, 0, 0};
@@ -144,9 +145,12 @@
     uint64_t full = 1024;
     while (full < 2 * n_marks + 2) full <<= 1;
     uint64_t cap = 1024;
-    while (cap < n_marks / 4 + 2) cap <<= 1;
+    while (cap < n_marks / (uint64_t)c->opt_filter2_div + 2) cap <<= 1;
     if (aggregated) cap = full;
     uint64_t tp = 0, used = 0;
+    c->ms_valid = false;
+    const bool want_slots = c->opt_emit_by_slot && c->C == 1 && !external && !records && c->rounds_done == 0 && c->n_keys == 0;
+    bool slots = false;
     c->stat_filter2_retries = 0;
     c->stat_filter2_counted = counted ? 1 : 0;
     for (;;) {
@@ -158,12 +162,18 @@
             c->table_alloc = cap;
         }
         c->table_cap = cap;
+        slots = want_slots && cap <= (1ull << 31);
+        if (slots) {
+            int rc = ensure(c, c->markslot, c->markslot_cap, n_marks);
+            if (rc) return rc;
+        }
         HIPCHK(c, hipMemsetAsync(c->counters + 6, 0, sizeof(unsigned long long), c->stream));
         {
             Timed t(c, TPC_K_FILTER2);
             tpc_launch_table_init(c->stream, c->table, cap);
             if (records ? tpc_launch_filter2_rec(a, c->C, marks, n_marks, c->table, cap, counted, c->counters + 6)
-                        : tpc_launch_filter2(a, c->C, marks, n_marks, c->table, cap, counted, c->counters + 6)) return fail(c, -1, "filter2 launch failed");
+                        : tpc_launch_filter2(a, c->C, marks, n_marks, c->table, cap, counted, c->counters + 6, slots ? c->markslot : nullptr))
+                return fail(c, -1, "filter2 launch failed");
         }
         uint64_t too_full = 0;
         {
@@ -186,8 +196,13 @@
                     c->keys = nk;
                     c->keys_cap = ncap;
                 }
+                if (slots) {
+                    int rc = ensure(c, c->key_slot, c->key_slot_cap, tp);
+                    if (rc) return rc;
+                }
                 if (records ? tpc_launch_scan2_write_rec(a, c->C, marks, c->table, cap, abundance, counted, c->scan_blocks, c->keys + c->n_keys * c->C)
-                            : tpc_launch_scan2_write(a, c->C, marks, c->table, cap, abundance, counted, c->scan_blocks, c->keys + c->n_keys * c->C))
+                            : tpc_launch_scan2_write(a, c->C, marks, c->table, cap, abundance, counted, c->scan_blocks, c->keys + c->n_keys * c->C,
+                                                     slots ? c->key_slot : nullptr))
                     return fail(c, -1, "scan2 launch failed");
                 c->n_keys += tp;
             }
@@ -207,6 +222,8 @@
     c->finalized = false;
     HIPCHK(c, hipGetLastError());
     HIPCHK(c, hipStreamSynchronize(c->stream));
+    c->ms_valid = slots;
+    c->ms_keys = c->n_keys;
     if (n_true) *n_true = tp;
     if (n_false) *n_false = used - tp;
     if (table_size) *table_size = used;
@@ -215,28 +232,44 @@
 
 }
 
+namespace {
+int build_idtab(tpc_ctx *c)
+{
+    uint64_t cap = 1024;
+    while (cap < 2 * c->n_keys + 2) cap <<= 1;
+    const size_t slot_bytes = c->C == 1 ? 16 : 4;
+    if (cap * slot_bytes > c->idtab_bytes) {
+        if (c->idtab) (void)hipFree(c->idtab);
+        c->idtab = nullptr;
+        c->idtab_bytes = 0;
+        HIPCHK(c, dev_malloc(c, (void **)&c->idtab, cap * slot_bytes));
+        c->idtab_bytes = cap * slot_bytes;
+    }
+    c->idtab_cap = cap;
+    HIPCHK(c, hipMemsetAsync(c->idtab, 0, cap * slot_bytes, c->stream));
+    if (c->n_keys >= 0xFFFFFFFFull) return fail(c, -1, "too many junctions for the 32-bit id index");
+    tpc_launch_idtab_build(c->stream, c->C, c->keys, c->n_keys, c->idtab, cap);
+    c->idtab_valid = true;
+    return 0;
+}
+inline bool slots_usable(const tpc_ctx *c)
+{
+    return c->opt_emit_by_slot && c->C == 1 && c->ms_valid && c->marks_valid && !c->mask_dirty && c->rounds_done == 1 && c->n_keys == c->ms_keys && c->n_keys < 0xFFFFFFFFull;
+}
+}
+
 int tpc_junctions_finalize(tpc_ctx *c, uint64_t *n_junctions)
 {
     if (!c || !c->have_params) return fail(c, -1, "set_params first");
     HIPCHK(c, hipSetDevice(c->device));
+    c->by_slot = slots_usable(c);
     {
         Timed t(c, TPC_K_SORT);
-        int rc = tpc_launch_sort_keys(c->stream, c->C, c->P.k, c->keys, c->n_keys, &c->sort_scratch, &c->sort_scratch_bytes);
+        int rc = tpc_launch_sort_keys(c->stream, c->C, c->P.k, c->keys, c->n_keys, &c->sort_scratch, &c->sort_scratch_bytes, c->by_slot ? c->key_slot : nullptr);
         if (rc) return fail(c, rc, "key sort failed (%d)", rc);
-        uint64_t cap = 1024;
-        while (cap < 2 * c->n_keys + 2) cap <<= 1;
-        const size_t slot_bytes = c->C == 1 ? 16 : 4;
-        if (cap * slot_bytes > c->idtab_bytes) {
-            if (c->idtab) (void)hipFree(c->idtab);
-            c->idtab = nullptr;
-            c->idtab_bytes = 0;
-            HIPCHK(c, dev_malloc(c, (void **)&c->idtab, cap * slot_bytes));
-            c->idtab_bytes = cap * slot_bytes;
-        }
-        c->idtab_cap = cap;
-        HIPCHK(c, hipMemsetAsync(c->idtab, 0, cap * slot_bytes, c->stream));
-        if (c->n_keys >= 0xFFFFFFFFull) return fail(c, -1, "too many junctions for the 32-bit id index");
-        tpc_launch_idtab_build(c->stream, c->C, c->keys, c->n_keys, c->idtab, cap);
+        c->idtab_valid = false;
+        c->ms_valid = c->by_slot;
+        if (!c->by_slot && (rc = build_idtab(c))) return rc;
     }
     HIPCHK(c, hipGetLastError());
     HIPCHK(c, hipStreamSynchronize(c->stream));
@@ -280,6 +313,7 @@
     }
     if (n) HIPCHK(c, hipMemcpy(c->keys, keys_host, n * c->C * sizeof(uint64_t), hipMemcpyHostToDevice));
     c->n_keys = n;
+    c->ms_valid = false;
     c->finalized = false;
     c->keys_host.clear();
     return 0;
@@ -314,6 +348,7 @@
     if (n) HIPCHK(c, hipMemcpyAsync(c->keys + base * c->C, src_dev, n * c->C * sizeof(uint64_t), hipMemcpyDeviceToDevice, c->stream));
     HIPCHK(c, hipStreamSynchronize(c->stream));
     c->n_keys = need;
+    c->ms_valid = false;
     c->finalized = false;
     c->keys_host.clear();
     return 0;
@@ -372,11 +407,20 @@
         c->emit_cap = cap;
     }
     HIPCHK(c, hipMemsetAsync(c->counters + 3, 0, sizeof(unsigned long long), c->stream));
+    const bool by_slot = c->by_slot && c->ms_valid && c->marks_valid;
+    if (by_slot && (rc = ensure(c, c->slotrank, c->slotrank_cap, c->table_cap))) return rc;
     {
         Timed t(c, TPC_K_EMIT);
-        if (tpc_launch_emit(make_launch(c), c->C, c->marks, c->n_marks, c->keys, c->n_keys, c->idtab, c->idtab_cap, c->emit_id, c->counters + 3))
-            return fail(c, -1, "emit launch failed");
-    }
+        if (by_slot) {
+            if (tpc_launch_emit_slots(c->stream, c->key_slot, c->n_keys, c->slotrank, c->table_cap, c->markslot, c->n_marks, c->emit_id, c->counters + 3))
+                return fail(c, -1, "emit launch failed");
+        } else {
+            if (!c->idtab_valid && (rc = build_idtab(c))) return rc;
+            if (tpc_launch_emit(make_launch(c), c->C, c->marks, c->n_marks, c->keys, c->n_keys, c->idtab, c->idtab_cap, c->emit_id, c->counters + 3))
+                return fail(c, -1, "emit launch failed");
+        }
+    }
+    c->stat_emit_by_slot = by_slot ? 1 : 0;
     HIPCHK(c, hipGetLastError());
     uint64_t nv = 0;
     if ((rc = read_counter(c, 3, &nv))) return rc;
@@ -571,5 +615,6 @@
     HIPCHK(c, hipStreamSynchronize(c->stream));
     c->n_marks = n; c->n_emit = n;
     c->marks_valid = false; c->rmask_sums_valid = false;
-    return 0;
-}
+    c->ms_valid = false;
+    return 0;
+}
diff --git a/twopaco_amd/csrc/tpc_ctx.h b/twopaco_amd/csrc/tpc_ctx.h
--- a/twopaco_amd/csrc/tpc_ctx.h
+++ b/twopaco_amd/csrc/tpc_ctx.h
@@ -59,6 +59,17 @@
     size_t idtab_bytes = 0;
     void *sort_scratch = nullptr;
     size_t sort_scratch_bytes = 0;
+    bool idtab_valid = false;
+    int opt_emit_by_slot = 1;
+    int64_t opt_filter2_div = 4;
+    uint32_t *markslot = nullptr;
+    uint32_t *key_slot = nullptr;
+    uint32_t *slotrank = nullptr;
+    uint64_t markslot_cap = 0, key_slot_cap = 0, slotrank_cap = 0;
+    bool ms_valid = false;
+    uint64_t ms_keys = 0;
+    bool by_slot = false;
+    int stat_emit_by_slot = 0;
     int64_t *emit_id = nullptr;
     uint64_t emit_cap = 0, n_emit = 0;
     uint32_t *stream_buf = nullptr;
diff --git a/twopaco_amd/csrc/tpc_internal.h b/twopaco_amd/csrc/tpc_internal.h
--- a/twopaco_amd/csrc/tpc_internal.h
+++ b/twopaco_amd/csrc/tpc_internal.h
@@ -221,18 +221,20 @@
                                const uint64_t *block_off, uint64_t *keys_out);
 int tpc_launch_permute_rows(hipStream_t s, const uint64_t *src, const uint32_t *perm, uint64_t n, int row_words, uint64_t *dst);
 int tpc_launch_filter2(const TpcLaunch &a, int C, const uint64_t *marks, uint64_t n_marks, void *table, uint64_t cap, bool counted,
-                       unsigned long long *overflow);
+                       unsigned long long *overflow, uint32_t *markslot);
 #define TPC_SCAN2_BLOCKS 4096
 int tpc_launch_scan2_count(const TpcLaunch &a, const void *table, uint64_t cap, uint64_t abundance, bool counted, uint64_t *block_tp,
                            uint64_t *block_used, unsigned long long *totals);
 int tpc_launch_scan2_write(const TpcLaunch &a, int C, const uint64_t *marks, const void *table, uint64_t cap, uint64_t abundance, bool counted,
-                           const uint64_t *block_off, uint64_t *keys_out);
-
-int tpc_launch_sort_keys(hipStream_t s, int C, int k, uint64_t *keys, uint64_t J, void **scratch, size_t *scratch_bytes);
+                           const uint64_t *block_off, uint64_t *keys_out, uint32_t *slots_out);
+
+int tpc_launch_sort_keys(hipStream_t s, int C, int k, uint64_t *keys, uint64_t J, void **scratch, size_t *scratch_bytes, uint32_t *vals);
 
 int tpc_launch_idtab_build(hipStream_t s, int C, const uint64_t *keys, uint64_t J, uint32_t *idtab, uint64_t cap);
 int tpc_launch_emit(const TpcLaunch &a, int C, const uint64_t *marks, uint64_t n_marks, const uint64_t *keys, uint64_t J,
                     const uint32_t *idtab, uint64_t cap, int64_t *ids, unsigned long long *n_valid);
+int tpc_launch_emit_slots(hipStream_t s, const uint32_t *key_slot, uint64_t J, uint32_t *slotrank, uint64_t cap, const uint32_t *markslot, uint64_t n_marks,
+                          int64_t *ids, unsigned long long *n_valid);
 
 size_t tpc_stream_plan_bytes(uint32_t n_rec);
 int tpc_launch_stream_plan(hipStream_t s, const uint64_t *d_rec_start, const uint64_t *d_rec_len, uint32_t n_rec, int k, const uint64_t *marks,
diff --git a/twopaco_amd/csrc/tpc_pass2.hip b/twopaco_amd/csrc/tpc_pass2.hip
--- a/twopaco_amd/csrc/tpc_pass2.hip
+++ b/twopaco_amd/csrc/tpc_pass2.hip
@@ -238,7 +238,7 @@
 __global__ void __launch_bounds__(256)
 k_filter2(TpcHashParams P, const uint64_t *__restrict__ tab, const uint64_t *__restrict__ bases,
           const uint32_t *__restrict__ nmask, const uint64_t *__restrict__ marks, uint64_t n_marks, Slot *table, uint64_t cap,
-          unsigned long long *overflow)
+          unsigned long long *overflow, uint32_t *__restrict__ markslot)
 {
     __shared__ uint64_t s_h0[4];
     __shared__ uint4 s_ct[C == 1 ? CANON_TAB : 1];
@@ -287,6 +287,7 @@
         }
         slot = (slot + 1) & mask;
     }
+    if (C == 1 && markslot) markslot[idx] = (uint32_t)slot | (ck[0] == fw[0] ? 1u << 31 : 0u);
     unsigned long long *meta = (unsigned long long *)&table[slot].meta;
     uint64_t want = (1ull << prev) | (1ull << (META_NEXT_SHIFT + next));
     if (!COUNTED && !claimed) want |= META_MULTI;
@@ -460,7 +461,7 @@
 __global__ void __launch_bounds__(256)
 k_scan2_write(TpcHashParams P, const uint64_t *__restrict__ tab, const uint64_t *__restrict__ bases,
               const uint64_t *__restrict__ marks, const Slot *__restrict__ table, uint64_t cap, uint64_t chunk, uint64_t abundance,
-              int counted, const uint64_t *__restrict__ block_off, uint64_t *keys_out)
+              int counted, const uint64_t *__restrict__ block_off, uint64_t *keys_out, uint32_t *__restrict__ slots_out)
 {
     __shared__ uint64_t s_h0[4];
     __shared__ uint32_t s_w[4];
@@ -486,6 +487,7 @@
             const uint64_t o = base + ex;
             if (C == 1) {
                 keys_out[o] = sl.key;
+                if (slots_out) slots_out[o] = (uint32_t)s;
             } else {
                 uint64_t fw[C], rc[C];
                 load_kmer<C>(bases, marks[sl.key], P.k, fw);
@@ -618,6 +620,44 @@
     block_add64(n_valid, valid, s_w);
 }
 
+#if TPC_PASS2_PART == 0
+__global__ void __launch_bounds__(256) k_slot_rank(const uint32_t *__restrict__ key_slot, uint64_t J, uint32_t *__restrict__ slotrank, uint64_t cap)
+{
+    const uint64_t r = (uint64_t)blockIdx.x * blockDim.x + threadIdx.x;
+    if (r < J) slotrank[key_slot[r] & (cap - 1)] = (uint32_t)(r + 1);
+}
+
+typedef uint32_t MsQuad __attribute__((ext_vector_type(4)));
+typedef long long IdPair __attribute__((ext_vector_type(2)));
+__device__ __forceinline__ int64_t slot_id(uint32_t ms, const uint32_t *__restrict__ slotrank, uint32_t smask, unsigned &valid)
+{
+    const uint32_t r = slotrank[ms & smask];
+    valid += r != 0;
+    return r == 0 ? INT64_MAX : (ms >> 31) ? (int64_t)r : -(int64_t)r;
+}
+
+__global__ void __launch_bounds__(256)
+k_emit_slots(const uint32_t *__restrict__ markslot, uint64_t n_marks, const uint32_t *__restrict__ slotrank, uint64_t cap,
+             int64_t *__restrict__ ids, unsigned long long *n_valid)
+{
+    __shared__ uint32_t s_w[4];
+    const uint32_t smask = (uint32_t)(cap - 1) & 0x7FFFFFFFu;
+    unsigned valid = 0;
+    const uint64_t quads = n_marks >> 2, stride = (uint64_t)gridDim.x * blockDim.x, t0 = (uint64_t)blockIdx.x * blockDim.x + threadIdx.x;
+    for (uint64_t q = t0; q < quads; q += stride) {
+        const MsQuad ms = __builtin_nontemporal_load(reinterpret_cast<const MsQuad *>(markslot) + q);
+        IdPair a, b;
+        a.x = slot_id(ms.x, slotrank, smask, valid); a.y = slot_id(ms.y, slotrank, smask, valid);
+        b.x = slot_id(ms.z, slotrank, smask, valid); b.y = slot_id(ms.w, slotrank, smask, valid);
+        __builtin_nontemporal_store(a, reinterpret_cast<IdPair *>(ids) + 2 * q);
+        __builtin_nontemporal_store(b, reinterpret_cast<IdPair *>(ids) + 2 * q + 1);
+    }
+    const uint64_t idx = 4 * quads + t0;
+    if (idx < n_marks) ids[idx] = slot_id(markslot[idx], slotrank, smask, valid);
+    block_add64(n_valid, valid, s_w);
+}
+#endif
+
 __global__ void k_iota(uint32_t *p, uint64_t n)
 {
     const uint64_t i = (uint64_t)blockIdx.x * blockDim.x + threadIdx.x;
@@ -657,9 +697,9 @@
     }
 #endif
 int tpc_launch_filter2_long(const TpcLaunch &a, int C, const uint64_t *marks, uint64_t n_marks, void *table, uint64_t cap, bool counted,
-                            unsigned long long *overflow);
+                            unsigned long long *overflow, uint32_t *markslot);
 int tpc_launch_scan2_write_long(const TpcLaunch &a, int C, const uint64_t *marks, const void *table, uint64_t cap, uint64_t abundance, bool counted,
-                                const uint64_t *block_off, uint64_t *keys_out);
+                                const uint64_t *block_off, uint64_t *keys_out, uint32_t *slots_out);
 int tpc_launch_idtab_build_long(hipStream_t s, int C, const uint64_t *keys, uint64_t J, uint32_t *idtab, uint64_t cap);
 int tpc_launch_sort_keys_long(hipStream_t s, int C, uint64_t *keys, uint64_t J);
 int tpc_launch_emit_long(const TpcLaunch &a, int C, const uint64_t *marks, uint64_t n_marks, const uint64_t *keys, uint64_t J,
@@ -738,17 +778,18 @@
 #endif
 
 int TPC_PASS2_FN(tpc_launch_filter2)(const TpcLaunch &a, int C, const uint64_t *marks, uint64_t n_marks, void *table, uint64_t cap, bool counted,
-                       unsigned long long *overflow)
+                       unsigned long long *overflow, uint32_t *markslot)
 {
     if (n_marks == 0) return 0;
-#if TPC_PASS2_PART == 0
-    if (C > 2) return tpc_launch_filter2_long(a, C, marks, n_marks, table, cap, counted, overflow);
+    if (markslot && (C != 1 || cap > (1ull << 31))) return -1;
+#if TPC_PASS2_PART == 0
+    if (C > 2) return tpc_launch_filter2_long(a, C, marks, n_marks, table, cap, counted, overflow, markslot);
 #endif
 #define CALL(C_)                                                                                                                         \
     if (counted) hipLaunchKernelGGL((k_filter2<C_, true>), dim3(nblk(n_marks, 256)), dim3(256), 0, a.stream, a.P, a.tab, a.bases, a.nmask, \
-                                    marks, n_marks, (Slot *)table, cap, overflow);                                                       \
+                                    marks, n_marks, (Slot *)table, cap, overflow, markslot);                                             \
     else hipLaunchKernelGGL((k_filter2<C_, false>), dim3(nblk(n_marks, 256)), dim3(256), 0, a.stream, a.P, a.tab, a.bases, a.nmask, marks, \
-                            n_marks, (Slot *)table, cap, overflow)
+                            n_marks, (Slot *)table, cap, overflow, markslot)
     TPC_DISPATCH_C(C, CALL)
 #undef CALL
     return 0;
@@ -845,21 +886,23 @@
 #endif
 
 int TPC_PASS2_FN(tpc_launch_scan2_write)(const TpcLaunch &a, int C, const uint64_t *marks, const void *table, uint64_t cap, uint64_t abundance, bool counted,
-                           const uint64_t *block_off, uint64_t *keys_out)
-{
-#if TPC_PASS2_PART == 0
-    if (C > 2) return tpc_launch_scan2_write_long(a, C, marks, table, cap, abundance, counted, block_off, keys_out);
+                           const uint64_t *block_off, uint64_t *keys_out, uint32_t *slots_out)
+{
+    if (slots_out && (C != 1 || cap > (1ull << 31))) return -1;
+#if TPC_PASS2_PART == 0
+    if (C > 2) return tpc_launch_scan2_write_long(a, C, marks, table, cap, abundance, counted, block_off, keys_out, slots_out);
 #endif
     const uint64_t chunk = TPC_PASS2_FN(tpc_scan2_chunk)(cap);
-#define CALL(C_) hipLaunchKernelGGL((k_scan2_write<C_>), dim3(TPC_SCAN2_BLOCKS), dim3(256), 0, a.stream, a.P, a.tab, a.bases, marks, (const Slot *)table, cap, chunk, abundance, counted ? 1 : 0, block_off, keys_out)
+#define CALL(C_) hipLaunchKernelGGL((k_scan2_write<C_>), dim3(TPC_SCAN2_BLOCKS), dim3(256), 0, a.stream, a.P, a.tab, a.bases, marks, (const Slot *)table, cap, chunk, abundance, counted ? 1 : 0, block_off, keys_out, slots_out)
     TPC_DISPATCH_C(C, CALL)
 #undef CALL
     return 0;
 }
 
 #if TPC_PASS2_PART == 0
-int tpc_launch_sort_keys(hipStream_t s, int C, int k, uint64_t *keys, uint64_t J, void **scratch, size_t *scratch_bytes)
-{
+int tpc_launch_sort_keys(hipStream_t s, int C, int k, uint64_t *keys, uint64_t J, void **scratch, size_t *scratch_bytes, uint32_t *vals)
+{
+    if (vals && C != 1) return -1;
     if (J < 2) return 0;
     hipError_t e;
     if (C == 1) {
@@ -867,8 +910,11 @@
         int end_bit = 2 * k;
         if (end_bit > 64) end_bit = 64;
         uint64_t *out = nullptr;
-        if ((e = rocprim::radix_sort_keys(nullptr, tmp_bytes, keys, out, J, 0, end_bit, s)) != hipSuccess) return -2;
-        const size_t out_bytes = (J * sizeof(uint64_t) + 255) & ~(size_t)255;
+        uint32_t *vout = nullptr;
+        if ((e = vals ? rocprim::radix_sort_pairs(nullptr, tmp_bytes, keys, out, vals, vout, J, 0, end_bit, s)
+                      : rocprim::radix_sort_keys(nullptr, tmp_bytes, keys, out, J, 0, end_bit, s)) != hipSuccess) return -2;
+        const size_t vout_bytes = vals ? (J * sizeof(uint32_t) + 255) & ~(size_t)255 : 0;
+        const size_t out_bytes = ((J * sizeof(uint64_t) + 255) & ~(size_t)255) + vout_bytes;
         const size_t need = out_bytes + (tmp_bytes ? tmp_bytes : 8);
         if (need > *scratch_bytes) {
             if (*scratch) (void)hipFree(*scratch);
@@ -877,9 +923,12 @@
             *scratch_bytes = need + need / 4;
         }
         out = (uint64_t *)*scratch;
+        vout = (uint32_t *)((char *)*scratch + out_bytes - vout_bytes);
         void *tmp = (char *)*scratch + out_bytes;
-        e = rocprim::radix_sort_keys(tmp, tmp_bytes, keys, out, J, 0, end_bit, s);
+        e = vals ? rocprim::radix_sort_pairs(tmp, tmp_bytes, keys, out, vals, vout, J, 0, end_bit, s)
+                 : rocprim::radix_sort_keys(tmp, tmp_bytes, keys, out, J, 0, end_bit, s);
         if (e == hipSuccess) e = hipMemcpyAsync(keys, out, J * sizeof(uint64_t), hipMemcpyDeviceToDevice, s);
+        if (e == hipSuccess && vals) e = hipMemcpyAsync(vals, vout, J * sizeof(uint32_t), hipMemcpyDeviceToDevice, s);
         return e == hipSuccess ? 0 : -2;
     }
     return tpc_launch_sort_keys_long(s, C, keys, J);
@@ -942,6 +991,18 @@
 }
 
 #if TPC_PASS2_PART == 0
+int tpc_launch_emit_slots(hipStream_t s, const uint32_t *key_slot, uint64_t J, uint32_t *slotrank, uint64_t cap, const uint32_t *markslot, uint64_t n_marks,
+                          int64_t *ids, unsigned long long *n_valid)
+{
+    if (cap == 0 || (cap & (cap - 1)) || cap > (1ull << 31) || J >= 0xFFFFFFFFull) return -1;
+    if (hipMemsetAsync(slotrank, 0, cap * sizeof(uint32_t), s) != hipSuccess) return -2;
+    if (J) hipLaunchKernelGGL(k_slot_rank, dim3(nblk(J, 256)), dim3(256), 0, s, key_slot, J, slotrank, cap);
+    if (n_marks) hipLaunchKernelGGL(k_emit_slots, dim3(std::min<unsigned>(nblk((n_marks + 3) / 4, 256), 2048u)), dim3(256), 0, s, markslot, n_marks, slotrank, cap, ids, n_valid);
+    return 0;
+}
+#endif
+
+#if TPC_PASS2_PART == 0
 __global__ void k_warm_pass2() {}
 int tpc_warm_pass2() { hipFuncAttributes a; return hipFuncGetAttributes(&a, reinterpret_cast<const void *>(k_warm_pass2)) == hipSuccess ? 0 : -1; }
 #endif
```

After: 12.11 billion. 0.978x the previous value.
